# mravanelli/pytorch-kaldi

Hardware: AMD Instinct MI355X
Metric: train_frames_per_sec (higher is better)
Workload: dtype bf16

## Files before the change

### include/pk_amd.h

```cpp
#ifndef PK_AMD_H
#define PK_AMD_H

#include <stdint.h>

#ifdef __cplusplus
extern "C" {
#endif

#define PK_PREC_F32 0
#define PK_PREC_BF16 1

#define PK_ACT_LINEAR 0
#define PK_ACT_RELU 1
#define PK_ACT_TANH 2
#define PK_ACT_SIGMOID 3
#define PK_ACT_LEAKY_RELU 4
#define PK_ACT_ELU 5

#define PK_CELL_LIGRU 0
#define PK_CELL_RNN 1
#define PK_CELL_LSTM 2
#define PK_CELL_GRU 3
#define PK_CELL_MINGRU 4

#define PK_REC_STEPWISE 0
#define PK_REC_PERSISTENT 1

int pk_version(void);
const char* pk_last_error(void);
int pk_num_cu(void);

int pk_gemm(void* stream, int prec, int M, int N, int K, float alpha, const float* A, int64_t a_rs,
            int64_t a_cs, const float* B, int64_t b_rs, int64_t b_cs, float beta, float* C, int64_t ldc,
            const float* bias, int splitk, float* workspace);
void pk_gemm_f32_set_form(int form);

int pk_gemm_bf16_tile_m(int M);
int pk_gemm_bf16_auto_splitk(int M, int N, int K);
int pk_gemm_bf16_auto_splitk_cus(int M, int N, int K, int cus);
void pk_gemm_bf16_set_tile(int tile);
int pk_gemm_bf16(void* stream, int M, int N, int K, float alpha, const uint16_t* A, int64_t lda, int a_kc,
                 const uint16_t* B, int64_t ldb, int b_kc, float beta, float* C, int64_t ldc, const float* bias,
                 int splitk, float* workspace);
int64_t pk_gemm_bf16_stats_floats(int M, int N);
int pk_gemm_bf16_stats(void* stream, int M, int N, int K, float alpha, const uint16_t* A, int64_t lda, int a_kc,
                       const uint16_t* B, int64_t ldb, int b_kc, float* C, int64_t ldc, const float* bias, float* stats,
                       int* row_blocks);
int pk_cvt_bf16(void* stream, const float* src, int64_t ld_src, int64_t rows, int nseg, int seglen, int segpad,
                uint16_t* dst, int64_t ld_dst);

int64_t pk_bn_partial_floats(int64_t M, int64_t N);
int pk_bn_stats(void* stream, const float* x, int64_t ldx, int64_t M, int64_t N, float* partial, float* mean,
                float* var);
int pk_bn_stats_merge(void* stream, const float* partial, int rb, int64_t N, float* mean, float* var);
int pk_bn_finalize(void* stream, int64_t N, const float* mean, const float* var, const float* gamma,
                   const float* beta, float eps, float* scale, float* shift, float* running_mean,
                   float* running_var, float momentum, double count);
int pk_bn_finalize_gates(void* stream, int G, int H, const float* mean, const float* var, const float* gamma,
                         const float* beta, float eps, float* scale, float* shift, float* const* running_mean,
                         float* const* running_var, int64_t* const* num_batches, float momentum, double count);
int pk_bn_stats_merge_finalize_gates(void* stream, const float* partial, int rb, int G, int H, float* mean, float* var,
                                     const float* gamma, const float* beta, float eps, float* scale, float* shift,
                                     float* const* running_mean, float* const* running_var, int64_t* const* num_batches,
                                     float momentum, double count);
int pk_affine_act_fwd(void* stream, const float* x, int64_t ldx, int64_t M, int64_t N, const float* scale,
                      const float* shift, int act, const float* mask, float* y, int64_t ldy);
int pk_act_bwd(void* stream, const float* dy, const float* a, const float* mask, int act, int64_t n, float* g);
int pk_bn_bwd_reduce(void* stream, const float* g, const float* g2, int64_t ldg, const float* x, int64_t ldx,
                     int64_t M, int64_t N, const float* mean, const float* var, float eps, float* partial,
                     float* sum_g, float* sum_gx);
int pk_bn_bwd_apply(void* stream, const float* g, const float* g2, int64_t ldg, const float* x, int64_t ldx,
                    int64_t M, int64_t N, const float* mean, const float* var, float eps, const float* gamma,
                    const float* sum_g, const float* sum_gx, double count, float* dx, int64_t lddx);
int pk_bn_bwd_bf16(void* stream, const uint16_t* g0, const uint16_t* g1, int64_t g_pitch, int G, int H, const float* x,
                   int64_t ldx, int64_t M, const float* mean, const float* var, float eps, const float* gamma,
                   double count, float* partial, float* sum_g, float* sum_gx, uint16_t* out, int64_t out_pitch,
                   float* acc_beta, float* acc_gamma);
int pk_bn_act_bwd_small_covers(int64_t M, int64_t N);
int pk_bn_act_bwd_small(void* stream, const float* dy, const float* a, const float* mask, int act, const float* z,
                        const float* mean, const float* var, float eps, const float* gamma, int64_t M, int64_t N,
                        uint16_t* dzb, int64_t ldb, float* dz, float* sum_g, float* sum_gx, float* acc_beta,
                        float* acc_gamma, float* db, float* acc_bias);
int pk_colsum(void* stream, const float* g, const float* g2, int64_t ldg, int64_t M, int64_t N, float* partial,
              float* out);
int pk_add(void* stream, const float* a, const float* b, int64_t n, float* out);

int pk_mt19937_bernoulli(void* stream, uint32_t* state, int64_t n, float keep, float* out);

int pk_sinc_bank_fwd(void* stream, const float* low_hz, const float* band_hz, const float* n_, const float* window, int N, int K,
                     float sample_rate, float min_low, float min_band, float* filt, float* mx, int32_t* kstar);
int pk_sinc_bank_bwd(void* stream, const float* g, const float* low_hz, const float* band_hz, const float* n_, const float* window,
                     const float* mx, const int32_t* kstar, int N, int K, float sample_rate, float min_low, float min_band,
                     float* dlow, float* dband);

int pk_ln_last_act_drop_fwd(void* stream, const float* z, int64_t B, int C, int L, const float* gamma, const float* beta,
                            float eps, int act, const float* mask, float* a, float* y, float* mean, float* rinv);
int pk_ln_last_act_drop_bwd(void* stream, const float* dy, const float* z, const float* a, const float* mask, int64_t B, int C,
                            int L, const float* gamma, const float* mean, const float* rinv, float eps, int act, float* dz,
                            float* pg);

int pk_layernorm_fwd(void* stream, const float* x, int64_t rows, int64_t F, const float* gamma, const float* beta,
                     float eps, float* y, float* mean, float* rinv);
int pk_layernorm_bwd(void* stream, const float* dy, const float* x, int64_t rows, int64_t F, const float* gamma,
                     const float* mean, const float* rinv, float eps, float* dx, float* dgx);

int pk_logsoftmax_fwd(void* stream, const float* x, int64_t rows, int64_t N, float* y);
int pk_logsoftmax_bwd(void* stream, const float* dy, const float* y, int64_t rows, int64_t N, float* dx);
int pk_logsoftmax_bwd_ld(void* stream, const float* dy, const float* y, int64_t rows, int64_t N, float* dx, int64_t lddx);
int pk_logsoftmax_fwd_ld(void* stream, const float* x, int64_t ldx, int64_t rows, int64_t N, float* y);
int64_t pk_logsoftmax_bwd_bf16_partial_floats(int64_t rows, int64_t N);
int pk_logsoftmax_bwd_bf16(void* stream, const float* dy, const float* y, int64_t rows, int64_t N, uint16_t* dxb,
                           int64_t ldb, float* partial, float* colsum);
int64_t pk_nll_err_partial_floats(int64_t rows);
int pk_nll_err_fwd(void* stream, const float* y, const int64_t* lab, int64_t ignore_index, int64_t rows, int64_t N,
                   float* partial, float* out4, float* loss_out, float* bad_acc);
int pk_logsoftmax_fwd_ld_argmax(void* stream, const float* x, int64_t ldx, int64_t rows, int64_t N, float* y, int32_t* amax);
int pk_nll_err_fwd_argmax(void* stream, const float* y, const int64_t* lab, const int32_t* amax, int64_t ignore_index,
                          int64_t rows, int64_t N, float* partial, float* out4, float* loss_out, float* bad_acc);
int pk_nll_logsoftmax_bwd_bf16(void* stream, const float* y, const int64_t* lab, const float* dloss, const float* count,
                               int64_t ignore_index, int64_t rows, int64_t N, uint16_t* dxb, int64_t ldb, float* partial,
                               float* colsum);
int pk_logsoftmax_bwd_bf16_p(void* stream, const float* dy, const float* y, int64_t rows, int64_t N, uint16_t* dxb,
                             int64_t ldb, int64_t pitch, float* partial, float* colsum);
int pk_nll_logsoftmax_bwd_bf16_p(void* stream, const float* y, const int64_t* lab, const float* dloss, const float* count,
                                 int64_t ignore_index, int64_t rows, int64_t N, uint16_t* dxb, int64_t ldb, int64_t pitch,
                                 float* partial, float* colsum);

int pk_rec_num_saved(int cell);
int pk_rec_num_gates(int cell);
int64_t pk_rec_work_floats(int cell, int T, int B, int bidir, int H);
int64_t pk_rec_ln_saved_floats(int T, int B, int bidir, int H);
int64_t pk_rec_ln_work_floats(int T, int B, int bidir, int H);
int pk_rec_fwd(void* stream, int algo, int prec, int cell, int act, int T, int B, int bidir, int H,
               const float* P, const float* pscale, const float* pshift, const float* U, const float* mask,
               float mask_scalar, const float* ln_gamma, const float* ln_beta, float* Y, float* S, float* LNS,
               float* work);
int pk_rec_bwd(void* stream, int algo, int prec, int cell, int act, int T, int B, int bidir, int H,
               const float* U, const float* mask, float mask_scalar, const float* ln_gamma, const float* Y,
               const float* S, const float* LNS, const float* dY, float* dP2, float* dU, float* dln_gamma,
               float* dln_beta, float* work);

int pk_rec_plan_cus(int R, int H);
int pk_rec_self_fill(int cell);
int pk_rec_fwd_bf16(void* stream, int cell, int act, int T, int B, int bidir, int H, const float* P,
                    const float* pscale, const float* pshift, const float* U, const float* mask, float mask_scalar,
                    float* Y, float* S, uint16_t* Yb, int64_t y_pitch, int prefilled);
int pk_rec_bwd_bf16(void* stream, int cell, int act, int T, int B, int bidir, int H, const float* U, const float* mask,
                    float mask_scalar, const float* Y, const float* S, const float* dY, float* dP2, uint16_t* dGb,
                    int64_t g_pitch, int prefilled);
int pk_rec_fwd_bf16_ln(void* stream, int cell, int act, int T, int B, int bidir, int H, const float* P,
                       const float* pscale, const float* pshift, const float* U, const float* mask, float mask_scalar,
                       const float* ln_gamma, const float* ln_beta, float ln_eps, float* Y, float* S, float* LNS,
                       uint16_t* Yb, int64_t y_pitch, int prefilled, float* lnwork);
int pk_rec_bwd_bf16_ln(void* stream, int cell, int act, int T, int B, int bidir, int H, const float* U, const float* mask,
                       float mask_scalar, const float* ln_gamma, float ln_eps, const float* Y, const float* S,
                       const float* LNS, const float* dY, float* dP2, uint16_t* dGb, int64_t g_pitch, int prefilled,
                       float* lnwork, float* dln_gamma, float* dln_beta);
void pk_persist2_set_trace(void* dev_buf);
void pk_persist2_set_empty_step(int on);
void pk_persist2_set_mode(int force_safe);
void pk_persist2_set_poll_delay(int units);
void pk_persist2_set_lstm_waves(int waves);
int pk_persist2_get_lstm_waves(void);
void pk_rec_helper_set_mode(int mode);
int pk_rec_helper_get_mode(void);
int pk_rec2p_fwd_bf16(void* stream, int cell, int act, int T, int B, int bidir, int H, const float* P,
                      const float* pscale, const float* pshift, const float* U, const float* mask, float mask_scalar,
                      float* Y, float* S, uint16_t* Yb, uint16_t* Xb, int64_t y_pitch, int prefilled);
int pk_rec2p_bwd_bf16(void* stream, int cell, int act, int T, int B, int bidir, int H, const float* U, const float* mask,
                      float mask_scalar, const float* Y, const float* S, const float* dY, uint16_t* dGb, int64_t g_pitch,
                      int prefilled);
int pk_rec2p_fwd_bf16_ln(void* stream, int cell, int act, int T, int B, int bidir, int H, const float* P,
                         const float* pscale, const float* pshift, const float* U, const float* mask, float mask_scalar,
                         const float* ln_gamma, const float* ln_beta, float ln_eps, float* Y, float* S, float* LNS,
                         uint16_t* Yb, uint16_t* Xb, int64_t y_pitch, int prefilled, float* lnwork);
int pk_rec2p_bwd_bf16_ln(void* stream, int cell, int act, int T, int B, int bidir, int H, const float* U, const float* mask,
                         float mask_scalar, const float* ln_gamma, float ln_eps, const float* Y, const float* S,
                         const float* LNS, const float* dY, uint16_t* dGb, int64_t g_pitch, int prefilled, float* lnwork,
                         float* dln_gamma, float* dln_beta);
unsigned pk_persist2_error_count(void);
void pk_persist2_error_reset(void);

int pk_conv1d_pool_fwd(void* stream, const float* x, const float* w, const float* bias, int B, int Cin, int L,
                       int Cout, int K, int pool, float* y, int32_t* argmax, float* work);
int64_t pk_conv_fwd_work_floats(int Cin, int Cout, int K);
int64_t pk_conv_partial_floats(int B, int Cin, int L, int Cout, int K, int pool);
int pk_conv1d_pool_bwd(void* stream, const float* x, const float* w, const float* dy, const int32_t* argmax, int B,
                       int Cin, int L, int Cout, int K, int pool, float* dw, float* dbias, float* dx,
                       float* partial);

int pk_rmsprop_step(void* stream, float* p, const float* g, float* square_avg, int64_t n, float lr, float alpha,
                    float eps, float weight_decay);
int pk_sgd_step(void* stream, float* p, const float* g, float* momentum_buf, int64_t n, float lr, float momentum,
                float weight_decay, int first_step);
int pk_adam_step(void* stream, float* p, const float* g, float* exp_avg, float* exp_avg_sq, float* max_exp_avg_sq,
                 int64_t n, float lr, float beta1, float beta2, float eps, float weight_decay, int step);
int pk_fused_step(void* stream, int kind, float* p, float* g, float* s0, float* s1, float* s2, int64_t n, float lr, float h0,
                  float h1, float h2, float weight_decay, int step, int zero_grad, const int64_t* segs, int nseg,
                  uint16_t* shadow);
#define PK_OPT_CENTERED 1u
#define PK_OPT_NESTEROV 2u
int pk_fused_step_ex(void* stream, int kind, float* p, float* g, float* s0, float* s1, float* s2, int64_t n, float lr, float h0,
                     float h1, float h2, float weight_decay, unsigned flags, int step, int zero_grad, const int64_t* segs,
                     int nseg, uint16_t* shadow);

#define PK_QUAT_MAX_GATES 8
int pk_quat_assemble(void* stream, const float* const* comps, const float* base, int G, int I, int O, float* W);
int pk_quat_fold(void* stream, const float* dW, int G, int I, int O, float beta, float* const* dcomps, float* dbase);

#define PK_PACK_MAX_GATES 8
int pk_gates_pack(void* stream, const float* w_ih, const float* w_hh, const float* b_ih, const float* b_hh, int G, int H, int D,
                  const int* perm, float* Wcat, float* Ucat, float* bcat);
int pk_gates_unpack(void* stream, const float* dWcat, const float* dUcat, const float* dbcat, int G, int H, int D,
                    const int* perm, float* dw_ih, float* dw_hh, float* db_ih, float* db_hh);
int pk_seq_join_fwd(void* stream, const float* yf, const float* yb, const float* mask, float scale, int64_t T, int64_t B,
                    int64_t H, int ndir, float* y, float* y_rev);
int pk_seq_join_bwd(void* stream, const float* dy, const float* dy_rev, const float* mask, float scale, int64_t T, int64_t B,
                    int64_t H, int ndir, float* dyf, float* dyb);

int pk_seq_pack_len(void* stream, const float* x, const int32_t* lens, int64_t T, int64_t B, int64_t D, float* out_f,
                    float* out_r, int64_t ldo);
int pk_seq_join_len(void* stream, const float* hf, const float* hb, int64_t ldi, const int32_t* lens, int64_t T, int64_t B,
                    int64_t H, float* y_f, float* y_r, int64_t ldo);

int pk_post_normalize(void* stream, const float* x, const int64_t* rows, int64_t R, int64_t n, int64_t C,
                      const void* logprior, void* out, int f64);

unsigned pk_persist_error_count(void);
void pk_persist_error_reset(void);
// ... 41 lines not shown
```

### pytorch-kaldi_amd/_lib.py

```python
import ctypes
import os
import re
import threading

HERE = os.path.dirname(os.path.abspath(__file__))
LIB_PATH = os.path.join(HERE, "lib", "libpk_amd.so")
HEADER = os.path.join(HERE, "..", "include", "pk_amd.h")

_lock = threading.Lock()
_lib = None

c_void_p, c_int, c_float, c_double, c_int64 = ctypes.c_void_p, ctypes.c_int, ctypes.c_float, ctypes.c_double, ctypes.c_int64
P = c_void_p

SIGNATURES = {
    "pk_version": (c_int, []),
    "pk_last_error": (ctypes.c_char_p, []),
    "pk_num_cu": (c_int, []),
    "pk_gemm": (c_int, [P, c_int, c_int, c_int, c_int, c_float, P, c_int64, c_int64, P, c_int64, c_int64, c_float, P,
                        c_int64, P, c_int, P]),
    "pk_gemm_f32_set_form": (None, [c_int]),
    "pk_gemm_bf16_tile_m": (c_int, [c_int]),
    "pk_gemm_bf16_auto_splitk": (c_int, [c_int, c_int, c_int]),
    "pk_gemm_bf16_set_tile": (None, [c_int]),
    "pk_gemm_bf16": (c_int, [P, c_int, c_int, c_int, c_float, P, c_int64, c_int, P, c_int64, c_int, c_float, P, c_int64, P,
                             c_int, P]),
    "pk_gemm_bf16_stats_floats": (c_int64, [c_int, c_int]),
    "pk_gemm_bf16_stats": (c_int, [P, c_int, c_int, c_int, c_float, P, c_int64, c_int, P, c_int64, c_int, P, c_int64, P, P, P]),
    "pk_bn_stats_merge": (c_int, [P, P, c_int, c_int64, P, P]),
    "pk_cvt_bf16": (c_int, [P, P, c_int64, c_int64, c_int, c_int, c_int, P, c_int64]),
    "pk_bn_partial_floats": (c_int64, [c_int64, c_int64]),
    "pk_bn_stats": (c_int, [P, P, c_int64, c_int64, c_int64, P, P, P]),
    "pk_bn_finalize": (c_int, [P, c_int64, P, P, P, P, c_float, P, P, P, P, c_float, c_double]),
    "pk_bn_finalize_gates": (c_int, [P, c_int, c_int, P, P, P, P, c_float, P, P, P, P, P, c_float, c_double]),
    "pk_bn_stats_merge_finalize_gates": (c_int, [P, P, c_int, c_int, c_int, P, P, P, P, c_float, P, P, P, P, P, c_float,
                                                 c_double]),
    "pk_affine_act_fwd": (c_int, [P, P, c_int64, c_int64, c_int64, P, P, c_int, P, P, c_int64]),
    "pk_act_bwd": (c_int, [P, P, P, P, c_int, c_int64, P]),
    "pk_bn_bwd_reduce": (c_int, [P, P, P, c_int64, P, c_int64, c_int64, c_int64, P, P, c_float, P, P, P]),
    "pk_bn_bwd_apply": (c_int, [P, P, P, c_int64, P, c_int64, c_int64, c_int64, P, P, c_float, P, P, P, c_double, P,
                                c_int64]),
    "pk_bn_bwd_bf16": (c_int, [P, P, P, c_int64, c_int, c_int, P, c_int64, c_int64, P, P, c_float, P, c_double, P, P, P, P,
                               c_int64, P, P]),
    "pk_colsum": (c_int, [P, P, P, c_int64, c_int64, c_int64, P, P]),
    "pk_add": (c_int, [P, P, P, c_int64, P]),
    "pk_mt19937_bernoulli": (c_int, [P, P, c_int64, c_float, P]),
    "pk_sinc_bank_fwd": (c_int, [P, P, P, P, P, c_int, c_int, c_float, c_float, c_float, P, P, P]),
    "pk_sinc_bank_bwd": (c_int, [P, P, P, P, P, P, P, P, c_int, c_int, c_float, c_float, c_float, P, P]),
    "pk_ln_last_act_drop_fwd": (c_int, [P, P, c_int64, c_int, c_int, P, P, c_float, c_int, P, P, P, P, P]),
    "pk_ln_last_act_drop_bwd": (c_int, [P, P, P, P, P, c_int64, c_int, c_int, P, P, P, c_float, c_int, P, P]),
    "pk_layernorm_fwd": (c_int, [P, P, c_int64, c_int64, P, P, c_float, P, P, P]),
    "pk_layernorm_bwd": (c_int, [P, P, P, c_int64, c_int64, P, P, P, c_float, P, P]),
    "pk_logsoftmax_fwd": (c_int, [P, P, c_int64, c_int64, P]),
    "pk_logsoftmax_bwd": (c_int, [P, P, P, c_int64, c_int64, P]),
    "pk_logsoftmax_bwd_ld": (c_int, [P, P, P, c_int64, c_int64, P, c_int64]),
    "pk_logsoftmax_fwd_ld": (c_int, [P, P, c_int64, c_int64, c_int64, P]),
    "pk_logsoftmax_fwd_ld_argmax": (c_int, [P, P, c_int64, c_int64, c_int64, P, P]),
    "pk_logsoftmax_bwd_bf16_partial_floats": (c_int64, [c_int64, c_int64]),
    "pk_logsoftmax_bwd_bf16": (c_int, [P, P, P, c_int64, c_int64, P, c_int64, P, P]),
    "pk_nll_err_partial_floats": (c_int64, [c_int64]),
    "pk_nll_err_fwd": (c_int, [P, P, P, c_int64, c_int64, c_int64, P, P, P, P]),
    "pk_nll_err_fwd_argmax": (c_int, [P, P, P, P, c_int64, c_int64, c_int64, P, P, P, P]),
    "pk_nll_logsoftmax_bwd_bf16": (c_int, [P, P, P, P, P, c_int64, c_int64, c_int64, P, c_int64, P, P]),
    "pk_logsoftmax_bwd_bf16_p": (c_int, [P, P, P, c_int64, c_int64, P, c_int64, c_int64, P, P]),
    "pk_nll_logsoftmax_bwd_bf16_p": (c_int, [P, P, P, P, P, c_int64, c_int64, c_int64, P, c_int64, c_int64, P, P]),
    "pk_rec_num_saved": (c_int, [c_int]),
    "pk_rec_num_gates": (c_int, [c_int]),
    "pk_conv1d_pool_dgrad": (c_int, [P, P, P, P, c_int, c_int, c_int, c_int, c_int, c_int, P, P]),
    "pk_conv_bf16_covers": (c_int, [c_int, c_int, c_int, c_int]),
    "pk_conv_bf16_work_floats": (c_int64, [c_int, c_int, c_int, c_int, c_int, c_int, c_int]),
    "pk_conv1d_pool_fwd_bf16": (c_int, [P, P, P, P, c_int, c_int, c_int, c_int, c_int, c_int, P, P, P]),
    "pk_conv1d_pool_bwd_bf16": (c_int, [P, P, P, P, P, c_int, c_int, c_int, c_int, c_int, c_int, P, P, P]),
    "pk_bn_act_bwd_small_covers": (c_int, [c_int64, c_int64]),
    "pk_bn_act_bwd_small": (c_int, [P, P, P, P, c_int, P, P, P, c_float, P, c_int64, c_int64, P, c_int64, P, P, P, P, P, P, P]),
    "pk_rec_work_floats": (c_int64, [c_int, c_int, c_int, c_int, c_int]),
    "pk_rec_ln_saved_floats": (c_int64, [c_int, c_int, c_int, c_int]),
    "pk_rec_ln_work_floats": (c_int64, [c_int, c_int, c_int, c_int]),
    "pk_rec_fwd": (c_int, [P, c_int, c_int, c_int, c_int, c_int, c_int, c_int, c_int, P, P, P, P, P, c_float, P, P, P,
                           P, P, P]),
    "pk_rec_bwd": (c_int, [P, c_int, c_int, c_int, c_int, c_int, c_int, c_int, c_int, P, P, c_float, P, P, P, P, P, P,
                           P, P, P, P]),
    "pk_rec_self_fill": (c_int, [c_int]),
    "pk_rec_plan_cus": (c_int, [c_int, c_int]),
    "pk_gemm_bf16_auto_splitk_cus": (c_int, [c_int, c_int, c_int, c_int]),
    "pk_rec_fwd_bf16": (c_int, [P, c_int, c_int, c_int, c_int, c_int, c_int, P, P, P, P, P, c_float, P, P, P, c_int64, c_int]),
    "pk_rec_bwd_bf16": (c_int, [P, c_int, c_int, c_int, c_int, c_int, c_int, P, P, c_float, P, P, P, P, P, c_int64, c_int]),
    "pk_rec2p_fwd_bf16_ln": (c_int, [P, c_int, c_int, c_int, c_int, c_int, c_int, P, P, P, P, P, c_float, P, P, c_float, P, P, P,
                                     P, P, c_int64, c_int, P]),
    "pk_rec2p_bwd_bf16_ln": (c_int, [P, c_int, c_int, c_int, c_int, c_int, c_int, P, P, c_float, P, c_float, P, P, P, P, P,
                                     c_int64, c_int, P, P, P]),
    "pk_rec_fwd_bf16_ln": (c_int, [P, c_int, c_int, c_int, c_int, c_int, c_int, P, P, P, P, P, c_float, P, P, c_float, P, P, P,
                                   P, c_int64, c_int, P]),
    "pk_rec_bwd_bf16_ln": (c_int, [P, c_int, c_int, c_int, c_int, c_int, c_int, P, P, c_float, P, c_float, P, P, P, P, P, P,
                                   c_int64, c_int, P, P, P]),
    "pk_rec2p_fwd_bf16": (c_int, [P, c_int, c_int, c_int, c_int, c_int, c_int, P, P, P, P, P, c_float, P, P, P, P, c_int64, c_int]),
    "pk_rec2p_bwd_bf16": (c_int, [P, c_int, c_int, c_int, c_int, c_int, c_int, P, P, c_float, P, P, P, P, c_int64, c_int]),
    "pk_persist2_set_trace": (None, [P]),
    "pk_persist2_set_empty_step": (None, [c_int]),
    "pk_persist2_set_mode": (None, [c_int]),
    "pk_persist2_set_poll_delay": (None, [c_int]),
    "pk_persist2_set_lstm_waves": (None, [c_int]),
    "pk_rec_helper_set_mode": (None, [c_int]),
    "pk_rec_helper_get_mode": (c_int, []),
    "pk_persist2_get_lstm_waves": (c_int, []),
    "pk_persist2_error_count": (ctypes.c_uint, []),
    "pk_persist2_error_reset": (None, []),
    "pk_conv1d_pool_fwd": (c_int, [P, P, P, P, c_int, c_int, c_int, c_int, c_int, c_int, P, P, P]),
    "pk_conv_fwd_work_floats": (c_int64, [c_int, c_int, c_int]),
    "pk_conv_partial_floats": (c_int64, [c_int, c_int, c_int, c_int, c_int, c_int]),
    "pk_conv1d_pool_bwd": (c_int, [P, P, P, P, P, c_int, c_int, c_int, c_int, c_int, c_int, P, P, P, P]),
    "pk_ark_open": (P, [ctypes.c_char_p, c_int64]),
    "pk_ark_close": (None, [P]),
    "pk_ark_next": (c_int, [P, c_int, ctypes.c_char_p, c_int, ctypes.POINTER(c_int64), ctypes.POINTER(c_int64)]),
    "pk_ark_read": (c_int, [P, P]),
    "pk_ark_skip": (c_int, [P]),
    "pk_ivec_next": (c_int, [P, ctypes.c_char_p, c_int, ctypes.POINTER(c_int64)]),
    "pk_ivec_read": (c_int, [P, P]),
    "pk_context_window": (c_int, [P, c_int64, c_int64, c_int, c_int, P]),
    "pk_mean_var_norm": (c_int, [P, c_int64, c_int64]),
    "pk_rmsprop_step": (c_int, [P, P, P, P, c_int64, c_float, c_float, c_float, c_float]),
    "pk_sgd_step": (c_int, [P, P, P, P, c_int64, c_float, c_float, c_float, c_int]),
    "pk_adam_step": (c_int, [P, P, P, P, P, P, c_int64, c_float, c_float, c_float, c_float, c_float, c_int]),
    "pk_fused_step": (c_int, [P, c_int, P, P, P, P, P, c_int64, c_float, c_float, c_float, c_float, c_float, c_int, c_int, P, c_int, P]),
    "pk_fused_step_ex": (c_int, [P, c_int, P, P, P, P, P, c_int64, c_float, c_float, c_float, c_float, c_float, ctypes.c_uint, c_int,
                                 c_int, P, c_int, P]),
    "pk_quat_assemble": (c_int, [P, P, P, c_int, c_int, c_int, P]),
    "pk_quat_fold": (c_int, [P, P, c_int, c_int, c_int, c_float, P, P]),
    "pk_gates_pack": (c_int, [P, P, P, P, P, c_int, c_int, c_int, P, P, P, P]),
    "pk_gates_unpack": (c_int, [P, P, P, P, c_int, c_int, c_int, P, P, P, P, P]),
    "pk_seq_join_fwd": (c_int, [P, P, P, P, c_float, c_int64, c_int64, c_int64, c_int, P, P]),
    "pk_seq_join_bwd": (c_int, [P, P, P, P, c_float, c_int64, c_int64, c_int64, c_int, P, P]),
    "pk_seq_pack_len": (c_int, [P, P, P, c_int64, c_int64, c_int64, P, P, c_int64]),
    "pk_seq_join_len": (c_int, [P, P, P, c_int64, P, c_int64, c_int64, c_int64, P, P, c_int64]),
    "pk_post_normalize": (c_int, [P, P, P, c_int64, c_int64, c_int64, P, P, c_int]),
    "pk_persist_error_count": (ctypes.c_uint, []),
    "pk_persist_error_reset": (None, []),
    "pk_linear_bn_act_bf16_covers": (c_int, [c_int64, c_int64, c_int64]),
    "pk_linear_bn_act_bf16": (c_int, [P, c_int, c_int, c_int, P, c_int64, P, c_int64, P, P, P, c_float, c_float, P, P, c_int, P,
                                      P, P, P, P, c_int64, P, P]),
    "pk_gemm_bf16_small_splitk": (c_int, [c_int, c_int, c_int]),
    "pk_linear_bn_act_bf16_sk": (c_int, [P, c_int, c_int, c_int, P, c_int64, P, c_int64, P, P, P, c_float, c_float, P, P, c_int, P,
                                         P, P, P, P, c_int64, P, P, c_int, P]),
    "pk_selftest_mfma": (c_int, [P, ctypes.POINTER(c_int)]),
    "pk_selftest_permlane": (c_int, [P, ctypes.POINTER(c_int)]),
    "pk_selftest_dpp_row_sum": (c_int, [P, ctypes.POINTER(c_int)]),
    "pk_selftest_cu_hog": (c_int, [P, c_int, c_int, P]),
}


def declared_symbols():
    with open(HEADER) as f:
        text = re.sub(r"/\*.*?\*/", "", f.read(), flags=re.S)
    return sorted(set(re.findall(r"\b(pk_[a-z0-9_]+)\s*\(", text)))


class PkError(RuntimeError):
    pass


def _map_torch_hip_runtime():
    import torch

    hip = os.path.join(os.path.dirname(torch.__file__), "lib", "libamdhip64.so")
    if os.path.exists(hip):
        ctypes.CDLL(hip, mode=ctypes.RTLD_GLOBAL)
    return hip


# ... 188 lines not shown
```

### pytorch-kaldi_amd/csrc/pk_gemm_bf16.hip

```cpp
#include <stdlib.h>

#include "pk_common.h"

namespace {

constexpr int TM = 128, TN = 128, TK = 64;
typedef short s4v __attribute__((ext_vector_type(4)));

struct BArgs {
    int M, N, K;
    float alpha, beta;
    const unsigned short* A;
    long lda;
    const unsigned short* B;
    long ldb;
    float* C;
    long ldc;
    const float* bias;
    float* ws;
    int k_per_split;
    int tiles_m, tiles_n;
    int items, per_xcd;
    const unsigned short* zeros;
    float* stats;
};

__device__ unsigned short g_zero_page[64];

__device__ __forceinline__ int swz_kc(int row) { return (row >> 1) & 7; }
__device__ __forceinline__ int swz_km(int kr) { return 2 * ((kr & 3) | ((kr >> 1) & 4)); }

__device__ __forceinline__ void glds16(const void* gsrc, void* lds_wave_base) {
    __builtin_amdgcn_global_load_lds((const __attribute__((address_space(1))) void*)gsrc,
                                     (__attribute__((address_space(3))) void*)lds_wave_base, 16, 0, 0);
}

__device__ __forceinline__ unsigned long long sel_addr(bool ok, const void* a, const void* z) {
    const unsigned long long m = 0ull - (unsigned long long)ok;
    return ((unsigned long long)a & m) | ((unsigned long long)z & ~m);
}

template <bool KC, int NT = 256>
__device__ __forceinline__ void stage(const unsigned short* __restrict__ base, long ld, int r0, int rmax, int k0, int kmax,
                                      const unsigned short* zeros, unsigned char* buf, int tid, int wave) {
#pragma unroll
    for (int j = 0; j < 1024 / NT; ++j) {
        const int q = j * NT + tid;
        unsigned long long src;
        if (KC) {
            const int row = q >> 3, ps = q & 7;
            const int ks = ps ^ swz_kc(row);
            int gr = r0 + row;
            gr = gr < rmax ? gr : rmax - 1;
            const int gk = k0 + ks * 8;
            src = sel_addr(gk < kmax, base + (long)gr * ld + gk, zeros);
        } else {
            const int kr = q >> 4, ps = q & 15;
            const int cs = ps ^ swz_km(kr);
            int gc = r0 + cs * 8;
            if (gc >= rmax) gc = (rmax - 1) & ~7;
            const int gk = k0 + kr;
            src = sel_addr(gk < kmax, base + (long)gk * ld + gc, zeros);
        }
        glds16(reinterpret_cast<const void*>(src), buf + (j * NT + wave * 64) * 16);
    }
}

template <bool KC, int NT = 256>
struct TileSrc {
    unsigned long long a[1024 / NT];
    unsigned long long step;
    __device__ __forceinline__ void init(const unsigned short* __restrict__ base, long ld, int r0, int rmax, int k0, int tid) {
#pragma unroll
        for (int j = 0; j < 1024 / NT; ++j) {
            const int q = j * NT + tid;
            if (KC) {
                const int row = q >> 3, ps = q & 7;
                const int ks = ps ^ swz_kc(row);
                int gr = r0 + row;
                gr = gr < rmax ? gr : rmax - 1;
                a[j] = (unsigned long long)(base + (long)gr * ld + k0 + ks * 8);
            } else {
                const int kr = q >> 4, ps = q & 15;
                const int cs = ps ^ swz_km(kr);
                int gc = r0 + cs * 8;
                if (gc >= rmax) gc = (rmax - 1) & ~7;
                a[j] = (unsigned long long)(base + (long)(k0 + kr) * ld + gc);
            }
        }
        step = KC ? (unsigned long long)(TK * 2) : (unsigned long long)ld * (TK * 2);
    }
    __device__ __forceinline__ void issue(unsigned char* buf, int wave) {
#pragma unroll
        for (int j = 0; j < 1024 / NT; ++j) {
            glds16(reinterpret_cast<const void*>(a[j]), buf + (j * NT + wave * 64) * 16);
            a[j] += step;
        }
    }
};

template <bool KC>
__device__ __forceinline__ bf16x8 frag(const unsigned char* buf, int sub, int kk, int lane) {
    if (KC) {
        const int row = sub + (lane & 15);
        const int ks = kk * 4 + (lane >> 4);
        const int ps = ks ^ swz_kc(row);
        return *reinterpret_cast<const bf16x8*>(buf + row * 128 + ps * 16);
// ... 699 lines not shown
#pragma unroll
                for (int r = 0; r < 4; ++r) o[r] += p.beta * c[r];
            }
        }
        *reinterpret_cast<f32x4*>(dst) = o;
    } else {
#pragma unroll
        for (int r = 0; r < 4; ++r) {
            if (col + r >= p.N) continue;
            float o = v[r];
            if (p.ws == nullptr) {
                o = p.alpha * o + (p.bias ? p.bias[col + r] : 0.f);
                if (p.beta != 0.f) o += p.beta * dst[r];
            }
            dst[r] = o;
        }
    }
}

__device__ __forceinline__ void tile_colstats(const BArgs& p, const f32x4 (&acc)[2][2][4][2], int m0, int n0, int tm, int wm,
                                              int wn, int lane, float* sh) {
    const int nrows = (p.M - m0) < 256 ? (p.M - m0) : 256;
    __syncthreads();
    float part[2][2][4];
#pragma unroll
    for (int pass = 0; pass < 2; ++pass) {
        float mu[2][2][4];
        if (pass == 1) {
#pragma unroll
            for (int bh = 0; bh < 2; ++bh)
#pragma unroll
                for (int j = 0; j < 2; ++j)
#pragma unroll
                    for (int r = 0; r < 4; ++r) {
                        const int cl = bh * 128 + wn * 32 + j * 16 + (lane >> 4) * 4 + r;
                        mu[bh][j][r] = (sh[cl] + sh[256 + cl]) / (float)nrows;
                    }
        }
#pragma unroll
        for (int bh = 0; bh < 2; ++bh)
#pragma unroll
            for (int j = 0; j < 2; ++j)
#pragma unroll
                for (int r = 0; r < 4; ++r) {
                    float t = 0.f;
#pragma unroll
                    for (int ah = 0; ah < 2; ++ah)
#pragma unroll
                        for (int i = 0; i < 4; ++i) {
                            const bool in = ah * 128 + wm * 64 + i * 16 + (lane & 15) < nrows;
                            const float v = acc[ah][bh][i][j][r];
                            const float d = pass == 0 ? v : v - mu[bh][j][r];
                            t += in ? (pass == 0 ? d : d * d) : 0.f;
                        }
#pragma unroll
                    for (int off = 1; off < 16; off <<= 1) t += __shfl_xor(t, off);
                    part[bh][j][r] = t;
                }
        if ((lane & 15) == 0) {
#pragma unroll
            for (int bh = 0; bh < 2; ++bh)
#pragma unroll
                for (int j = 0; j < 2; ++j)
#pragma unroll
                    for (int r = 0; r < 4; ++r)
                        sh[pass * 512 + wm * 256 + bh * 128 + wn * 32 + j * 16 + (lane >> 4) * 4 + r] = part[bh][j][r];
        }
        __syncthreads();
    }
    const int c = threadIdx.x;
    if (c < 256 && n0 + c < p.N) {
        const float mean_v = (sh[c] + sh[256 + c]) / (float)nrows;
        const float m2_v = sh[512 + c] + sh[768 + c];
        float* o = p.stats + ((long)tm * p.N + n0 + c) * 3;
        o[0] = (float)nrows;
        o[1] = p.alpha * mean_v + (p.bias ? p.bias[n0 + c] : 0.f);
        o[2] = p.alpha * p.alpha * m2_v;
    }
}

#define PK_VMCNT(n) asm volatile("s_waitcnt vmcnt(" #n ")" ::: "memory")

template <bool A_KC, bool B_KC>
__global__ __launch_bounds__(512, 1) void gemm_bf16_256_kernel(BArgs p) {
    extern __shared__ __attribute__((aligned(1024))) unsigned char smem[];
    const int tid = threadIdx.x, lane = tid & 63, wave = tid >> 6;
    const int wm = wave >> 2, wn = wave & 3;
    const int item = (blockIdx.x & 7) * p.per_xcd + (blockIdx.x >> 3);
    if (item >= p.items) return;
    const int tn = item % p.tiles_n;
    const int tm = (item / p.tiles_n) % p.tiles_m;
    const int split = item / (p.tiles_n * p.tiles_m);
    const int m0 = tm * 256, n0 = tn * 256;
    const int kbeg = split * p.k_per_split;
    const int kend = min(p.K, kbeg + p.k_per_split);
    const int nk = (kend - kbeg + TK - 1) / TK;
    const bool a1_live = m0 + 128 < p.M, b1_live = n0 + 128 < p.N;

    f32x4 acc[2][2][4][2];
#pragma unroll
    for (int a = 0; a < 2; ++a)
#pragma unroll
        for (int b = 0; b < 2; ++b)
#pragma unroll
            for (int i = 0; i < 4; ++i)
#pragma unroll
                for (int j = 0; j < 2; ++j) acc[a][b][i][j] = f32x4{0.f, 0.f, 0.f, 0.f};

    PieceSrc<A_KC> sa0, sa1;
    PieceSrc<B_KC> sb0, sb1;
    sa0.init(p.A, p.lda, m0, p.M, kbeg, tid);
    sa1.init(p.A, p.lda, m0 + 128, p.M, kbeg, tid);
    sb0.init(p.B, p.ldb, n0, p.N, kbeg, tid);
    sb1.init(p.B, p.ldb, n0 + 128, p.N, kbeg, tid);
    auto slot = [&](int kt, int piece) { return smem + (((kt & 1) * 4 + piece) * PIECE); };
    auto issueA0 = [&](int kt, auto C) { sa0.template issue<decltype(C)::value != 0>(kbeg + kt * TK, kend, p.zeros, slot(kt, 0), tid, wave); };
    auto issueB0 = [&](int kt, auto C) { sb0.template issue<decltype(C)::value != 0>(kbeg + kt * TK, kend, p.zeros, slot(kt, 1), tid, wave); };
    auto issueB1 = [&](int kt, auto C) { sb1.template issue<decltype(C)::value != 0>(kbeg + kt * TK, kend, p.zeros, slot(kt, 2), tid, wave); };
    auto issueA1 = [&](int kt, auto C) { sa1.template issue<decltype(C)::value != 0>(kbeg + kt * TK, kend, p.zeros, slot(kt, 3), tid, wave); };

    issueA0(0, BoolK<1>()); issueB0(0, BoolK<1>()); issueB1(0, BoolK<1>()); issueA1(0, BoolK<1>());
    issueA0(1, BoolK<1>()); issueB0(1, BoolK<1>()); issueB1(1, BoolK<1>());
    PK_VMCNT(10);
    __builtin_amdgcn_s_barrier();
    if (wm == 1) __builtin_amdgcn_s_barrier();

    bf16x8 a[4][2], b[2][2][2];
#define PK_MFMA_BLOCK(AH, BH)                                                                                         \
    do {                                                                                                              \
        __builtin_amdgcn_s_setprio(1);                                                                                \
        _Pragma("unroll") for (int kk = 0; kk < 2; ++kk) _Pragma("unroll") for (int i = 0; i < 4; ++i)                   \
            _Pragma("unroll") for (int j = 0; j < 2; ++j)                                                              \
                acc[AH][BH][i][j] = __builtin_amdgcn_mfma_f32_16x16x32_bf16(b[BH][j][kk], a[i][kk], acc[AH][BH][i][j], 0, 0, 0); \
        __builtin_amdgcn_s_setprio(0);                                                                                \
    } while (0)
#define PK_END_L()                                         \
    do {                                                   \
        asm volatile("s_waitcnt lgkmcnt(0)" ::: "memory"); \
        __builtin_amdgcn_sched_barrier(0);                 \
        __builtin_amdgcn_s_barrier();                      \
    } while (0)
    auto ktile = [&](int kt, auto FQC, auto CKC) {
        constexpr bool FQ = decltype(FQC)::value != 0;
        issueA1(kt + 1, CKC);
#pragma unroll
        for (int kk = 0; kk < 2; ++kk) {
#pragma unroll
            for (int j = 0; j < 2; ++j) b[0][j][kk] = frag8<B_KC>(slot(kt, 1), wn * 32 + j * 16, kk, lane);
#pragma unroll
            for (int i = 0; i < 4; ++i) a[i][kk] = frag8<A_KC>(slot(kt, 0), wm * 64 + i * 16, kk, lane);
        }
        PK_VMCNT(10);
        PK_END_L();
        PK_MFMA_BLOCK(0, 0);
        __builtin_amdgcn_s_barrier();
        issueA0(kt + 2, CKC);
#pragma unroll
        for (int kk = 0; kk < 2; ++kk)
#pragma unroll
            for (int j = 0; j < 2; ++j) b[1][j][kk] = frag8<B_KC>(slot(kt, 2), wn * 32 + j * 16, kk, lane);
        PK_VMCNT(10);
        PK_END_L();
        if (FQ || b1_live) PK_MFMA_BLOCK(0, 1);
        __builtin_amdgcn_s_barrier();
        issueB0(kt + 2, CKC);
#pragma unroll
        for (int kk = 0; kk < 2; ++kk)
#pragma unroll
            for (int i = 0; i < 4; ++i) a[i][kk] = frag8<A_KC>(slot(kt, 3), wm * 64 + i * 16, kk, lane);
        PK_END_L();
        if (FQ || (a1_live && b1_live)) PK_MFMA_BLOCK(1, 1);
        __builtin_amdgcn_s_barrier();
        issueB1(kt + 2, CKC);
        PK_VMCNT(10);
        __builtin_amdgcn_s_barrier();
        if (FQ || a1_live) PK_MFMA_BLOCK(1, 0);
        __builtin_amdgcn_s_barrier();
    };
    const int nk_full = (kend - kbeg) / TK;
    auto run = [&](auto FQC) {
        int kt = 0;
        for (; kt + 2 < nk_full; ++kt) ktile(kt, FQC, BoolK<0>());
        for (; kt < nk; ++kt) ktile(kt, FQC, BoolK<1>());
    };
    if (a1_live && b1_live) run(BoolK<1>());
    else run(BoolK<0>());
#undef PK_MFMA_BLOCK
#undef PK_END_L
    if (wm == 0) __builtin_amdgcn_s_barrier();
    PK_VMCNT(0);
    if constexpr (A_KC && B_KC) {
        if (p.stats != nullptr) tile_colstats(p, acc, m0, n0, tm, wm, wn, lane, reinterpret_cast<float*>(smem));
    }
    const bool vec_ok = (((uintptr_t)(p.ws ? p.ws : p.C) & 15) == 0) && (((p.ws ? (long)p.N : p.ldc) & 3) == 0);
    const bool interior = m0 + 256 <= p.M && n0 + 256 <= p.N;
    if (vec_ok && interior && (p.ws != nullptr || p.beta == 0.f)) {
        const bool direct = p.ws == nullptr;
        float* base = direct ? p.C : p.ws + (long)split * p.M * p.N;
        const long ld = direct ? p.ldc : (long)p.N;
        const float alpha = direct ? p.alpha : 1.f;
#pragma unroll
        for (int bh = 0; bh < 2; ++bh)
#pragma unroll
            for (int j = 0; j < 2; ++j) {
                const int col = n0 + bh * 128 + wn * 32 + j * 16 + (lane >> 4) * 4;
                f32x4 bv = f32x4{0.f, 0.f, 0.f, 0.f};
                if (direct && p.bias != nullptr) {
#pragma unroll
                    for (int r = 0; r < 4; ++r) bv[r] = p.bias[col + r];
                }
#pragma unroll
                for (int ah = 0; ah < 2; ++ah)
#pragma unroll
                    for (int i = 0; i < 4; ++i) {
                        const int row = m0 + ah * 128 + wm * 64 + i * 16 + (lane & 15);
                        const f32x4 v = acc[ah][bh][i][j];
                        f32x4 o;
#pragma unroll
                        for (int r = 0; r < 4; ++r) o[r] = alpha * v[r] + bv[r];
                        *reinterpret_cast<f32x4*>(base + (long)row * ld + col) = o;
                    }
            }
        return;
    }
#pragma unroll
    for (int ah = 0; ah < 2; ++ah)
#pragma unroll
        for (int bh = 0; bh < 2; ++bh)
#pragma unroll
            for (int i = 0; i < 4; ++i)
#pragma unroll
                for (int j = 0; j < 2; ++j)
                    store_frag(p, acc[ah][bh][i][j], m0 + ah * 128 + wm * 64 + i * 16 + (lane & 15),
                               n0 + bh * 128 + wn * 32 + j * 16 + (lane >> 4) * 4, split, vec_ok);
}

__global__ void splitk_reduce_bf_kernel(const float* __restrict__ ws, int splitk, int M, int N, float alpha, float beta,
                                        const float* __restrict__ bias, float* __restrict__ C, long ldc) {
    const long total = (long)M * N;
    if ((N & 3) == 0 && (ldc & 3) == 0 && (((uintptr_t)C | (uintptr_t)ws) & 15) == 0) {
        const long quads = total >> 2;
        for (long qd = blockIdx.x * (long)blockDim.x + threadIdx.x; qd < quads; qd += (long)gridDim.x * blockDim.x) {
            const long i = qd << 2;
            const int row = (int)(i / N), col = (int)(i - (long)row * N);
            f32x4 s = f32x4{0.f, 0.f, 0.f, 0.f};
            for (int k0 = 0; k0 < splitk; k0 += 8) {
                f32x4 t[8];
#pragma unroll
                for (int j = 0; j < 8; ++j) t[j] = *reinterpret_cast<const f32x4*>(ws + (long)(k0 + j < splitk ? k0 + j : splitk - 1) * total + i);
#pragma unroll
                for (int j = 0; j < 8; ++j)
#pragma unroll
                    for (int e = 0; e < 4; ++e) s[e] += (k0 + j < splitk) ? t[j][e] : 0.f;
            }
            float* c = C + (long)row * ldc + col;
            f32x4 o;
#pragma unroll
            for (int e = 0; e < 4; ++e) o[e] = alpha * s[e] + (bias ? bias[col + e] : 0.f);
            if (beta != 0.f) {
                const f32x4 cv = *reinterpret_cast<const f32x4*>(c);
#pragma unroll
                for (int e = 0; e < 4; ++e) o[e] += beta * cv[e];
            }
            *reinterpret_cast<f32x4*>(c) = o;
        }
        return;
    }
    for (long i = blockIdx.x * (long)blockDim.x + threadIdx.x; i < total; i += (long)gridDim.x * blockDim.x) {
        const int row = (int)(i / N), col = (int)(i % N);
        float s = 0.f;
        for (int k = 0; k < splitk; ++k) s += ws[(long)k * total + i];
        float o = alpha * s + (bias ? bias[col] : 0.f);
        float* c = C + (long)row * ldc + col;
        if (beta != 0.f) o += beta * (*c);
        *c = o;
    }
}

__global__ void cvt_bf16_kernel(const float* __restrict__ src, long lds, long rows, int nseg, int seglen, int segpad,
                                unsigned short* __restrict__ dst, long ldd) {
    const long chunks_per_row = ldd >> 3;
    const long total = rows * chunks_per_row;
    for (long i = blockIdx.x * (long)blockDim.x + threadIdx.x; i < total; i += (long)gridDim.x * blockDim.x) {
        const long r = i / chunks_per_row;
        const int c0 = (int)(i - r * chunks_per_row) * 8;
        const float* s = src + r * lds;
        unsigned pk[4];
#pragma unroll
        for (int e = 0; e < 4; ++e) {
            float v[2];
#pragma unroll
            for (int h = 0; h < 2; ++h) {
                const int c = c0 + 2 * e + h;
                const int sg = c / segpad, off = c - sg * segpad;
                v[h] = (sg < nseg && off < seglen) ? s[sg * seglen + off] : 0.f;
            }
            pk[e] = pk_pack_bf2(v[0], v[1]);
        }
        *reinterpret_cast<uint4*>(dst + r * ldd + c0) = make_uint4(pk[0], pk[1], pk[2], pk[3]);
    }
}

}

extern "C" int pk_cvt_bf16(void* stream, const float* src, int64_t ld_src, int64_t rows, int nseg, int seglen, int segpad,
                           uint16_t* dst, int64_t ld_dst) {
    if (rows <= 0) return 0;
    PK_REQUIRE(nseg >= 1 && seglen >= 1 && segpad >= seglen, "pk_cvt_bf16: bad segments");
    PK_REQUIRE((ld_dst % 8) == 0 && ld_dst >= (int64_t)nseg * segpad - (segpad - seglen) && ((uintptr_t)dst & 15) == 0,
               "pk_cvt_bf16: destination pitch must be a multiple of 8 elements and hold every segment");
    const long total = rows * (ld_dst >> 3);
    long blocks = (total + 255) / 256;
    if (blocks > 8192) blocks = 8192;
    hipLaunchKernelGGL(cvt_bf16_kernel, dim3((unsigned)blocks), dim3(256), 0, pk_stream(stream), src, (long)ld_src,
                       (long)rows, nseg, seglen, segpad, (unsigned short*)dst, (long)ld_dst);
    PK_LAUNCH_CHECK();
    return 0;
}

static int g_gemm_tile_forced = -1;
extern "C" void pk_gemm_bf16_set_tile(int tile) { g_gemm_tile_forced = (tile == 128 || tile == 256) ? tile : 0; }
static int gemm_tile_for(int M, int N, int a_kc, int b_kc, int K = 1 << 30) {
    int& forced = g_gemm_tile_forced;
    if (forced < 0) {
        const char* e = pk_experiment("gemm_tile");
        forced = (e && atoi(e) == 128) ? 128 : (e && atoi(e) == 256) ? 256 : 0;
    }
    if (forced) return forced;
    static int rows256 = -1;
    if (rows256 < 0) {
        const char* e = pk_experiment("gemm_tile_rows");
        rows256 = (e && atoi(e) == 0) ? 0 : 1;
    }
    if (rows256 && a_kc && M >= 16384 && N >= 1024) return 256;
    if (!a_kc && !b_kc && M >= 1024 && N >= 1024) {
        const long tiles256 = (long)((M + 255) / 256) * ((N + 255) / 256);
        if (K < 2048 && tiles256 < 64) return 128;
        return 256;
    }
    return 128;
}

extern "C" int pk_gemm_bf16_tile_m(int M) {
    (void)M;
    return TM;
}

extern "C" int pk_gemm_bf16_auto_splitk_cus(int M, int N, int K, int cus) {
    if (K < 2048 || M <= 0 || N <= 0) return 1;
    const int t = gemm_tile_for(M, N, 0, 0);
    const long tiles = (long)((M + t - 1) / t) * ((N + t - 1) / t);
    long ncu = pk_num_cu();
    if (cus > 0 && cus < ncu) ncu = cus;
    long s = (t == 256 ? ncu : 2 * ncu) / (tiles > 0 ? tiles : 1);
    if (s < 1) s = 1;
    if (s > 32) s = 32;
    const long kmax = K / 512 > 0 ? K / 512 : 1;
    if (s > kmax) s = kmax;
    return (int)s;
}
extern "C" int pk_gemm_bf16_auto_splitk(int M, int N, int K) { return pk_gemm_bf16_auto_splitk_cus(M, N, K, 0); }

static int gemm_bf16_impl(void* stream, int M, int N, int K, float alpha, const uint16_t* A, int64_t lda, int a_kc,
                          const uint16_t* B, int64_t ldb, int b_kc, float beta, float* C, int64_t ldc, const float* bias,
                          int splitk, float* workspace, float* stats) {
    if (M <= 0 || N <= 0) return 0;
    PK_REQUIRE(K >= 0, "pk_gemm_bf16: negative K");
    PK_REQUIRE((lda % 8) == 0 && (ldb % 8) == 0 && ((uintptr_t)A & 15) == 0 && ((uintptr_t)B & 15) == 0,
               "pk_gemm_bf16: operands need 16-byte aligned bases and pitches that are multiples of 8 elements");
    PK_REQUIRE(!a_kc || (K % 8) == 0 || lda >= ((K + 7) & ~7), "pk_gemm_bf16: A pitch shorter than K rounded up to 8");
    PK_REQUIRE(!b_kc || (K % 8) == 0 || ldb >= ((K + 7) & ~7), "pk_gemm_bf16: B pitch shorter than K rounded up to 8");
    PK_REQUIRE(a_kc || lda >= ((M + 7) & ~7), "pk_gemm_bf16: k-major A needs a pitch of at least M rounded up to 8");
    PK_REQUIRE(b_kc || ldb >= ((N + 7) & ~7), "pk_gemm_bf16: k-major B needs a pitch of at least N rounded up to 8");
    hipStream_t st = pk_stream(stream);
    BArgs p;
    p.M = M; p.N = N; p.K = K;
    p.alpha = alpha; p.beta = beta;
    p.A = A; p.lda = lda; p.B = B; p.ldb = ldb;
    p.C = C; p.ldc = ldc; p.bias = bias;
    p.stats = stats;
    const int tile = gemm_tile_for(M, N, a_kc, b_kc, K);
    PK_REQUIRE(stats == nullptr || (tile == 256 && a_kc && b_kc && splitk <= 1 && beta == 0.f), "pk_gemm_bf16_stats: internal: shape not covered");
    p.tiles_m = (M + tile - 1) / tile;
    p.tiles_n = (N + tile - 1) / tile;
    static void* zp = nullptr;
    if (zp == nullptr) PK_CHECK_HIP(hipGetSymbolAddress(&zp, HIP_SYMBOL(g_zero_page)));
    p.zeros = (const unsigned short*)zp;
    if (splitk < 1) splitk = 1;
    if (splitk > 1) {
        PK_REQUIRE(workspace != nullptr, "pk_gemm_bf16: split-K needs a workspace");
        int kps = (K + splitk - 1) / splitk;
        kps = ((kps + TK - 1) / TK) * TK;
        splitk = kps > 0 ? (K + kps - 1) / kps : 1;
        p.k_per_split = kps;
    }
    if (splitk <= 1) {
        splitk = 1;
        p.k_per_split = ((K + TK - 1) / TK) * TK;
        if (p.k_per_split == 0) p.k_per_split = TK;
    }
    p.ws = splitk > 1 ? workspace : nullptr;
    p.items = splitk * p.tiles_m * p.tiles_n;
    p.per_xcd = (p.items + 7) / 8;
    {
        static int skinny_on = -1;
        if (skinny_on < 0) {
            const char* e = pk_experiment("gemm_skinny");
            skinny_on = (e && e[0] == '0') ? 0 : 1;
        }
        if (skinny_on && !g_gemm_tile_forced && a_kc && M <= TM && splitk > 1 && p.k_per_split <= SK_TILES * TK && stats == nullptr) {
            static bool attr_done = false;
            if (!attr_done) {
                PK_CHECK_HIP(hipFuncSetAttribute((const void*)gemm_bf16sk_kernel<true>, hipFuncAttributeMaxDynamicSharedMemorySize, SK_TILES * SSTAGE));
                PK_CHECK_HIP(hipFuncSetAttribute((const void*)gemm_bf16sk_kernel<false>, hipFuncAttributeMaxDynamicSharedMemorySize, SK_TILES * SSTAGE));
                attr_done = true;
            }
            const dim3 sgrid((unsigned)((N + SN - 1) / SN), (unsigned)splitk);
            if (b_kc) hipLaunchKernelGGL((gemm_bf16sk_kernel<true>), sgrid, dim3(256), SK_TILES * SSTAGE, st, p);
            else hipLaunchKernelGGL((gemm_bf16sk_kernel<false>), sgrid, dim3(256), SK_TILES * SSTAGE, st, p);
            PK_LAUNCH_CHECK();
            const long total = (long)M * N;
            int blocks = (int)((total + 255) / 256);
            if (blocks > 2048) blocks = 2048;
            hipLaunchKernelGGL(splitk_reduce_bf_kernel, dim3(blocks), dim3(256), 0, st, workspace, splitk, M, N, alpha, beta,
                               bias, C, (long)ldc);
            PK_LAUNCH_CHECK();
            return 0;
        }
        if (skinny_on && !g_gemm_tile_forced && !a_kc && !b_kc && splitk == 1 && K <= 512 && stats == nullptr &&
            (long)((M + TM - 1) / TM) * ((N + TN - 1) / TN) <= 192 && M >= 64 && N >= 64) {
            const dim3 tgrid((unsigned)((N + 63) / 64), (unsigned)((M + 63) / 64));
            hipLaunchKernelGGL(gemm_bf16_t64_kernel, tgrid, dim3(256), T64_TILES * T64_STAGE, st, p);
            PK_LAUNCH_CHECK();
            return 0;
        }
        if (skinny_on && !g_gemm_tile_forced && a_kc && M <= TM && N >= 4 * SN && splitk == 1 && stats == nullptr) {
            BnActArgs q = {};
            const dim3 sgrid((unsigned)((N + SN - 1) / SN));
            if (b_kc) hipLaunchKernelGGL((gemm_bf16s_kernel<false, true>), sgrid, dim3(256), 2 * SSTAGE, st, p, q);
            else hipLaunchKernelGGL((gemm_bf16s_kernel<false, false>), sgrid, dim3(256), 2 * SSTAGE, st, p, q);
            PK_LAUNCH_CHECK();
            return 0;
        }
    }
    if (tile == 256) {
        static bool attr_done = false;
        if (!attr_done) {
            PK_CHECK_HIP(hipFuncSetAttribute((const void*)gemm_bf16_256_kernel<true, true>, hipFuncAttributeMaxDynamicSharedMemorySize, 8 * PIECE));
            PK_CHECK_HIP(hipFuncSetAttribute((const void*)gemm_bf16_256_kernel<true, false>, hipFuncAttributeMaxDynamicSharedMemorySize, 8 * PIECE));
            PK_CHECK_HIP(hipFuncSetAttribute((const void*)gemm_bf16_256_kernel<false, true>, hipFuncAttributeMaxDynamicSharedMemorySize, 8 * PIECE));
            PK_CHECK_HIP(hipFuncSetAttribute((const void*)gemm_bf16_256_kernel<false, false>, hipFuncAttributeMaxDynamicSharedMemorySize, 8 * PIECE));
            attr_done = true;
        }
        dim3 grid256((unsigned)(p.per_xcd * 8)), block512(512);
        const size_t lds256 = 8 * PIECE;
        if (a_kc && b_kc) hipLaunchKernelGGL((gemm_bf16_256_kernel<true, true>), grid256, block512, lds256, st, p);
        else if (a_kc && !b_kc) hipLaunchKernelGGL((gemm_bf16_256_kernel<true, false>), grid256, block512, lds256, st, p);
        else if (!a_kc && b_kc) hipLaunchKernelGGL((gemm_bf16_256_kernel<false, true>), grid256, block512, lds256, st, p);
        else hipLaunchKernelGGL((gemm_bf16_256_kernel<false, false>), grid256, block512, lds256, st, p);
        PK_LAUNCH_CHECK();
        if (splitk > 1) {
            const long total = (long)M * N;
            int blocks = (int)((total + 255) / 256);
            if (blocks > 2048) blocks = 2048;
            hipLaunchKernelGGL(splitk_reduce_bf_kernel, dim3(blocks), dim3(256), 0, st, workspace, splitk, M, N, alpha, beta,
                               bias, C, (long)ldc);
            PK_LAUNCH_CHECK();
        }
        return 0;
    }
    dim3 grid((unsigned)(p.per_xcd * 8)), block(256);
    static int forced = -1;
    if (forced < 0) {
        const char* e = pk_experiment("gemm_stages");
        forced = (e && e[0] == '1') ? 1 : (e && e[0] == '2') ? 2 : 0;
        PK_CHECK_HIP(hipFuncSetAttribute((const void*)gemm_bf16x_kernel<true, true, 2>, hipFuncAttributeMaxDynamicSharedMemorySize, 65536));
        PK_CHECK_HIP(hipFuncSetAttribute((const void*)gemm_bf16x_kernel<true, false, 2>, hipFuncAttributeMaxDynamicSharedMemorySize, 65536));
        PK_CHECK_HIP(hipFuncSetAttribute((const void*)gemm_bf16x_kernel<false, true, 2>, hipFuncAttributeMaxDynamicSharedMemorySize, 65536));
        PK_CHECK_HIP(hipFuncSetAttribute((const void*)gemm_bf16x_kernel<false, false, 2>, hipFuncAttributeMaxDynamicSharedMemorySize, 65536));
    }
    const int stages = forced ? forced : (a_kc ? 1 : 2);
    const size_t lds = stages == 2 ? 65536 : 32768;
#define PK_LAUNCH_BF(ST)                                                                                     \
    do {                                                                                                     \
        if (a_kc && b_kc) hipLaunchKernelGGL((gemm_bf16x_kernel<true, true, ST>), grid, block, lds, st, p);    \
        else if (a_kc && !b_kc) hipLaunchKernelGGL((gemm_bf16x_kernel<true, false, ST>), grid, block, lds, st, p); \
        else if (!a_kc && b_kc) hipLaunchKernelGGL((gemm_bf16x_kernel<false, true, ST>), grid, block, lds, st, p); \
        else hipLaunchKernelGGL((gemm_bf16x_kernel<false, false, ST>), grid, block, lds, st, p);              \
    } while (0)
    if (stages == 2) PK_LAUNCH_BF(2);
    else PK_LAUNCH_BF(1);
#undef PK_LAUNCH_BF
    PK_LAUNCH_CHECK();
    if (splitk > 1) {
        const long total = (long)M * N;
        int blocks = (int)((total + 255) / 256);
        if (blocks > 2048) blocks = 2048;
        hipLaunchKernelGGL(splitk_reduce_bf_kernel, dim3(blocks), dim3(256), 0, st, workspace, splitk, M, N, alpha, beta,
                           bias, C, (long)ldc);
        PK_LAUNCH_CHECK();
    }
    return 0;
}

extern "C" int pk_gemm_bf16(void* stream, int M, int N, int K, float alpha, const uint16_t* A, int64_t lda, int a_kc,
                            const uint16_t* B, int64_t ldb, int b_kc, float beta, float* C, int64_t ldc,
                            const float* bias, int splitk, float* workspace) {
    return gemm_bf16_impl(stream, M, N, K, alpha, A, lda, a_kc, B, ldb, b_kc, beta, C, ldc, bias, splitk, workspace, nullptr);
}

extern "C" int64_t pk_gemm_bf16_stats_floats(int M, int N) { return (int64_t)((M + 255) / 256) * N * 3; }

extern "C" int pk_gemm_bf16_stats(void* stream, int M, int N, int K, float alpha, const uint16_t* A, int64_t lda, int a_kc,
                                  const uint16_t* B, int64_t ldb, int b_kc, float* C, int64_t ldc, const float* bias,
                                  float* stats, int* row_blocks) {
    PK_REQUIRE(row_blocks != nullptr, "pk_gemm_bf16_stats: null row_blocks");
    const bool fused = stats != nullptr && M > 0 && N > 0 && K > 0 && a_kc && b_kc && gemm_tile_for(M, N, a_kc, b_kc) == 256;
    *row_blocks = fused ? (M + 255) / 256 : 0;
    return gemm_bf16_impl(stream, M, N, K, alpha, A, lda, a_kc, B, ldb, b_kc, 0.f, C, ldc, bias, 1, nullptr,
                          fused ? stats : nullptr);
}

extern "C" int pk_gemm_bf16_small_splitk(int M, int N, int K) {
    if (M < 1 || M > TM || N < 1 || K < 2 * TK) return 1;
    const int col_tiles = (N + SN - 1) / SN;
    int s = 256 / col_tiles;
    const int need = (K + SK_TILES * TK - 1) / (SK_TILES * TK);
    if (s < need) s = need;
    if (s > 16) s = 16;
    const int tiles = (K + TK - 1) / TK;
    if (s > tiles) s = tiles;
    if (s < 2) return 1;
    int kps = ((K + s - 1) / s + TK - 1) / TK * TK;
    if (kps > SK_TILES * TK) return 1;
    return (K + kps - 1) / kps;
}

extern "C" int pk_linear_bn_act_bf16_sk(void* stream, int M, int N, int K, const uint16_t* xb, int64_t ldx, const uint16_t* wb,
                                        int64_t ldw, const float* bias, const float* gamma, const float* beta, float eps,
                                        float momentum, float* running_mean, float* running_var, int act, const float* mask,
                                        float* z, float* a, float* y, uint16_t* yb, int64_t ldyb, float* mean, float* var,
                                        int splitk, float* ws) {
    PK_REQUIRE(pk_linear_bn_act_bf16_covers(M, N, K), "pk_linear_bn_act_bf16_sk: needs 2 <= M <= 128 rows and N a multiple of 8 (got %d x %d)", M, N);
    PK_REQUIRE((ldx % 8) == 0 && (ldw % 8) == 0 && ((uintptr_t)xb & 15) == 0 && ((uintptr_t)wb & 15) == 0 && ldx >= ((K + 7) & ~7) &&
                   ldw >= ((K + 7) & ~7),
               "pk_linear_bn_act_bf16_sk: operands need 16-byte aligned bases and pitches that are multiples of 8 elements");
    PK_REQUIRE(z && a && yb && mean && var && (mask == nullptr || y != nullptr) && ldyb >= N && (ldyb % 4) == 0,
               "pk_linear_bn_act_bf16_sk: null output or bad pitch");
    PK_REQUIRE((((uintptr_t)z | (uintptr_t)a | (uintptr_t)y | (uintptr_t)mask | (uintptr_t)ws | (uintptr_t)bias) & 15) == 0 && ((uintptr_t)yb & 7) == 0,
               "pk_linear_bn_act_bf16_sk: fp32 matrices need 16-byte aligned bases");
    PK_REQUIRE(splitk >= 2 && ws != nullptr, "pk_linear_bn_act_bf16_sk: needs splitk >= 2 and a workspace of splitk x M x N floats");
    int kps = ((K + splitk - 1) / splitk + TK - 1) / TK * TK;
    PK_REQUIRE(kps <= SK_TILES * TK, "pk_linear_bn_act_bf16_sk: %d splits of K = %d exceed %d k-tiles per workgroup", splitk, K, SK_TILES);
    splitk = (K + kps - 1) / kps;
    hipStream_t st = pk_stream(stream);
    BArgs p;
    p.M = M; p.N = N; p.K = K;
    p.alpha = 1.f; p.beta = 0.f;
    p.A = xb; p.lda = ldx; p.B = wb; p.ldb = ldw;
    p.C = z; p.ldc = N; p.bias = nullptr;
    p.stats = nullptr; p.ws = ws;
    p.tiles_m = 1; p.tiles_n = (N + TN - 1) / TN;
    p.k_per_split = kps;
    p.items = p.tiles_n; p.per_xcd = (p.items + 7) / 8;
    static void* zp = nullptr;
    if (zp == nullptr) PK_CHECK_HIP(hipGetSymbolAddress(&zp, HIP_SYMBOL(g_zero_page)));
    p.zeros = (const unsigned short*)zp;
    static bool attr_done = false;
    if (!attr_done) {
        PK_CHECK_HIP(hipFuncSetAttribute((const void*)gemm_bf16sk_kernel<true>, hipFuncAttributeMaxDynamicSharedMemorySize, SK_TILES * SSTAGE));
        attr_done = true;
    }
    hipLaunchKernelGGL((gemm_bf16sk_kernel<true>), dim3((unsigned)((N + SN - 1) / SN), (unsigned)splitk), dim3(256), SK_TILES * SSTAGE, st, p);
    PK_LAUNCH_CHECK();
    BnActArgs q;
    q.gamma = gamma; q.beta = beta; q.mask = mask;
    q.eps = eps; q.momentum = momentum; q.unbias = M > 1 ? (float)M / (float)(M - 1) : 1.f;
    q.rmean = running_mean; q.rvar = running_var; q.mean = mean; q.var = var;
    q.zout = z; q.aout = a; q.yout = y; q.yb = (unsigned short*)yb; q.ldyb = ldyb; q.act = act;
    hipLaunchKernelGGL(linear_bn_act_epi_kernel, dim3((unsigned)((N + EP_COLS - 1) / EP_COLS)), dim3(256), 0, st, ws, splitk, M, N, bias, q);
    PK_LAUNCH_CHECK();
    return 0;
}

extern "C" int pk_linear_bn_act_bf16_covers(int64_t M, int64_t N, int64_t K) {
    return M >= 2 && M <= TM && N >= 8 && (N % 8) == 0 && K >= 1;
}
extern "C" int pk_linear_bn_act_bf16(void* stream, int M, int N, int K, const uint16_t* xb, int64_t ldx, const uint16_t* wb,
                                     int64_t ldw, const float* bias, const float* gamma, const float* beta, float eps,
                                     float momentum, float* running_mean, float* running_var, int act, const float* mask,
                                     float* z, float* a, float* y, uint16_t* yb, int64_t ldyb, float* mean, float* var) {
    PK_REQUIRE(pk_linear_bn_act_bf16_covers(M, N, K), "pk_linear_bn_act_bf16: needs 2 <= M <= 128 rows and N a multiple of 8 (got %d x %d)", M, N);
    PK_REQUIRE((ldx % 8) == 0 && (ldw % 8) == 0 && ((uintptr_t)xb & 15) == 0 && ((uintptr_t)wb & 15) == 0 && ldx >= ((K + 7) & ~7) &&
                   ldw >= ((K + 7) & ~7),
               "pk_linear_bn_act_bf16: operands need 16-byte aligned bases and pitches that are multiples of 8 elements");
    PK_REQUIRE(z && a && yb && mean && var && (mask == nullptr || y != nullptr) && ldyb >= N && (ldyb % 4) == 0,
               "pk_linear_bn_act_bf16: null output or bad pitch");
    PK_REQUIRE((((uintptr_t)z | (uintptr_t)a | (uintptr_t)y | (uintptr_t)mask) & 15) == 0 && ((uintptr_t)yb & 7) == 0,
               "pk_linear_bn_act_bf16: fp32 matrices need 16-byte aligned bases");
    hipStream_t st = pk_stream(stream);
    BArgs p;
    p.M = M; p.N = N; p.K = K;
    p.alpha = 1.f; p.beta = 0.f;
// ... 19 lines not shown
```

### pytorch-kaldi_amd/csrc/pk_rec2_common.h

```cpp
#pragma once
#ifndef PK_REC2_PRECISE
#define PK_CELL_FAST_MATH 1
#endif
#include "pk_cell.h"

#define PK_R2_FILL_AHEAD 4
struct R2Args {
    int T, B, R, H, Hp, YH, act;
    int C, Pn, rpc, row0;
    const float *P, *pscale, *pshift, *U, *mask;
    float mask_scalar;
    float* Y;
    float* S;
    unsigned short* Yb;
    unsigned short* Xb;
    int Ypitch;
    const float* dY;
    float* dP2;
    unsigned short* dGb;
    int Gpitch;
    float* Yx;
    float* dGx;
    float* Xx;
    unsigned* err;
    int spin_limit;
    float* trash;
    int poll_delay;
    int force_safe;
    unsigned* xcd_tab;
    unsigned hs_gen;
    unsigned long long* trace;
    int helper_delay;
    int self_fill;
    int flush_late;
    int empty_step;
    const float *ln_gamma, *ln_beta;
    float ln_eps;
    float* lnh;
    float* lnstat;
    float* lnx;
    float* lnpart;
    int ln_cg0;
    int ln_ncg;
};

struct Plan2 {
    int Pn, C, rpc, launches;
};

namespace {

typedef unsigned int u32x4 __attribute__((ext_vector_type(4)));

constexpr int KPAD = 576;
constexpr int KSTEPS = 18;
constexpr int RMAX = 16;

__host__ __device__ constexpr int pk_r2_lda_bf16(int k_elems) { return k_elems + 8 * ((((2 - k_elems / 8) % 16) + 16) % 16); }
__host__ __device__ constexpr int pk_r2_lda_f32(int k_elems) { return k_elems + 4 * ((((2 - k_elems / 4) % 16) + 16) % 16); }


#define PK_TRACE(slot)                                                                      \
    do {                                                                                    \
        if (TR && a.trace != nullptr && blockIdx.x == 0 && tid == 0) a.trace[(long)step_idx * 8 + (slot)] = __builtin_amdgcn_s_memtime(); \
    } while (0)

__device__ __forceinline__ bool has_sent16(const u32x4 v) {
    const unsigned m01 = v[0] > v[1] ? v[0] : v[1], m23 = v[2] > v[3] ? v[2] : v[3];
    return (m01 > m23 ? m01 : m23) == 0xFFFFFFFFu;
}
__device__ __forceinline__ unsigned short to_bf_pub(float f) {
    const unsigned short u = __builtin_bit_cast(unsigned short, (__bf16)f);
    return u == (unsigned short)0xFFFF ? (unsigned short)0x7FC0 : u;
}
__device__ __forceinline__ bool spin_check2(int& spins, int spin_limit, unsigned* err, int lane) {
    if (++spins > spin_limit) {
        if (lane == 0) atomicAdd_system(err, 1u);
        return true;
    }
    if ((spins & 63) == 0 && __hip_atomic_load(err, __ATOMIC_RELAXED, __HIP_MEMORY_SCOPE_SYSTEM) != 0u) return true;
    __builtin_amdgcn_s_sleep(1);
    return false;
}
__device__ __forceinline__ __amdgpu_buffer_rsrc_t make_rsrc(const void* p, unsigned bytes) {
    return __builtin_amdgcn_make_buffer_rsrc(const_cast<void*>(p), 0, (int)bytes, 0x00020000);
}

template <bool FAST>
__device__ __forceinline__ u32x4 poll_load(__amdgpu_buffer_rsrc_t rs, unsigned off) {
    return FAST ? __builtin_amdgcn_raw_buffer_load_b128(rs, off, 0, 2) : __builtin_amdgcn_raw_buffer_load_b128(rs, off, 0, 16);
}
template <bool FAST>
__device__ __forceinline__ void pub_store(__amdgpu_buffer_rsrc_t rs, unsigned off, u32x4 v) {
    if (FAST) __builtin_amdgcn_raw_buffer_store_b128(v, rs, off, 0, 0);
    else __builtin_amdgcn_raw_buffer_store_b128(v, rs, off, 0, 16);
}

template <int NCH, bool FAST>
__device__ __forceinline__ bool poll_to_lds(__amdgpu_buffer_rsrc_t rs, const unsigned (&goff)[NCH], const int (&loff)[NCH],
                                            unsigned char* tile, unsigned* err, int spin_limit, int lane, bool dead,
                                            int& retries) {
    u32x4 v[NCH];
#pragma unroll
    for (int i = 0; i < NCH; ++i) v[i] = poll_load<FAST>(rs, goff[i]);
    bool bad = false;
#pragma unroll
    for (int i = 0; i < NCH; ++i) bad = bad | has_sent16(v[i]);
    if (__any(bad) && !dead) {
        int spins = 0;
        while (true) {
#pragma unroll
            for (int i = 0; i < NCH; ++i)
                if (has_sent16(v[i])) v[i] = poll_load<FAST>(rs, goff[i]);
            bad = false;
#pragma unroll
            for (int i = 0; i < NCH; ++i) bad = bad | has_sent16(v[i]);
            ++retries;
            if (!__any(bad)) break;
            if (spin_check2(spins, spin_limit, err, lane)) {
                dead = true;
                break;
            }
        }
    }
#pragma unroll
    for (int i = 0; i < NCH; ++i) *reinterpret_cast<u32x4*>(tile + loff[i]) = v[i];
// ... 271 lines not shown
```

### pytorch-kaldi_amd/csrc/pk_rec_persist2.hip

```cpp
#include <atomic>
#include <stdlib.h>

#include "pk_rec2_common.h"

namespace {

template <int CELL, int ACT, bool TR, bool LN = false, bool NOSAVE = false>
__global__ __launch_bounds__(256, 1) void rec2_fwd_kernel(R2Args a) {
    const int act = ACT >= 0 ? ACT : a.act;
    constexpr int G = pk_cell_gates(CELL), NS = pk_cell_saved(CELL);
    constexpr int LDA = pk_r2_lda_bf16(KPAD);
    constexpr int ATILE = RMAX * LDA * 2;
    constexpr int NCH = (RMAX * (KPAD / 8) + 255) / 256;
    constexpr int NF = G + 1 + NS + (LN ? 1 : 0);
    constexpr int WAVE_LDS = NF * 1024 + 512;
    constexpr int LDS_TRASH = 2 * ATILE + 4 * WAVE_LDS;
    extern __shared__ __attribute__((aligned(16))) unsigned char smem[];

    const int tid = threadIdx.x, lane = tid & 63, wave = tid >> 6;
    const int c = blockIdx.x % a.C, p = blockIdx.x / a.C;
    const int H = a.H, Hp = a.Hp, B = a.B, T = a.T, GH = G * H;
    const int n_base = a.row0 + c * a.rpc;
    int nrows = a.R - n_base;
    nrows = nrows < a.rpc ? nrows : a.rpc;
    if (nrows <= 0) return;
    const int ubase = p * 64 + wave * 16;
    const int unit = ubase + (lane & 15);
    const bool unit_ok = unit < H;
    const int kq = lane >> 4;

    bf16x8 Bf[G][KSTEPS];
    {
        const unsigned szU = (unsigned)((size_t)G * H * H * 4);
        const __amdgpu_buffer_rsrc_t rsU = make_rsrc(a.U, szU);
#pragma unroll
        for (int g = 0; g < G; ++g) {
            u32x4 raw[KSTEPS][2];
#pragma unroll
            for (int kk = 0; kk < KSTEPS; ++kk) {
                const int k0 = kk * 32 + kq * 8;
                const unsigned off = (unsigned)(((g * H + unit) * H + k0) * 4);
                raw[kk][0] = __builtin_amdgcn_raw_buffer_load_b128(rsU, (unit_ok && k0 < H) ? off : szU, 0, 0);
                raw[kk][1] = __builtin_amdgcn_raw_buffer_load_b128(rsU, (unit_ok && k0 + 4 < H) ? off + 16 : szU, 0, 0);
            }
#pragma unroll
            for (int kk = 0; kk < KSTEPS; ++kk) {
                bf16x8 f;
#pragma unroll
                for (int e = 0; e < 8; ++e) {
                    const int k = kk * 32 + kq * 8 + e;
                    const float w = (k < H) ? __uint_as_float(raw[kk][e >> 2][e & 3]) : 0.f;
                    f[e] = (short)pk_f2bf(w);
                }
                Bf[g][kk] = f;
            }
        }
    }
    float psc[G], psh[G];
#pragma unroll
    for (int g = 0; g < G; ++g) {
        psc[g] = unit_ok ? a.pscale[g * H + unit] : 0.f;
        psh[g] = unit_ok ? a.pshift[g * H + unit] : 0.f;
    }
    for (int i = tid; i < (LDS_TRASH + 16) / 4; i += 256) reinterpret_cast<unsigned*>(smem)[i] = 0u;

    const int CPR = Hp >> 3;
    const unsigned TS = (unsigned)B * a.Ypitch * 2u;
    const unsigned szYb = (unsigned)T * TS;
    unsigned cbase[NCH], cstep[NCH];
    int clds[NCH];
#pragma unroll
    for (int i = 0; i < NCH; ++i) {
        const int ci = tid + 256 * i;
        const bool ok = ci < nrows * CPR;
        const int row = ok ? ci / CPR : 0, col = ok ? ci - row * CPR : 0;
        const int n = n_base + row;
        const int dir = n >= B ? 1 : 0, b = n - dir * B;
        cbase[i] = ok ? ((unsigned)b * a.Ypitch + dir * Hp + col * 8) * 2u + (unsigned)(dir ? (T - 1) : 0) * TS : szYb;
        cstep[i] = ok ? (dir ? 0u - TS : TS) : 0u;
        clds[i] = ok ? row * (LDA * 2) + col * 16 : LDS_TRASH;
    }
    float rvf[4], msk[4], hprev[4], cprev[4];
#pragma unroll
    for (int r = 0; r < 4; ++r) {
        const int row = kq * 4 + r, n = n_base + row;
        const bool ok = row < nrows && unit_ok;
        rvf[r] = ok ? 1.f : 0.f;
        msk[r] = (a.mask != nullptr && ok) ? a.mask[(long)n * H + unit] : a.mask_scalar;
        hprev[r] = 0.f;
        cprev[r] = 0.f;
    }
    const int vrow = lane >> 2, vu0 = ubase + (lane & 3) * 4;
    const int vn = n_base + (vrow < nrows ? vrow : 0);
    const int vdir = vn >= B ? 1 : 0, vb = vn - vdir * B;
    int vnv = H - vu0;
    vnv = vnv > 4 ? 4 : (vnv < 0 ? 0 : vnv);
    const int edge = __any(vnv > 0 && vnv < 4) != 0 ? ((H & 1) ? 2 : 1) : 0;
    vnv = vrow < nrows ? vnv : 0;
    const unsigned vP0 = ((unsigned)vb * GH + vu0), vPs = (unsigned)B * GH;
    const unsigned vY0 = ((unsigned)vb * a.YH + vdir * H + vu0), vYs = (unsigned)B * a.YH;
    const unsigned vS0 = (((unsigned)vdir * T * B + vb) * (NS * H) + vu0), vSs = (unsigned)B * NS * H;
    const int prow = lane >> 1, phalf = lane & 1;
    const int pu0 = ubase + phalf * 8;
    const bool pk_ok = lane < 32 && prow < nrows && pu0 < Hp;
    const int pn = n_base + (prow < nrows ? prow : 0);
    const int pdir = pn >= B ? 1 : 0, pb = pn - pdir * B;
    const unsigned pbase = pk_ok ? ((unsigned)pb * a.Ypitch + pdir * Hp + pu0) * 2u : szYb;

    unsigned char* wl = smem + 2 * ATILE + wave * WAVE_LDS;
    float* patchP = reinterpret_cast<float*>(wl);
    float* patchY = reinterpret_cast<float*>(wl + G * 1024);
    float* patchS = reinterpret_cast<float*>(wl + (G + 1) * 1024);
    float* patchL = reinterpret_cast<float*>(wl + (G + 1 + NS) * 1024);
    unsigned short* patchB = reinterpret_cast<unsigned short*>(wl + NF * 1024);
    const __amdgpu_buffer_rsrc_t rs = make_rsrc(a.Yb, szYb);
    float* trash = a.trash + (tid & 63) * 4;
    const LnSlots ls = LN ? ln_slots(a, c, p, wave, lane, T) : LnSlots();
    const __amdgpu_buffer_rsrc_t rsx = make_rsrc(LN ? (const void*)a.lnx : (const void*)a.Yb, LN ? ls.size : 0u);
    const float gam = (LN && unit_ok) ? a.ln_gamma[unit] : 0.f, bet = (LN && unit_ok) ? a.ln_beta[unit] : 0.f;
    const float invH = 1.0f / (float)H, inv_nm1 = 1.0f / (float)(H - 1);
    float piv[4] = {0.f, 0.f, 0.f, 0.f};
    pk_f32x2 st_val = {0.f, 0.f};
    const int st_row = kq * 4 + (lane & 3);
    const bool st_ok = LN && p == 0 && wave == 0 && (lane & 15) < 4 && st_row < nrows;
    float* const st_base = st_ok ? a.lnstat + (long)(n_base + st_row) * 2 : trash;
    const long st_step = st_ok ? (long)a.R * 2 : 0;

    f32x4 pv[G];
    auto load_proj = [&](int tt, auto E) {
        const unsigned ts = (unsigned)(vdir ? (T - 1 - tt) : tt);
#pragma unroll
        for (int g = 0; g < G; ++g) pv[g] = ld4<decltype(E)::value>(a.P, vP0 + ts * vPs + g * H, vnv);
    };
    const bool want_y = a.Y != nullptr;
    auto flush_outputs = [&](int tt, auto E) {
        constexpr int EE = decltype(E)::value;
        const unsigned ts = (unsigned)(vdir ? (T - 1 - tt) : tt);
        if (!NOSAVE || want_y) st4<EE>(a.Y, vY0 + ts * vYs, vnv, trash, patch_get_vec(patchY, lane));
        if constexpr (!NOSAVE) {
#pragma unroll
            for (int k = 0; k < NS; ++k) st4<EE>(a.S, vS0 + ts * vSs + k * H, vnv, trash, patch_get_vec(patchS + k * 256, lane));
        }
        if (LN) {
            st4<EE>(a.lnh, vY0 + ts * vYs, vnv, trash, patch_get_vec(patchL, lane));
            *reinterpret_cast<pk_f32x2*>(st_base + (long)tt * st_step) = st_val;
        }
    };
#define PK_LP0(E) load_proj(0, E)
    PK_EDGE_DISPATCH(PK_LP0);
    const u32x4 sentinel = u32x4{0xFFFFFFFFu, 0xFFFFFFFFu, 0xFFFFFFFFu, 0xFFFFFFFFu};
    if (a.self_fill) {
        for (int tt = 0; tt < PK_R2_FILL_AHEAD && tt < T; ++tt)
            pub_store<false>(rs, pbase + (pk_ok ? (unsigned)(pdir ? (T - 1 - tt) : tt) * TS : 0u), sentinel);
        asm volatile("s_waitcnt vmcnt(0)" ::: "memory");
    }
    __syncthreads();

    bool dead = false;
    const bool fast_rt = __builtin_amdgcn_readfirstlane((int)(cluster_on_one_xcd(a, c, p, tid, dead) && a.force_safe == 0)) != 0;
    auto run = [&](auto FASTC, auto SEC) {
    const bool fast = decltype(FASTC)::value < 0 ? fast_rt : decltype(FASTC)::value != 0;
    constexpr int SE = decltype(SEC)::value;
    for (int t = 0; t < T; ++t) {
        const int step_idx = t;
        PK_TRACE(0);
        f32x4 acc[G];
#pragma unroll
        for (int g = 0; g < G; ++g) acc[g] = f32x4{0.f, 0.f, 0.f, 0.f};
        unsigned char* At = smem + (t & 1) * ATILE;
        if (t > 0) {
            unsigned goff[NCH];
#pragma unroll
            for (int i = 0; i < NCH; ++i) goff[i] = cbase[i] + (unsigned)(t - 1) * cstep[i];
            for (int d = 0; d < a.poll_delay; ++d) __builtin_amdgcn_s_sleep(1);
            int retries = 0;
            dead = fast ? poll_to_lds<NCH, true>(rs, goff, clds, At, a.err, a.spin_limit, lane, dead, retries)
                        : poll_to_lds<NCH, false>(rs, goff, clds, At, a.err, a.spin_limit, lane, dead, retries);
            if (a.trace != nullptr && blockIdx.x == 0 && tid == 0) a.trace[(long)step_idx * 8 + 6] = (unsigned long long)retries;
        }
        PK_TRACE(1);
#pragma unroll
        for (int g = 0; g < G; ++g) patch_put_vec(patchP + g * 256, lane, pv[g]);
        if (t > 0) PK_BARRIER_LDS();
        else PK_LDS_ORDER();
        PK_TRACE(2);
        if (t > 0) {
#define PK_FO(E) flush_outputs(t - 1, E)
            PK_EDGE_DISPATCH_S(PK_FO);
        }
        if (t + 1 < T) {
#define PK_LP1(E) load_proj(t + 1, E)
            PK_EDGE_DISPATCH_S(PK_LP1);
        }
        if (a.self_fill && t + PK_R2_FILL_AHEAD < T) {
            const unsigned off = pbase + (pk_ok ? (unsigned)(pdir ? (T - 1 - (t + PK_R2_FILL_AHEAD)) : (t + PK_R2_FILL_AHEAD)) * TS : 0u);
            if (fast) pub_store<true>(rs, off, sentinel);
            else pub_store<false>(rs, off, sentinel);
        }
        const bool empty = TR && a.empty_step != 0;
        if (t > 0 && !empty) {
            const unsigned char* Ar = At + (lane & 15) * (LDA * 2) + kq * 16;
#pragma unroll
            for (int kk = 0; kk < KSTEPS; ++kk) {
                const bf16x8 af = *reinterpret_cast<const bf16x8*>(Ar + kk * 64);
#pragma unroll
                for (int g = 0; g < G; ++g) acc[g] = __builtin_amdgcn_mfma_f32_16x16x32_bf16(af, Bf[g][kk], acc[g], 0, 0, 0);
            }
        }
        PK_TRACE(3);
        float pre[G][4];
#pragma unroll
        for (int g = 0; g < G; ++g) patch_get_cd(patchP + g * 256, kq, lane, pre[g]);
        float hv[4], sv[NS][4];
#pragma unroll
        for (int r = 0; r < 4; ++r) {
            float pr[G];
#pragma unroll
            for (int g = 0; g < G; ++g) pr[g] = pre[g][r] * psc[g] + psh[g] + acc[g][r];
            float h, cc, s[NS];
            if (empty) {
                h = 0.25f;
                cc = 0.f;
#pragma unroll
                for (int k = 0; k < NS; ++k) s[k] = pr[0];
            } else {
                pk_cell_fwd<CELL>(act, pr, hprev[r], cprev[r], msk[r], h, cc, s);
            }
            h = rvf[r] != 0.f ? h : 0.f;
            cc = rvf[r] != 0.f ? cc : 0.f;
            hprev[r] = h;
            cprev[r] = cc;
            hv[r] = h;
#pragma unroll
            for (int k = 0; k < NS; ++k) sv[k][r] = s[k];
            if (!LN) patchB[(kq * 4 + r) * 16 + (lane & 15)] = to_bf_pub(h);
        }
        if (LN) {
            if (t == 0) {
                float ma[4], mb[4];
#pragma unroll
                for (int r = 0; r < 4; ++r) {
                    ma[r] = rvf[r] != 0.f ? hv[r] : 0.f;
                    mb[r] = 0.f;
                }
                unsigned po0[3];
                ls.poll_at(T, po0);
                dead = fast ? ln_row_allreduce<true>(rsx, ls.pub_at(T), po0, ma, mb, a.err, a.spin_limit, lane, dead)
                            : ln_row_allreduce<false>(rsx, ls.pub_at(T), po0, ma, mb, a.err, a.spin_limit, lane, dead);
#pragma unroll
                for (int r = 0; r < 4; ++r) piv[r] = ma[r] * invH;
            }
            float la[4], lb[4];
#pragma unroll
            for (int r = 0; r < 4; ++r) {
                const float d = hv[r] - piv[r];
                la[r] = rvf[r] != 0.f ? d : 0.f;
                lb[r] = rvf[r] != 0.f ? d * d : 0.f;
            }
            unsigned po[3];
            ls.poll_at(t, po);
            dead = fast ? ln_row_allreduce<true>(rsx, ls.pub_at(t), po, la, lb, a.err, a.spin_limit, lane, dead)
                        : ln_row_allreduce<false>(rsx, ls.pub_at(t), po, la, lb, a.err, a.spin_limit, lane, dead);
            patch_put_cd(patchL, kq, lane, hv);
            float mu4[4], ri4[4];
#pragma unroll
            for (int r = 0; r < 4; ++r) {
                const float md = la[r] * invH;
                const float mu = piv[r] + md;
                const float var = fmaxf((lb[r] - la[r] * md) * inv_nm1, 0.f);
                const float ri = 1.0f / (sqrtf(var) + a.ln_eps);
                const float hn = rvf[r] != 0.f ? gam * ((hv[r] - mu) * ri) + bet : 0.f;
                hv[r] = hn;
                hprev[r] = hn;
                piv[r] = mu;
                mu4[r] = mu;
                ri4[r] = ri;
                patchB[(kq * 4 + r) * 16 + (lane & 15)] = to_bf_pub(hn);
            }
            const int u3 = lane & 3;
            st_val[0] = u3 == 0 ? mu4[0] : u3 == 1 ? mu4[1] : u3 == 2 ? mu4[2] : mu4[3];
            st_val[1] = u3 == 0 ? ri4[0] : u3 == 1 ? ri4[1] : u3 == 2 ? ri4[2] : ri4[3];
        }
        PK_TRACE(4);
        PK_LDS_ORDER();
        {
            const u32x4 o = *reinterpret_cast<const u32x4*>(reinterpret_cast<const unsigned char*>(patchB) + (prow & 15) * 32 + phalf * 16);
            const unsigned off = pbase + (pk_ok ? (unsigned)(pdir ? (T - 1 - t) : t) * TS : 0u);
            if (fast) pub_store<true>(rs, off, o);
            else pub_store<false>(rs, off, o);
        }
        if (!NOSAVE || want_y) patch_put_cd(patchY, kq, lane, hv);
        if constexpr (!NOSAVE) {
#pragma unroll
            for (int k = 0; k < NS; ++k) patch_put_cd(patchS + k * 256, kq, lane, sv[k]);
        }
        PK_LDS_ORDER();
        PK_TRACE(5);
    }
    };
    if constexpr (LN) {
        run(BoolC<-1>(), BoolC<-1>());
    } else {
        PK_RUN_SPECIALISED(run, fast_rt);
    }
#define PK_FOL(E) flush_outputs(T - 1, E)
    PK_EDGE_DISPATCH(PK_FOL);
}

template <int CELL, int ACT, bool TR, bool LN = false>
__global__ __launch_bounds__(256, 1) void rec2_bwd_kernel(R2Args a) {
    const int act = ACT >= 0 ? ACT : a.act;
    constexpr int G = pk_cell_gates(CELL), NS = pk_cell_saved(CELL);
    constexpr bool LSTM = (CELL == PK_CELL_LSTM);
    constexpr int LDA = pk_r2_lda_bf16(G * KPAD);
    constexpr int ATILE = RMAX * LDA * 2;
    constexpr int NBUF = (2 * ATILE > 96 * 1024) ? 1 : 2;
    constexpr int NCH = (RMAX * G * (KPAD / 8) + 255) / 256;
    constexpr int NIN = NS + 2 + (LSTM ? 1 : 0) + (LN ? 1 : 0);
    constexpr int ILN = NS + 2 + (LSTM ? 1 : 0);
    constexpr int WAVE_LDS = (NIN + G) * 1024 + G * 512;
    constexpr int LDS_TRASH = NBUF * ATILE + 4 * WAVE_LDS;
    extern __shared__ __attribute__((aligned(16))) unsigned char smem[];

    const int tid = threadIdx.x, lane = tid & 63, wave = tid >> 6;
    const int c = blockIdx.x % a.C, p = blockIdx.x / a.C;
    const int H = a.H, Hp = a.Hp, B = a.B, T = a.T, GH = G * H;
    const unsigned TB = (unsigned)T * B;
    const int n_base = a.row0 + c * a.rpc;
    int nrows = a.R - n_base;
    nrows = nrows < a.rpc ? nrows : a.rpc;
    if (nrows <= 0) return;
    const int ubase = p * 64 + wave * 16;
    const int unit = ubase + (lane & 15);
    const bool unit_ok = unit < H;
    const int kq = lane >> 4;

    bf16x8 Bf[G][KSTEPS];
    {
        const unsigned szU = (unsigned)((size_t)G * H * H * 4);
        const __amdgpu_buffer_rsrc_t rsU = make_rsrc(a.U, szU);
#pragma unroll
        for (int g = 0; g < G; ++g)
#pragma unroll
            for (int kk = 0; kk < KSTEPS; ++kk) {
                unsigned raw[8];
#pragma unroll
                for (int e = 0; e < 8; ++e) {
                    const int j = kk * 32 + kq * 8 + e;
                    raw[e] = __builtin_amdgcn_raw_buffer_load_b32(rsU, (unit_ok && j < H) ? (unsigned)(((g * H + j) * H + unit) * 4) : szU, 0, 0);
                }
                bf16x8 f;
#pragma unroll
                for (int e = 0; e < 8; ++e) f[e] = (short)pk_f2bf(__uint_as_float(raw[e]));
                Bf[g][kk] = f;
            }
    }
    for (int i = tid; i < (LDS_TRASH + 16) / 4; i += 256) reinterpret_cast<unsigned*>(smem)[i] = 0u;

    const int CPR = Hp >> 3;
    const unsigned TS = (unsigned)B * a.Gpitch * 2u;
    const unsigned ndir = (unsigned)(a.R / B);
    const unsigned szGb = ndir * (unsigned)T * TS;
    unsigned cbase[NCH], cstep[NCH];
    int clds[NCH];
#pragma unroll
    for (int i = 0; i < NCH; ++i) {
        const int ci = tid + 256 * i;
        const bool ok = ci < nrows * G * CPR;
        const int row = ok ? ci / (G * CPR) : 0;
        const int rem = ok ? ci - row * (G * CPR) : 0;
        const int g = rem / CPR, col = rem - g * CPR;
        const int n = n_base + row;
        const int dir = n >= B ? 1 : 0, b = n - dir * B;
        cbase[i] = ok ? (unsigned)dir * (unsigned)T * TS + ((unsigned)b * a.Gpitch + g * Hp + col * 8) * 2u +
                            (unsigned)(dir ? 0 : (T - 1)) * TS
                      : szGb;
        cstep[i] = ok ? (dir ? TS : 0u - TS) : 0u;
        clds[i] = ok ? row * (LDA * 2) + (g * KPAD + col * 8) * 2 : LDS_TRASH;
    }
    float rvf[4], msk[4], dh_dir[4], dc_car[4];
#pragma unroll
    for (int r = 0; r < 4; ++r) {
        const int row = kq * 4 + r, n = n_base + row;
        const bool ok = row < nrows && unit_ok;
        rvf[r] = ok ? 1.f : 0.f;
        msk[r] = (a.mask != nullptr && ok) ? a.mask[(long)n * H + unit] : a.mask_scalar;
        dh_dir[r] = 0.f;
        dc_car[r] = 0.f;
// ... 417 lines not shown
    }
    if (cs != hipStreamCaptureStatusNone) PK_CHECK_HIP(hipMemsetAsync(g2_xcd_tab, 0xFF, XCD_TAB_BYTES, st));
    a.hs_gen = g;
    return 0;
}

int pk_rec2_run(hipStream_t st, R2Args& a, const Plan2& pl, int cell, bool backward, Rec2Kernel k, int threads, size_t lds,
                const char* who, const PkLnHost* ln, Rec2Help help_policy) {
    int rc = pk_rec2_ln_setup(st, a, pl, ln, backward);
    if (rc) return rc;
    rc = pk_grant_dynamic_lds((const void*)k, lds);
    if (rc) return rc;
    const bool proj = help_policy == REC2_HELP_PROJ;
    for (int l = 0; l < pl.launches; ++l) {
        a.row0 = l * pl.C * pl.rpc;
        a.ln_cg0 = l * pl.C;
        rc = pk_rec2_reset_handshake(st, a);
        if (rc) return rc;
        rc = pk_rec2_check_residency((const void*)k, threads, lds, pl.C * pl.Pn, who);
        if (rc) return rc;
        const int help = (ln || help_policy == REC2_HELP_NONE) ? 0 : pk_rec_helper_wanted(backward, pl.launches, cell) & (proj ? 1 : 7);
        if (help && (rc = pk_rec_helper_fork(st)) != 0) return rc;
        hipLaunchKernelGGL(k, dim3(pl.C * pl.Pn), dim3(threads), lds, st, a);
        PK_LAUNCH_CHECK();
        if (help && (rc = pk_rec_helper_launch(st, a, pl, pk_cell_gates(cell), proj ? 0 : pk_cell_saved(cell), backward, !proj, help)) != 0)
            return rc;
    }
    return backward ? pk_rec2_ln_finish(st, a, ln) : 0;
}

extern "C" int pk_rec_self_fill(int cell) {
    (void)cell;
    return 1;
}

extern "C" int pk_rec_plan_cus(int R, int H) {
    Plan2 pl;
    if (R <= 0 || H <= 0 || H > KPAD || pk_rec2_make_plan(R, H, pl) != 0) return 0;
    return pl.C * pl.Pn;
}

extern "C" void pk_persist2_set_mode(int force_safe) { g2_force_safe = force_safe ? 1 : 0; }
extern "C" void pk_persist2_set_poll_delay(int units) { g2_poll_delay = units; }
extern "C" void pk_persist2_set_trace(void* dev_buf) { g2_trace = (unsigned long long*)dev_buf; }
extern "C" void pk_persist2_set_empty_step(int on) { g2_empty_step = on; }
extern "C" unsigned pk_persist2_error_count(void) { return g2_err_host ? *g2_err_host : 0u; }
extern "C" void pk_persist2_error_reset(void) {
    if (g2_err_host) *g2_err_host = 0u;
}

template <int CELL>
Rec2Kernel pick_fwd(int act) {
    return pk_rec2_pick_act(act, rec2_fwd_kernel<CELL, PK_ACT_RELU, false>, rec2_fwd_kernel<CELL, PK_ACT_TANH, false>,
                            rec2_fwd_kernel<CELL, -1, false>);
}
template <int CELL>
Rec2Kernel pick_fwd_nosave(int act) {
    return pk_rec2_pick_act(act, rec2_fwd_kernel<CELL, PK_ACT_RELU, false, false, true>,
                            rec2_fwd_kernel<CELL, PK_ACT_TANH, false, false, true>, rec2_fwd_kernel<CELL, -1, false, false, true>);
}
template <int CELL>
Rec2Kernel pick_bwd(int act) {
    return pk_rec2_pick_act(act, rec2_bwd_kernel<CELL, PK_ACT_RELU, false>, rec2_bwd_kernel<CELL, PK_ACT_TANH, false>,
                            rec2_bwd_kernel<CELL, -1, false>);
}
inline bool traced(int cell, int act) { return g2_trace != nullptr && cell == PK_CELL_LIGRU && act == PK_ACT_RELU; }
inline Rec2Kernel pick_fwd_ln(int cell) {
    return cell == PK_CELL_LIGRU ? rec2_fwd_kernel<PK_CELL_LIGRU, -1, false, true>
         : cell == PK_CELL_RNN ? rec2_fwd_kernel<PK_CELL_RNN, -1, false, true> : rec2_fwd_kernel<PK_CELL_LSTM, -1, false, true>;
}
inline Rec2Kernel pick_bwd_ln(int cell) {
    return cell == PK_CELL_LIGRU ? rec2_bwd_kernel<PK_CELL_LIGRU, -1, false, true>
         : cell == PK_CELL_RNN ? rec2_bwd_kernel<PK_CELL_RNN, -1, false, true> : rec2_bwd_kernel<PK_CELL_LSTM, -1, false, true>;
}
inline Rec2Kernel pick_fwd(int cell, int act) {
    if (traced(cell, act)) return rec2_fwd_kernel<PK_CELL_LIGRU, PK_ACT_RELU, true>;
    return cell == PK_CELL_LIGRU ? pick_fwd<PK_CELL_LIGRU>(act) : cell == PK_CELL_RNN ? pick_fwd<PK_CELL_RNN>(act) : pick_fwd<PK_CELL_LSTM>(act);
}
inline Rec2Kernel pick_bwd(int cell, int act) {
    if (traced(cell, act)) return rec2_bwd_kernel<PK_CELL_LIGRU, PK_ACT_RELU, true>;
    return cell == PK_CELL_LIGRU ? pick_bwd<PK_CELL_LIGRU>(act) : cell == PK_CELL_RNN ? pick_bwd<PK_CELL_RNN>(act) : pick_bwd<PK_CELL_LSTM>(act);
}

static int rec_fwd_bf16_impl(void* stream, int cell, int act, int T, int B, int bidir, int H, const float* P,
                             const float* pscale, const float* pshift, const float* U, const float* mask,
                             float mask_scalar, float* Y, float* S, uint16_t* Yb, int64_t y_pitch, int prefilled,
                             const PkLnHost* ln) {
    const char* who = "pk_rec_fwd_bf16";
    int rc = pk_rec2_check(who, 1, cell, T, B, bidir, H);
    if (rc) return rc;
    PK_REQUIRE(S != nullptr || (ln == nullptr && !traced(cell, act)), "pk_rec_fwd_bf16: S may be null only without per-step LayerNorm");
    PK_REQUIRE(Y != nullptr || S == nullptr, "pk_rec_fwd_bf16: Y may be null only together with S");
    hipStream_t st = pk_stream(stream);
    const int ndir = 1 + bidir, Hp = (H + 7) & ~7;
    PK_REQUIRE(y_pitch >= (int64_t)ndir * Hp && (y_pitch % 8) == 0 && ((uintptr_t)Yb & 15) == 0,
               "pk_rec_fwd_bf16: Yb pitch must be a multiple of 8 and hold %d x %d elements", ndir, Hp);
    PK_REQUIRE((double)T * B * y_pitch * 2.0 < 4.0e9, "pk_rec_fwd_bf16: exchange buffer exceeds the 4 GB buffer-descriptor range");
    R2Args a{};
    Plan2 pl;
    rc = pk_rec2_prepare_fwd(a, pl, pk_rec2_make_plan, cell, act, T, B, bidir, H, y_pitch, P, pscale, pshift, U, mask, mask_scalar, Y, S);
    if (rc) return rc;
    a.Yb = (unsigned short*)Yb;
    a.self_fill = prefilled == 2 ? 1 : 0;
    if (prefilled != 1 && !a.self_fill) PK_CHECK_HIP(hipMemsetAsync(Yb, 0xFF, (size_t)T * B * y_pitch * 2, st));
    size_t lds;
    if (!ln && cell == PK_CELL_LSTM && pk_rec2l_enabled()) {
        const Rec2Kernel k8 = pk_rec2l_kernel(a, act, false, &lds);
        return pk_rec2_run(st, a, pl, cell, false, k8, 512, lds, "pk_rec_*_bf16 (LSTM, eight waves)", ln, REC2_HELP_FULL);
    }
    if (!ln && pk_rec3_covers(cell, 0)) {
        const Rec2Kernel k3 = pk_rec3_kernel(cell, act, false, traced(cell, act), &lds);
        return pk_rec2_run(st, a, pl, cell, false, k3, 256, lds, who, ln, REC2_HELP_FULL);
    }
    lds = 2 * (size_t)RMAX * pk_r2_lda_bf16(KPAD) * 2 + 4 * ((size_t)(pk_cell_gates(cell) + 1 + pk_cell_saved(cell) + (ln ? 1 : 0)) * 1024 + 512) + 16;
    const bool nosave = S == nullptr;
    const Rec2Kernel k = ln ? pick_fwd_ln(cell)
                       : nosave ? (cell == PK_CELL_LIGRU ? pick_fwd_nosave<PK_CELL_LIGRU>(act) : cell == PK_CELL_RNN ? pick_fwd_nosave<PK_CELL_RNN>(act)
                                                                                                                      : pick_fwd_nosave<PK_CELL_LSTM>(act))
                                : pick_fwd(cell, act);
    return pk_rec2_run(st, a, pl, cell, false, k, 256, lds, who, ln, REC2_HELP_FULL);
}
extern "C" int pk_rec_fwd_bf16(void* stream, int cell, int act, int T, int B, int bidir, int H, const float* P,
                               const float* pscale, const float* pshift, const float* U, const float* mask,
                               float mask_scalar, float* Y, float* S, uint16_t* Yb, int64_t y_pitch, int prefilled) {
    return rec_fwd_bf16_impl(stream, cell, act, T, B, bidir, H, P, pscale, pshift, U, mask, mask_scalar, Y, S, Yb, y_pitch,
                             prefilled, nullptr);
}
extern "C" int pk_rec_fwd_bf16_ln(void* stream, int cell, int act, int T, int B, int bidir, int H, const float* P,
                                  const float* pscale, const float* pshift, const float* U, const float* mask,
                                  float mask_scalar, const float* ln_gamma, const float* ln_beta, float ln_eps, float* Y,
                                  float* S, float* LNS, uint16_t* Yb, int64_t y_pitch, int prefilled, float* lnwork) {
    PK_REQUIRE(ln_gamma && ln_beta && LNS && lnwork, "pk_rec_fwd_bf16_ln: null LayerNorm argument");
    const PkLnHost ln = {ln_gamma, ln_beta, ln_eps, LNS, lnwork, nullptr, nullptr};
    return rec_fwd_bf16_impl(stream, cell, act, T, B, bidir, H, P, pscale, pshift, U, mask, mask_scalar, Y, S, Yb, y_pitch,
                             prefilled, &ln);
}

static int rec_bwd_bf16_impl(void* stream, int cell, int act, int T, int B, int bidir, int H, const float* U,
                             const float* mask, float mask_scalar, const float* Y, const float* S, const float* dY,
                             float* dP2, uint16_t* dGb, int64_t g_pitch, int prefilled, const PkLnHost* ln) {
    const char* who = "pk_rec_bwd_bf16";
    int rc = pk_rec2_check(who, 1, cell, T, B, bidir, H);
    if (rc) return rc;
    hipStream_t st = pk_stream(stream);
    const int ndir = 1 + bidir, Hp = (H + 7) & ~7, G = pk_cell_gates(cell);
    PK_REQUIRE(g_pitch >= (int64_t)G * Hp && (g_pitch % 8) == 0 && ((uintptr_t)dGb & 15) == 0,
               "pk_rec_bwd_bf16: dGb pitch must be a multiple of 8 and hold %d x %d elements", G, Hp);
    PK_REQUIRE((double)ndir * T * B * g_pitch * 2.0 < 4.0e9, "pk_rec_bwd_bf16: exchange buffer exceeds the 4 GB buffer-descriptor range");
    R2Args a{};
    Plan2 pl;
    rc = pk_rec2_prepare_bwd(a, pl, pk_rec2_make_plan, cell, act, T, B, bidir, H, g_pitch, U, mask, mask_scalar, Y, S, dY, dP2);
    if (rc) return rc;
    a.dGb = (unsigned short*)dGb;
    a.self_fill = prefilled == 2 ? 1 : 0;
    if (prefilled != 1 && !a.self_fill) PK_CHECK_HIP(hipMemsetAsync(dGb, 0xFF, (size_t)ndir * T * B * g_pitch * 2, st));
    size_t lds;
    if (!ln && cell == PK_CELL_LSTM && pk_rec2l_enabled()) {
        const Rec2Kernel k8 = pk_rec2l_kernel(a, act, true, &lds);
        return pk_rec2_run(st, a, pl, cell, true, k8, 512, lds, "pk_rec_*_bf16 (LSTM, eight waves)", ln, REC2_HELP_FULL);
    }
    if (!ln && pk_rec3_covers(cell, 1)) {
        const Rec2Kernel k3 = pk_rec3_kernel(cell, act, true, traced(cell, act), &lds);
        return pk_rec2_run(st, a, pl, cell, true, k3, 256, lds, who, ln, REC2_HELP_FULL);
    }
    const size_t atile = (size_t)RMAX * pk_r2_lda_bf16(G * KPAD) * 2;
    const int nin = pk_cell_saved(cell) + 2 + (cell == PK_CELL_LSTM ? 1 : 0) + (ln ? 1 : 0);
    lds = (2 * atile > 96 * 1024 ? 1 : 2) * atile + 4 * ((size_t)(nin + G) * 1024 + (size_t)G * 512) + 16;
    return pk_rec2_run(st, a, pl, cell, true, ln ? pick_bwd_ln(cell) : pick_bwd(cell, act), 256, lds, who, ln, REC2_HELP_FULL);
}
extern "C" int pk_rec_bwd_bf16(void* stream, int cell, int act, int T, int B, int bidir, int H, const float* U,
                               const float* mask, float mask_scalar, const float* Y, const float* S, const float* dY,
                               float* dP2, uint16_t* dGb, int64_t g_pitch, int prefilled) {
    return rec_bwd_bf16_impl(stream, cell, act, T, B, bidir, H, U, mask, mask_scalar, Y, S, dY, dP2, dGb, g_pitch, prefilled,
                             nullptr);
}
extern "C" int pk_rec_bwd_bf16_ln(void* stream, int cell, int act, int T, int B, int bidir, int H, const float* U,
                                  const float* mask, float mask_scalar, const float* ln_gamma, float ln_eps, const float* Y,
                                  const float* S, const float* LNS, const float* dY, float* dP2, uint16_t* dGb,
                                  int64_t g_pitch, int prefilled, float* lnwork, float* dln_gamma, float* dln_beta) {
    PK_REQUIRE(ln_gamma && LNS && lnwork && dln_gamma && dln_beta, "pk_rec_bwd_bf16_ln: null LayerNorm argument");
    const PkLnHost ln = {ln_gamma, nullptr, ln_eps, const_cast<float*>(LNS), lnwork, dln_gamma, dln_beta};
    return rec_bwd_bf16_impl(stream, cell, act, T, B, bidir, H, U, mask, mask_scalar, Y, S, dY, dP2, dGb, g_pitch, prefilled,
                             &ln);
}
```

### pytorch-kaldi_amd/functional.py

```python
import ctypes
import os
import weakref
from typing import NamedTuple

import torch

from . import _lib

PREC = {"fp32": 0, "bf16": 1}
ACT = {"linear": 0, "relu": 1, "tanh": 2, "sigmoid": 3, "leaky_relu": 4, "elu": 5}
CELL = {"liGRU": 0, "RNN": 1, "LSTM": 2, "GRU": 3, "minimalGRU": 4}
REC_STEPWISE, REC_PERSISTENT = 0, 1


class _Settings:

    def __init__(self):
        self.precision = os.environ.get("PK_PRECISION", "fp32")
        self.rec_algo = os.environ.get("PK_REC_ALGO", "auto")
        self.mask_rng = os.environ.get("PK_MASK_RNG", "device")
        assert self.mask_rng in ("reference", "reference_host", "device"), self.mask_rng
        self.wgrad_side = _lib.experiment("wgrad_side", "1") != "0"
        self.self_fill = _lib.experiment("rec_self_fill", "1") != "0"
        self.side_late = _lib.experiment("side_late", "1") != "0"
        self.side_cus = _lib.experiment("side_cus", "0") != "0"
        self.fused_cost = _lib.experiment("fused_cost", "1") != "0"
        assert self.precision in PREC, self.precision
        assert self.rec_algo in ("auto", "stepwise", "persistent"), self.rec_algo


settings = _Settings()


def set_precision(p):
    assert p in PREC, p
    settings.precision = p


def set_mask_rng(m):
    assert m in ("reference", "reference_host", "device"), m
    settings.mask_rng = m


def set_rec_algo(a):
    assert a in ("auto", "stepwise", "persistent"), a
    settings.rec_algo = a


class _Kinks:
    queue = None
    report = None


def set_forced_kinks(patterns):
    _Kinks.queue = None if patterns is None else list(patterns)
    _Kinks.report = []
    return _Kinks.report


_KINK_SLOT = {"liGRU": 1, "RNN": 0, "GRU": 2, "minimalGRU": 1}


def _force_kinks(S, cell, T, B, ndir, H):
    if _Kinks.queue is None:
        return
    if cell not in _KINK_SLOT:
        raise _lib.PkError("kink-forced mode covers the cells whose candidate goes through act(a): %s" % cell)
    k = _Kinks.queue.pop(0).to(S.device)
    NS = S.shape[2] // H
    flipped, worst = 0, 0.0
    for d in range(ndir):
        a = S[d].view(T, B, NS, H)[:, :, _KINK_SLOT[cell], :]
        kd = k[:, d * B:(d + 1) * B]
        if d == 1:
            kd = torch.flip(kd, [0])
        diff = (a > 0) != kd
        n = int(diff.sum())
        if n:
            flipped += n
            worst = max(worst, float(a[diff].abs().max()))
        mag = a.abs().clamp_min(1e-30)
        a.copy_(torch.where(kd, mag, -mag))
    _Kinks.report.append((flipped, ndir * T * B * H, worst))


class _Drops:
    queue = None


def set_forced_dropout(masks):
    _Drops.queue = None if masks is None else list(masks)


class _Decisions:
    relu = None
    pool = None
    report = None


def set_forced_decisions(relu=None, pool=None):
    _Decisions.relu = None if relu is None else list(relu)
    _Decisions.pool = None if pool is None else list(pool)
    _Decisions.report = []
    return _Decisions.report


class _RefRng:
    dev = None
    base = None
# ... 178 lines not shown
    lib = _lib.load()
    ws = None
    if splitk == 1 and a_cs == 1 and (prec or settings.precision) == "fp32":
        splitk = _small_m_splitk(M, N, K)
    if splitk > 1:
        ws = torch.empty(splitk * M * N, device=C.device, dtype=torch.float32)
    rc = lib.pk_gemm(_stream(), PREC[prec or settings.precision], M, N, K, alpha, _p(A), a_rs, a_cs, _p(B), b_rs, b_cs,
                     beta, _p(C), ldc, _p(bias), splitk, _p(ws))
    _lib.check(rc, "pk_gemm")
    return C


def _tiles(M, N):
    return ((M + 127) // 128) * ((N + 127) // 128)


def _tiles_bf(M, N):
    return (M, N)


def _up(n, m):
    return (n + m - 1) // m * m


def weight_bf16(w):
    sh = getattr(w, "_pk_shadow", None)
    if sh is not None:
        view, version, alive, flat_version = sh
        if alive() is not None:
            owner = getattr(w, "_pk_owner", None)
            owner = owner() if owner is not None else None
            fv = owner.flat._version if owner is not None else flat_version
            if w._version == version and fv == flat_version:
                return view
            cvt_bf16(w.detach(), out=view)
            w._pk_shadow = (view, w._version, alive, fv)
            return view
    owner = getattr(w, "_pk_owner", None)
    owner = owner() if owner is not None else None
    if owner is not None and w.is_contiguous():
        owner.want_shadow(w)
    return cvt_bf16(w.contiguous())


def cvt_bf16(x2, nseg=1, seglen=None, segpad=None, out=None):
    lib = _lib.load()
    rows, cols = x2.shape
    if seglen is None:
        nseg, seglen = 1, cols
    if segpad is None:
        segpad = _up(seglen, 8)
    assert nseg * seglen == cols and x2.stride(1) == 1
    pitch = _up(nseg * segpad, 64)
    if out is None:
        out = torch.empty(rows, pitch, device=x2.device, dtype=torch.bfloat16)
    assert tuple(out.shape) == (rows, pitch) and out.dtype == torch.bfloat16 and out.is_contiguous()
    _lib.check(lib.pk_cvt_bf16(_stream(), _p(x2), x2.stride(0), rows, nseg, seglen, segpad, _p(out), pitch),
               "pk_cvt_bf16")
    return out


_SMALL_SPLITK = _lib.experiment("small_splitk", "1") != "0"


def gemm_bf16(M, N, K, A, lda, a_kc, B, ldb, b_kc, C, ldc, alpha=1.0, beta=0.0, bias=None, splitk=1):
    lib = _lib.load()
    ws = None
    if splitk == 1 and a_kc and M <= 128 and _SMALL_SPLITK:
        splitk = int(lib.pk_gemm_bf16_small_splitk(M, N, K))
    if splitk > 1:
        ws = torch.empty(splitk * M * N, device=C.device, dtype=torch.float32)

    def ptr(t):
        if isinstance(t, tuple):
            return ctypes.c_void_p(t[0].data_ptr() + 2 * t[1])
        return ctypes.c_void_p(t.data_ptr())

    rc = lib.pk_gemm_bf16(_stream(), M, N, K, alpha, ptr(A), lda, int(a_kc), ptr(B), ldb, int(b_kc), beta, _p(C), ldc,
                          _p(bias), splitk, _p(ws))
    _lib.check(rc, "pk_gemm_bf16")
    return C


def gemm_bf16_bn_stats(M, N, K, A, lda, a_kc, B, ldb, b_kc, C, ldc, bias=None, gates=None):
    lib = _lib.load()

    def done(mean, var):
        return (mean, var) if gates is None else (mean, var) + tuple(bn_finalize_gates(mean, var, *gates))

    if _lib.experiment("gemm_stats", "1") == "0":
        gemm_bf16(M, N, K, A, lda, a_kc, B, ldb, b_kc, C, ldc, bias=bias)
        return done(*bn_stats(C if ldc == N else C.as_strided((M, N), (ldc, 1))))
    stats = torch.empty(int(lib.pk_gemm_bf16_stats_floats(M, N)), device=C.device, dtype=torch.float32)
    rb = ctypes.c_int(0)
    rc = lib.pk_gemm_bf16_stats(_stream(), M, N, K, 1.0, _p(A), lda, int(a_kc), _p(B), ldb, int(b_kc), _p(C), ldc, _p(bias),
                                _p(stats), ctypes.byref(rb))
    _lib.check(rc, "pk_gemm_bf16_stats")
    if rb.value == 0:
        return done(*bn_stats(C if ldc == N else C.as_strided((M, N), (ldc, 1))))
    mean, var = torch.empty(N, device=C.device), torch.empty(N, device=C.device)
    if gates is not None:
        gamma, beta, eps, H, rms, rvs, nbs, momentum, count = gates
        G = len(rms)
        scale, shift = torch.empty_like(mean), torch.empty_like(mean)
        arr = lambda ts: (ctypes.c_void_p * G)(*[t.data_ptr() for t in ts])
        _lib.check(lib.pk_bn_stats_merge_finalize_gates(_stream(), _p(stats), rb.value, G, H, _p(mean), _p(var), _p(gamma),
                                                        _p(beta), eps, _p(scale), _p(shift), arr(rms), arr(rvs), arr(nbs),
                                                        momentum, float(count)), "pk_bn_stats_merge_finalize_gates")
        return mean, var, scale, shift
    _lib.check(lib.pk_bn_stats_merge(_stream(), _p(stats), rb.value, N, _p(mean), _p(var)), "pk_bn_stats_merge")
    return mean, var


def _splitk_bf(out_tiles, K):
    M, N = out_tiles
    return int(_lib.load().pk_gemm_bf16_auto_splitk_cus(int(M), int(N), int(K), int(_SideCus.cus)))


class _SideCus:
    cus = 0


def _sized_for(cus, fn):
    def run():
        old, _SideCus.cus = _SideCus.cus, cus
        try:
            fn()
        finally:
            _SideCus.cus = old
    return run


def bf16_mode():
    return settings.precision == "bf16"



class _Side:
    stream = None
    pending = False
    listener = None
    deferred = []


def set_side_listener(fn):
    _Side.listener = fn


def side_targets_ok(params):
    return bf16_mode() and side_targets_any_ok(params)


def side_targets_any_ok(params):
    if not bf16_mode() and _lib.experiment("f32_wgrad_side", "1") == "0":
        return False
    return (settings.wgrad_side and params is not None and len(params) > 0
            and all(getattr(q, "_pk_flat", False) and q.grad is not None and q.requires_grad for q in params))


class accumulating_backward:
    depth = 0

    def __enter__(self):
        accumulating_backward.depth += 1
        return self

    def __exit__(self, *exc):
        accumulating_backward.depth -= 1
        return False


def direct_grads_ok(params):
    return (accumulating_backward.depth > 0 and _Side.listener is None and _lib.experiment("direct_grads", "1") != "0"
            and torch.is_grad_enabled() is False and side_targets_ok(params))


def direct_affine_ok(params):
    return (accumulating_backward.depth > 0 and _Side.listener is None and _lib.experiment("direct_grads", "1") != "0"
            and torch.is_grad_enabled() and side_targets_ok(params))


_DEBUG_SKIP_SIDE = _lib.experiment("debug_skip_side", "0") == "1"


def _make_side_stream():
    return torch.cuda.Stream()


def side_launch(fn, keep, params=None, defer=False):
    if defer and settings.side_late and _lib.experiment("side_defer_heads", "1") != "0":
        _Side.deferred.append((fn, keep, params))
        _Side.pending = True
        return
    flush_deferred_side()
    main = torch.cuda.current_stream()
    if _Side.stream is None:
        _Side.stream = _make_side_stream()
    side = _Side.stream
    side.wait_stream(main)
    with torch.cuda.stream(side):
        if not _DEBUG_SKIP_SIDE:
            fn()
    for t in keep:
        if t is not None:
            t.record_stream(side)
    _Side.pending = True
    if _Side.listener is not None and params:
        _Side.listener(params)


def flush_deferred_side():
    if _Side.deferred:
        items, _Side.deferred = _Side.deferred, []
        for fn, keep, params in items:
            side_launch(fn, keep, params)


def join_side():
    flush_deferred_side()
    if _Side.pending:
        if _Side.stream is not None:
            torch.cuda.current_stream().wait_stream(_Side.stream)
        _Side.pending = False


def adjacent_view(ts):
    if not ts:
        return None
    base = ts[0]
    if len(ts) == 1:
        return base.detach() if base.is_contiguous() else None
    ptr, rows = base.data_ptr(), 0
    for t in ts:
        if (not t.is_contiguous() or t.dtype != base.dtype or t.shape[1:] != base.shape[1:] or t.data_ptr() != ptr
                or t.untyped_storage().data_ptr() != base.untyped_storage().data_ptr()):
            return None
        ptr += t.numel() * t.element_size()
        rows += t.shape[0]
    if base.data_ptr() % 16 != 0:
        return None
    return base.detach().as_strided((rows,) + tuple(base.shape[1:]), base.stride())


def _accumulate_rows(params, rows):
    with torch.no_grad():
        gview = adjacent_view([q.grad for q in params])
        whole = adjacent_view(list(rows)) if gview is not None else None
        if whole is not None and whole.shape == gview.shape:
            gview.add_(whole)
            return
        for q, r in zip(params, rows):
            q.grad.add_(r)

_XB_LAST = None


def _cvt_bf16_shared(x2):
    global _XB_LAST
    key = (x2.data_ptr(), tuple(x2.shape), tuple(x2.stride()), x2._version)
    if _XB_LAST is not None and _XB_LAST[1] == key and x2.numel() >= (1 << 20):
        return _XB_LAST[2]
    xb = cvt_bf16(x2)
    _XB_LAST = (x2, key, xb) if x2.numel() >= (1 << 20) else None
    return xb


class LinearFn(torch.autograd.Function):
    @staticmethod
    def forward(ctx, x, weight, bias):
        _need_gpu(x, weight, bias)
        x2 = _rows2d(x)
        weight = weight.contiguous()
        M, K = x2.shape
        N = weight.shape[0]
        y = _new(M, N, like=x2)
        ctx.bf = bf16_mode()
        if ctx.bf:
            xb, wb = _cvt_bf16_shared(x2), cvt_bf16(weight)
            gemm_bf16(M, N, K, xb, xb.shape[1], 1, wb, wb.shape[1], 1, y, N, bias=bias)
            ctx.save_for_backward(xb, wb)
        else:
            gemm(M, N, K, x2, x2.stride(0), 1, weight, 1, K, y, N, bias=bias)
            ctx.save_for_backward(x2, weight)
        ctx.dims = (M, N, K)
        ctx.has_bias = bias is not None
        ctx.in_shape = x.shape
        ctx.wparam = weight if isinstance(weight, torch.nn.Parameter) else None
        return y.view(*x.shape[:-1], N)

    @staticmethod
    def backward(ctx, dy):
        x2, weight = ctx.saved_tensors
        M, N, K = ctx.dims
        if (not ctx.bf and dy.dim() == 2 and dy.stride(1) == 1 and dy.stride(0) % 4 == 0 and dy.stride(0) >= N
                and dy.data_ptr() % 16 == 0):
            dy2 = dy
        else:
            dy2 = _rows2d(dy.contiguous())
        ldy = dy2.stride(0)
        dx = dw = db = None
        if ctx.bf:
            dx, dw = _linear_bwd_bf16(ctx, cvt_bf16(dy2), x2, weight, dy2)
            if ctx.has_bias and ctx.needs_input_grad[2]:
                db = colsum(dy2)
            return dx, dw, db
        if ctx.needs_input_grad[0]:
            dx = _new(M, K, like=dy2)
            gemm(M, K, N, dy2, ldy, 1, weight, K, 1, dx, K)
            dx = dx.view(ctx.in_shape)
        if ctx.needs_input_grad[1]:
            wp = ctx.wparam
            sk = _splitk(_tiles(N, K), M)
            if M >= 4096 and wp is not None and wp.is_contiguous() and side_targets_any_ok([wp]):
                side_launch(lambda: gemm(N, K, M, dy2, 1, ldy, x2, x2.stride(0), 1, wp.grad, K, beta=1.0, splitk=sk), (dy2, x2), [wp],
                            defer=True)
            else:
                dw = _new(N, K, like=dy2)
                gemm(N, K, M, dy2, 1, ldy, x2, x2.stride(0), 1, dw, K, splitk=sk)
        if ctx.has_bias and ctx.needs_input_grad[2]:
            db = colsum(dy2)
        return dx, dw, db


class _DxShare:
    on = _lib.experiment("head_dx_share", "1") != "0"
    epoch = 0
    epoch_fwd = 0
    table = {}
    alias = None
    cat = {}
    wcat = {}


def _cat_register(key, ctx_id, N, wb, M):
    if not (_DxShare.on and _lib.experiment("head_dx_cat", "1") != "0" and M >= 4096):
# ... 73 lines not shown


def _dx_share_key(x):
    return (x.data_ptr(), x._version, tuple(x.shape), tuple(x.stride()))


def _linear_bwd_bf16(ctx, dyb, xb, wb, like, cat=None):
    M, N, K = ctx.dims
    xseg = getattr(ctx, "xseg", None)
    Kx = K if xseg is None else xseg[0] * xseg[2]
    dx = dw = None
    ldy = dyb.stride(0)
    if ctx.needs_input_grad[0] and cat is not None:
        c = cat[0]
        c["done"].add(id(ctx))
        c["dims"], c["in_shape"] = (M, K), ctx.in_shape
    elif ctx.needs_input_grad[0]:
        key = getattr(ctx, "dx_share", None)
        shared = _DxShare.table.get(key) if key is not None else None
        if shared is not None and shared[0] == _DxShare.epoch and id(ctx) not in shared[2]:
            gemm_bf16(M, K, N, dyb, ldy, 1, wb, wb.shape[1], 0, shared[1], K, beta=1.0)
            shared[2].add(id(ctx))
            dx = None
        else:
            dx = _new(M, K, like=like)
            gemm_bf16(M, K, N, dyb, ldy, 1, wb, wb.shape[1], 0, dx, K)
            if key is not None:
                _DxShare.table[key] = (_DxShare.epoch, dx, {id(ctx)})
            dx = dx.view(ctx.in_shape)
    if ctx.needs_input_grad[1]:
        wp = ctx.wparam
        side = M >= 4096 and wp is not None and wp.is_contiguous() and side_targets_ok([wp])
        sk = _splitk_bf(_tiles_bf(N, Kx), M)
        if xseg is None:
            if side:
                side_launch(lambda: gemm_bf16(N, K, M, dyb, ldy, 0, xb, xb.shape[1], 0, wp.grad, K, beta=1.0,
                                              splitk=sk), (dyb, xb), [wp])
            elif M <= 512 and wp is not None and wp.is_contiguous() and direct_grads_ok([wp]):
                gemm_bf16(N, K, M, dyb, ldy, 0, xb, xb.shape[1], 0, wp.grad, K, beta=1.0, splitk=sk)
            else:
                dw = _new(N, K, like=like)
                gemm_bf16(N, K, M, dyb, ldy, 0, xb, xb.shape[1], 0, dw, K, splitk=sk)
        else:
            nseg, seglen, segpad = xseg
            dwp = _new(N, Kx, like=like)

            def run():
                gemm_bf16(N, Kx, M, dyb, ldy, 0, xb, xb.shape[1], 0, dwp, Kx, splitk=sk)
                if side:
                    with torch.no_grad():
                        for s_ in range(nseg):
                            wp.grad[:, s_ * seglen:(s_ + 1) * seglen].add_(dwp[:, s_ * segpad:s_ * segpad + seglen])

            if side:
                side_launch(run, (dyb, xb, dwp), [wp], defer=True)
            else:
                run()
                dw = torch.cat([dwp[:, s_ * segpad:s_ * segpad + seglen] for s_ in range(nseg)], 1)
    return dx, dw


def input_twin(x2):
    tw = getattr(x2, "_pk_twin", None)
    if tw is None:
        return None
    xb, xseg, version = tw
    if x2._version != version or x2.dim() != 2 or xb.shape[0] != x2.shape[0] or xseg[0] * xseg[1] != x2.shape[1]:
        return None
    return xb, xseg


class LinearLogSoftmaxFn(torch.autograd.Function):

    @staticmethod
    def forward(ctx, x, weight, bias, xb, wb, wb_plain, xseg):
        _need_gpu(x, weight, bias)
        lib = _lib.load()
        x2 = _rows2d(x)
        M, K = x2.shape
        N = weight.shape[0]
        ldz = _up(N, 32)
        z = torch.empty(M, ldz, device=x2.device, dtype=torch.float32)
        Kx = K if xseg is None else xseg[0] * xseg[2]
        gemm_bf16(M, N, Kx, xb, xb.shape[1], 1, wb, wb.shape[1], 1, z, ldz, bias=bias)
        y = _new(M, N, like=x2)
        amax = torch.empty(M, device=x2.device, dtype=torch.int32)
        _lib.check(lib.pk_logsoftmax_fwd_ld_argmax(_stream(), _p(z), ldz, M, N, _p(y), _p(amax)), "pk_logsoftmax_fwd_ld_argmax")
        ctx.save_for_backward(xb, wb_plain, y)
        ctx.xseg = xseg
        ctx.dims = (M, N, K)
        ctx.has_bias = bias is not None
        ctx.in_shape = x.shape
        ctx.wparam = weight if isinstance(weight, torch.nn.Parameter) else None
        ctx.mark_non_differentiable(amax)
        return y, amax

    @staticmethod
    def backward(ctx, dy, _damax=None):
        lib = _lib.load()
        xb, wb, y = ctx.saved_tensors
        M, N, K = ctx.dims
        dy2 = dy.contiguous()
        ldb = _up(N, 64)
        dzb = torch.empty(M, ldb, device=y.device, dtype=torch.bfloat16)
        part = _new(int(lib.pk_logsoftmax_bwd_bf16_partial_floats(M, N)), like=y)
        db = _new(N, like=y)
        _lib.check(lib.pk_logsoftmax_bwd_bf16(_stream(), _p(dy2), _p(y), M, N, _p(dzb), ldb, _p(part), _p(db)),
                   "pk_logsoftmax_bwd_bf16")
        dx, dw = _linear_bwd_bf16(ctx, dzb, xb, wb, y)
        return dx, dw, (db if ctx.has_bias and ctx.needs_input_grad[2] else None), None, None, None, None


def linear_log_softmax_ok(x, weight):
    return bf16_mode() and x.dim() == 2 and weight.shape[0] <= 8192


def linear_log_softmax(x, weight, bias=None):
    with torch.no_grad():
        w = weight.contiguous()
        x2 = _rows2d(x)
        tw = input_twin(x2)
        wb_plain = weight_bf16(weight)
        if tw is None:
            xb, xseg, wb = _cvt_bf16_shared(x2), None, wb_plain
        elif tw[1][0] == 1 and tw[0].shape[1] == wb_plain.shape[1]:
            xb, xseg, wb = tw[0], None, wb_plain
        else:
            xb, xseg = tw
            wb = cvt_bf16(w, *xseg)
            assert wb.shape[1] == xb.shape[1]
    _DxShare.epoch += 1
    _DxShare.table.clear()
    _DxShare.epoch_fwd = _DxShare.epoch
    xs = _head_input(x)
    y, amax = LinearLogSoftmaxFn.apply(xs, weight if weight.is_contiguous() else w, bias, xb, wb, wb_plain, xseg)
    y._pk_head = (xs, weight, bias, xb, wb_plain, xseg, y._version, amax)
    return y


class HeadNllFn(torch.autograd.Function):

    @staticmethod
    def forward(ctx, x, weight, bias, y, lab, xb, wb, xseg, ignore_index, amax=None):
        lib = _lib.load()
        ctx.set_materialize_grads(False)
        ctx.xseg = xseg
        M, N = y.shape
        lab = lab.contiguous()
        out4 = _new(4, like=y)
        loss = torch.empty((), device=y.device, dtype=torch.float32)
        part = _new(int(lib.pk_nll_err_partial_floats(M)), like=y)
        if amax is not None and _lib.experiment("head_argmax", "1") != "0":
            _lib.check(lib.pk_nll_err_fwd_argmax(_stream(), _p(y), _p(lab), _p(amax), int(ignore_index), M, N, _p(part), _p(out4),
                                                 _p(loss), _p(label_check_counter(y.device))), "pk_nll_err_fwd_argmax")
        else:
            _lib.check(lib.pk_nll_err_fwd(_stream(), _p(y), _p(lab), int(ignore_index), M, N, _p(part), _p(out4), _p(loss),
                                          _p(label_check_counter(y.device))), "pk_nll_err_fwd")
        ctx.save_for_backward(xb, wb, y, lab, out4)
        ctx.dx_share = _dx_share_key(x) if (_DxShare.on and x.is_contiguous()) else None
        if ctx.dx_share is not None and x.requires_grad:
            _cat_register(ctx.dx_share, id(ctx), N, wb, M)
        ctx.dims = (M, N, x.shape[-1])
        ctx.has_bias = bias is not None
        ctx.in_shape = x.shape
        ctx.wparam = weight if isinstance(weight, torch.nn.Parameter) else None
        ctx.ignore_index = int(ignore_index)
        ctx.mark_non_differentiable(out4)
        return loss, out4

    @staticmethod
    def backward(ctx, dloss, _d4):
        lib = _lib.load()
        if dloss is None:
            return (None,) * 10
        xb, wb, y, lab, out4 = ctx.saved_tensors
        M, N, K = ctx.dims
        dl = dloss.contiguous().float()
        ldb = _up(N, 64)
        part = _new(int(lib.pk_logsoftmax_bwd_bf16_partial_floats(M, N)), like=y)
        db = _new(N, like=y)
        cnt = ctypes.c_void_p(out4.data_ptr() + 8)
        cat = _cat_slot(ctx, M) if ctx.needs_input_grad[0] else None
        if cat is not None:
            dz, off = cat[0]["dz"], cat[1]["off"]
            dzb = dz[:, off:off + ldb]
            _lib.check(lib.pk_nll_logsoftmax_bwd_bf16_p(_stream(), _p(y), _p(lab), _p(dl), cnt, ctx.ignore_index, M, N,
                                                        ctypes.c_void_p(dzb.data_ptr()), ldb, dz.shape[1], _p(part), _p(db)),
                       "pk_nll_logsoftmax_bwd_bf16_p")
        else:
            dzb = torch.empty(M, ldb, device=y.device, dtype=torch.bfloat16)
            _lib.check(lib.pk_nll_logsoftmax_bwd_bf16(_stream(), _p(y), _p(lab), _p(dl), cnt, ctx.ignore_index, M, N, _p(dzb),
                                                      ldb, _p(part), _p(db)), "pk_nll_logsoftmax_bwd_bf16")
        dx, dw = _linear_bwd_bf16(ctx, dzb, xb, wb, y, cat)
        return dx, dw, (db if ctx.has_bias and ctx.needs_input_grad[2] else None), None, None, None, None, None, None, None


def linear(x, weight, bias=None):
    return LinearFn.apply(x, weight, bias)


def colsum(g, g2=None):
    lib = _lib.load()
    M, N = g.shape
    out = _new(N, like=g)
    part = _new(int(lib.pk_bn_partial_floats(M, N)), like=g)
    _lib.check(lib.pk_colsum(_stream(), _p(g), _p(g2), g.stride(0), M, N, _p(part), _p(out)), "pk_colsum")
    return out


class _LabelCheck:
    bad = {}


# ... 700 lines not shown
    if want == "stepwise":
        return REC_STEPWISE
    return REC_PERSISTENT if ok else REC_STEPWISE


def perf_path_ok(cell, H, use_ln, use_bn, training):
    if not bf16_mode() or settings.rec_algo == "stepwise":
        return False
    if cell not in ("liGRU", "RNN", "LSTM", "GRU", "minimalGRU") or H > 576 or use_ln:
        return False
    return training or not use_bn or not torch.is_grad_enabled()


class RecRoute(NamedTuple):
    perf: bool
    algo: int
    family: str


_REC_BF16 = {"bf16": "pk_rec_%s_bf16", "bf16_ln": "pk_rec_%s_bf16_ln", "2p_bf16": "pk_rec2p_%s_bf16", "2p_bf16_ln": "pk_rec2p_%s_bf16_ln"}


def rec_route(cell, H, use_ln, use_bn, training):
    two_phase = cell in ("GRU", "minimalGRU")
    if perf_path_ok(cell, H, use_ln, use_bn, training):
        return RecRoute(True, REC_PERSISTENT, "2p_bf16" if two_phase else "bf16")
    algo = choose_rec_algo(cell, H, use_ln)
    if not bf16_mode() or algo != REC_PERSISTENT:
        return RecRoute(False, algo, "generic")
    if use_ln:
        return RecRoute(False, algo, "2p_bf16_ln" if two_phase else "bf16_ln")
    return RecRoute(False, algo, "2p_bf16" if two_phase else "bf16")


def rec_keep_y(routes, i, grad_enabled):
    return bool(grad_enabled or i == len(routes) - 1 or not routes[i].perf or not routes[i + 1].perf)


class RecCfg(NamedTuple):
    cell: str
    act: str
    H: int
    bidir: bool
    use_bn: bool
    training: bool
    eps: float
    momentum: float
    mask_scalar: float
    xseg: tuple = None
    wparams: list = None
    uparams: list = None
    side_w: bool = False
    side_u: bool = False
    bn_bufs: tuple = None
    affine: tuple = None
    keep_y: bool = True
    route: RecRoute = None


_RecGeom = NamedTuple("_RecGeom", [(n, int) for n in "T B D G NS ndir TB GH Hp y_pitch g_pitch".split()])


def _rec_geom(lib, cfg, shape):
    T, B, D = shape
    G, NS = lib.pk_rec_num_gates(CELL[cfg.cell]), lib.pk_rec_num_saved(CELL[cfg.cell])
    ndir, Hp = 2 if cfg.bidir else 1, _up(cfg.H, 8)
    return _RecGeom(T, B, D, G, NS, ndir, T * B, G * cfg.H, Hp, _up(ndir * Hp, 64), _up(G * Hp, 64))


def _proj_scale_shift(cfg, P, mean, var, gamma, beta, running_mean, running_var, bcat):
    if not cfg.use_bn:
        pscale = torch.ones(P.shape[1], device=P.device)
        return None, None, pscale, bcat.contiguous() if bcat is not None else torch.zeros(P.shape[1], device=P.device)
    if cfg.training:
        return (mean, var) + bn_finalize(mean, var, gamma, beta, cfg.eps, running_mean, running_var, cfg.momentum,
                                         (2 if cfg.bidir else 1) * P.shape[0])
    return (running_mean, running_var) + bn_finalize(running_mean, running_var, gamma, beta, cfg.eps)


def _accumulate_gate_rows(params, d, G, H):
    _accumulate_rows(params, [d[g * H:(g + 1) * H] for g in range(G)])


def _rec_bf16_fwd(lib, cfg, geom, P, pscale, pshift, Ucat, mask, Y, S, Yb, prefilled, Xb=None, ln=None):
    name = _REC_BF16[cfg.route.family] % "fwd"
    a = [_stream(), CELL[cfg.cell], ACT[cfg.act], geom.T, geom.B, int(cfg.bidir), cfg.H, _p(P), _p(pscale), _p(pshift),
         _p(Ucat), _p(mask), float(cfg.mask_scalar)]
    if ln is not None:
        a += [_p(ln[0]), _p(ln[1]), LN_EPS]
    a += [_p(Y), _p(S)] + ([_p(ln[2])] if ln is not None else []) + [_p(Yb)]
    if cfg.route.family.startswith("2p"):
        a.append(_p(Xb))
    a += [geom.y_pitch, prefilled] + ([_p(ln[3])] if ln is not None else [])
    _lib.check(getattr(lib, name)(*a), name)


def _rec_bf16_bwd(lib, cfg, geom, Ucat, mask, Y, S, dY, dP2, dGb, prefilled, ln=None):
    name = _REC_BF16[cfg.route.family] % "bwd"
    a = [_stream(), CELL[cfg.cell], ACT[cfg.act], geom.T, geom.B, int(cfg.bidir), cfg.H, _p(Ucat), _p(mask),
         float(cfg.mask_scalar)]
    if ln is not None:
        a += [_p(ln[0]), LN_EPS]
    a += [_p(Y), _p(S)] + ([_p(ln[1])] if ln is not None else []) + [_p(dY)]
    if not cfg.route.family.startswith("2p"):
        a.append(_p(dP2))
    a += [_p(dGb), geom.g_pitch, prefilled] + ([_p(x) for x in ln[2:]] if ln is not None else [])
    _lib.check(getattr(lib, name)(*a), name)


_DU_SPLITK = 16


def _gemm_km_f32(M, N, K, A, a_ld, bflat, b_off, b_ld, oflat, overwrite, realign=True):
    Bm = bflat[b_off:]
    shift = (Bm.data_ptr() % 16) // 4
    if not realign or shift == 0 or b_ld % 4 != 0 or a_ld % 4 != 0 or b_off < shift or _lib.experiment("f32_du_shift", "1") == "0":
        gemm(M, N, K, A, 1, a_ld, Bm, b_ld, 1, oflat, N, beta=0.0 if overwrite else 1.0, splitk=_DU_SPLITK, prec="fp32")
        return
    Nw = N + shift
    tmp = torch.empty(M, Nw, device=oflat.device, dtype=torch.float32)
    gemm(M, Nw, K, A, 1, a_ld, bflat[b_off - shift:], b_ld, 1, tmp, Nw, beta=0.0, splitk=_DU_SPLITK, prec="fp32")
    o2 = oflat[:M * N].view(M, N)
    with torch.no_grad():
        if overwrite:
            o2.copy_(tmp[:, shift:])
        else:
            o2.add_(tmp[:, shift:])


def _deferred_dU_f32(cell, T, B, ndir, H, G, NS, Y, S, dP2, out, accumulate):
    TB, GH, YH = T * B, G * H, ndir * H
    two_phase = cell in ("GRU", "minimalGRU")
    Gh = G - 1 if two_phase else G
    Kh = (T - 1) * B
    dflat, yflat, sflat, oflat = dP2.reshape(-1), Y.reshape(-1), S.reshape(-1), out.reshape(-1)
    first = not accumulate
    realign = cell in ("liGRU", "RNN") or _lib.experiment("f32_du_shift", "") == "all"
    if Kh == 0 and not accumulate:
        out[:Gh * H].zero_()
    for d in range(ndir if Kh > 0 else 0):
        A = dflat[(d * TB + (0 if d else B)) * GH:]
        _gemm_km_f32(Gh * H, H, Kh, A, GH, yflat, (B if d else 0) * YH + d * H, YH, oflat, first, realign)
        first = False
    if two_phase:
        slot = 3 if cell == "GRU" else 2
        for d in range(ndir):
            A = dflat[d * TB * GH + Gh * H:]
            _gemm_km_f32(H, H, TB, A, GH, sflat, d * TB * NS * H + slot * H, NS * H, oflat[Gh * H * H:], not (accumulate or d),
                         realign)


def _deferred_dU_bf16(lib, cell, T, B, ndir, H, G, Y, S, dP2, dU, Yb=None, dGb=None, Xb=None):
    TB, GH = T * B, G * H
    two_phase = cell in ("GRU", "minimalGRU")
    Gh = G - 1 if two_phase else G
    Kh = (T - 1) * B
    Hp = _up(H, 8)
    if Yb is None:
        Yb = cvt_bf16(Y.view(TB, ndir * H), ndir, H, Hp)
    Yp = Yb.shape[1]
    if dGb is None:
        dGb = cvt_bf16(dP2.view(ndir * TB, GH), G, H, Hp)
    Gp = dGb.shape[1]
    Mp = Gh * H if Hp == H else Gh * Hp
    out = dU[:Gh * H] if Hp == H else _new(Mp, H, like=dU)
    if Kh == 0:
        dU[:Gh * H].zero_()
    else:
        for d in range(ndir):
            a_off = (d * TB + (0 if d else B)) * Gp
            b_off = (B if d else 0) * Yp + d * Hp
            gemm_bf16(Mp, H, Kh, (dGb, a_off), Gp, 0, (Yb, b_off), Yp, 0, out, H, beta=0.0 if d == 0 else 1.0,
                      splitk=_splitk_bf(_tiles_bf(Mp, H), Kh))
        if Hp != H:
            for g in range(Gh):
                dU[g * H:(g + 1) * H].copy_(out[g * Hp:g * Hp + H])
    if two_phase:
# ... 145 lines not shown
                                                 _p(dPraw), ldp), "pk_affine_act_fwd")
        else:
            if g2 is not None:
                _lib.check(lib.pk_add(_stream(), _p(g1), _p(g2), TB * GH, _p(dPraw)), "pk_add")
            else:
                dPraw = g1
            if ctx.has_bias:
                dbias = colsum(dPraw)
        dx = dW = None
        dW = _new(GH, D, like=dY)
        if bf:
            xb, Wb = x2, Wcat
            dPb = cvt_bf16(dPraw)
            if ctx.needs_input_grad[0]:
                dx = _new(TB, D, like=dY)
                gemm_bf16(TB, D, GH, dPb, dPb.shape[1], 1, Wb, Wb.shape[1], 0, dx, D)
                dx = dx.view(T, B, D)
            gemm_bf16(GH, D, TB, dPb, dPb.shape[1], 0, xb, xb.shape[1], 0, dW, D, splitk=_splitk_bf(_tiles_bf(GH, D), TB))
            return dx, dW, dbias, dU, dgamma, dbeta, None, None, None, dlg, dlb, None
        if ctx.needs_input_grad[0]:
            dx = _new(TB, D, like=dY)
            gemm(TB, D, GH, dPraw, ldp, 1, Wcat, D, 1, dx, D)
            dx = dx.view(T, B, D)
        side_w = cfg.side_w and side_targets_any_ok(cfg.wparams)
        if cfg.side_w and not side_w:
            raise _lib.PkError("recurrent layer: the flat gradient buffer of the input weights is gone between forward and backward")
        if cfg.side_u:
            side_launch(do_dU_f32, (Y, S, dP2, dU), cfg.uparams)

        def do_dW_f32():
            gview = adjacent_view([q.grad for q in cfg.wparams])
            sk = _splitk(_tiles(GH, D), TB)
            if gview is not None:
                gemm(GH, D, TB, dPraw, 1, ldp, x2, x2.stride(0), 1, gview, D, beta=1.0, splitk=sk)
            else:
                gemm(GH, D, TB, dPraw, 1, ldp, x2, x2.stride(0), 1, dW, D, splitk=sk)
                _accumulate_gate_rows(cfg.wparams, dW, G, H)

        if side_w:
            side_launch(do_dW_f32, (dPraw, x2, dW), cfg.wparams)
        else:
            gemm(GH, D, TB, dPraw, 1, ldp, x2, x2.stride(0), 1, dW, D, splitk=_splitk(_tiles(GH, D), TB))
        return (dx, None if side_w else dW, dbias, None if cfg.side_u else dU, dgamma, dbeta, None, None, None, dlg, dlb, None)


class _Prefill:
    stream = None

    def __init__(self):
        self.done = 0

    def start(self, *bufs):
        if not settings.wgrad_side:
            return
        main = torch.cuda.current_stream()
        if _Prefill.stream is None:
            _Prefill.stream = torch.cuda.Stream()
        st = _Prefill.stream
        st.wait_stream(main)
        with torch.cuda.stream(st):
            for b in bufs:
                if b is not None:
                    b.view(torch.int16).fill_(-1)
        for b in bufs:
            if b is not None:
                b.record_stream(st)
        self.done = 1

    def wait(self):
        if self.done:
            torch.cuda.current_stream().wait_stream(_Prefill.stream)


class RecLayerPerfFn(torch.autograd.Function):

    @staticmethod
    def forward(ctx, x, xb_in, Wcat, bcat, Ucat, gamma, beta, running_mean, running_var, mask, cfg, edge=None):
        ctx.set_materialize_grads(False)
        _need_gpu(x, Wcat, bcat, Ucat, gamma, beta, mask)
        lib = _lib.load()
        geom = _rec_geom(lib, cfg, x.shape)
        H, bn_train = cfg.H, cfg.use_bn and cfg.training
        T, B, D, ndir, TB, GH = geom.T, geom.B, geom.D, geom.ndir, geom.TB, geom.GH
        Wcat, Ucat = Wcat.contiguous(), Ucat.contiguous()
        if xb_in is None:
            xseg = None
            xb, Wb, K = cvt_bf16(_rows2d(x)), cvt_bf16(Wcat), D
        else:
            xseg = cfg.xseg
            nseg, seglen, segpad = xseg
            assert nseg * seglen == D and xb_in.shape[0] == TB
            xb, Wb, K = xb_in, cvt_bf16(Wcat, nseg, seglen, segpad), nseg * segpad
            assert Wb.shape[1] == xb.shape[1]
        Yb = torch.empty(TB, geom.y_pitch, device=x.device, dtype=torch.bfloat16)
        self_fill = settings.self_fill and lib.pk_rec_self_fill(CELL[cfg.cell]) == 1
        dGb = None
        if any(ctx.needs_input_grad) and not self_fill:
            dGb = torch.empty(ndir * TB, geom.g_pitch, device=x.device, dtype=torch.bfloat16)
        Xb = torch.empty_like(Yb) if cfg.route.family.startswith("2p") else None
        fill = _Prefill()
        if not self_fill:
            fill.start(Yb, Xb, dGb)
        P = _new(TB, GH, like=Wcat)
        mean = var = pscale = pshift = None
        if bn_train and cfg.bn_bufs is not None:
            mean, var, pscale, pshift = gemm_bf16_bn_stats(TB, GH, K, xb, xb.shape[1], 1, Wb, Wb.shape[1], 1, P, GH, gates=(
                gamma, beta, cfg.eps, H, cfg.bn_bufs[0], cfg.bn_bufs[1], cfg.bn_bufs[2], cfg.momentum, ndir * TB))
        elif bn_train:
            mean, var = gemm_bf16_bn_stats(TB, GH, K, xb, xb.shape[1], 1, Wb, Wb.shape[1], 1, P, GH)
        else:
            gemm_bf16(TB, GH, K, xb, xb.shape[1], 1, Wb, Wb.shape[1], 1, P, GH)
        if pscale is None:
            mean, var, pscale, pshift = _proj_scale_shift(cfg, P, mean, var, gamma, beta, running_mean, running_var, bcat)
        infer = not any(ctx.needs_input_grad) and _Kinks.queue is None and _lib.experiment("fwd_nosave", "1") != "0"
        Y = _new(T, B, ndir * H, like=Wcat)
        S = None if infer else _new(ndir, TB, geom.NS * H, like=Wcat)
        Yarg = Y if (cfg.keep_y or not infer) else None
        _lib.raise_if_persist_failed()
        fill.wait()
        _rec_bf16_fwd(lib, cfg, geom, P, pscale, pshift, Ucat, mask, Yarg, S, Yb, 2 if self_fill else fill.done, Xb)
        if S is not None:
            _force_kinks(S, cfg.cell, T, B, ndir, H)
        ctx.self_fill = self_fill
        ctx.dGb = dGb if fill.done else None
        ctx.Xb = Xb
        ctx.save_for_backward(xb, Wb, Wcat, Ucat, P, mean, var, gamma, mask, Y, S, Yb)
        ctx.cfg, ctx.geom, ctx.xseg = cfg, geom, xseg
        ctx.has_bias = bcat is not None
        if bn_train:
            ctx.mark_non_differentiable(mean, var, Yb)
            return Y, mean, var, Yb
        ctx.mark_non_differentiable(Yb)
        return Y, None, None, Yb

    @staticmethod
    def backward(ctx, dY, _dm, _dv, _dyb):
        if dY is None:
            return (None,) * 12
        lib = _lib.load()
        xb, Wb, Wcat, Ucat, P, mean, var, gamma, mask, Y, S, Yb = ctx.saved_tensors
        cfg, geom, xseg = ctx.cfg, ctx.geom, ctx.xseg
        cell, H, use_bn = cfg.cell, cfg.H, cfg.use_bn
        if use_bn and not cfg.training:
            raise _lib.PkError("perf-mode recurrent layer: backward through frozen BatchNorm statistics is not covered")
        T, B, D, G, ndir, TB, GH, Gp = geom.T, geom.B, geom.D, geom.G, geom.ndir, geom.TB, geom.GH, geom.g_pitch
        dY = dY.contiguous()
        dGb, prefilled = ctx.dGb, 1
        ctx.dGb = None
        if dGb is None:
            dGb = torch.empty(ndir * TB, Gp, device=dY.device, dtype=torch.bfloat16)
            prefilled = 2 if ctx.self_fill else 0
        flush_deferred_side()
        _rec_bf16_bwd(lib, cfg, geom, Ucat, mask, Y, S, dY, None, dGb, prefilled)
        side_u, side_w = cfg.side_u, cfg.side_w
        Xb = ctx.Xb
        ctx.Xb = None
        dU = _new(GH, H, like=dY)

        def do_dU():
            _deferred_dU_bf16(lib, cell, T, B, ndir, H, G, Y, S, None, dU, Yb, dGb, Xb)
            if side_u:
                _accumulate_gate_rows(cfg.uparams, dU, G, H)

        late = settings.side_late and bool(ctx.needs_input_grad[0])
        if side_u and not late:
            side_launch(do_dU, (Y, S, Yb, dGb, Xb, dU), cfg.uparams)
        elif not side_u:
            do_dU()
        dPb = torch.empty(TB, _up(GH, 64), device=dY.device, dtype=torch.bfloat16)
        part = _new(int(lib.pk_bn_partial_floats(TB, GH)), like=dY)
        sum_g = _new(GH, like=dY)
        sum_gx = _new(GH, like=dY) if use_bn else None
        g1 = ctypes.c_void_p(dGb.data_ptr() + 2 * TB * Gp) if cfg.bidir else None
        acc_g = acc_b = None
        if use_bn and cfg.affine is not None:
            acc_g = adjacent_view([q.grad for q in cfg.affine[0]])
            acc_b = adjacent_view([q.grad for q in cfg.affine[1]])
            if acc_g is None or acc_b is None:
                raise _lib.PkError("perf-mode recurrent layer: the BatchNorm gradients left the flat buffer between forward "
                                   "and backward (optim.FlatParams.zero_grad() re-aliases them)")
        rc = lib.pk_bn_bwd_bf16(_stream(), _p(dGb), g1, Gp, G, H, _p(P), GH, TB, _p(mean) if use_bn else None,
                                _p(var) if use_bn else None, cfg.eps, _p(gamma) if use_bn else None, float(TB), _p(part),
                                _p(sum_g), _p(sum_gx), _p(dPb), dPb.shape[1], _p(acc_b), _p(acc_g))
        _lib.check(rc, "pk_bn_bwd_bf16")
        dgamma = dbeta = dbias = None
        if use_bn and acc_g is None:
            dgamma, dbeta = sum_gx, sum_g
        elif not use_bn and ctx.has_bias:
            dbias = sum_g
        Kx = D if xseg is None else xseg[0] * xseg[2]
        dWp = _new(GH, Kx, like=dY)
        dW = None

        def do_dW():
            nonlocal dW
            gview = adjacent_view([q.grad for q in cfg.wparams]) if side_w else None
            sk = _splitk_bf(_tiles_bf(GH, Kx), TB)
            if gview is not None and xseg is None:
                gemm_bf16(GH, Kx, TB, dPb, dPb.shape[1], 0, xb, xb.shape[1], 0, gview, Kx, beta=1.0, splitk=sk)
                return
            gemm_bf16(GH, Kx, TB, dPb, dPb.shape[1], 0, xb, xb.shape[1], 0, dWp, Kx, splitk=sk)
            if gview is not None:
                nseg, seglen, segpad = xseg
# ... 108 lines not shown
```

Measured before the change: 3.870 million.

## Overlap next layer's projection GEMM with recurrent forward via time-windowed slices

Splits the persistent recurrent forward kernel into time windows and records an event after each one. The next layer's input-projection GEMM (with fused BN stats or logsoftmax) then runs on a side stream over the row tiles already finished, capped to the CUs the recurrence leaves free. A walking GEMM kernel and row-window entry points are added to support this. The aim is to hide the serial recurrence tail behind projection work, at the cost of extra launches, cross-stream synchronisation and restarting the recurrence at each window boundary.

After: 3.818 million. -1.3%, worse.

```diff
diff --git a/include/pk_amd.h b/include/pk_amd.h
--- a/include/pk_amd.h
+++ b/include/pk_amd.h
@@ -46,6 +46,12 @@
 int pk_gemm_bf16_stats(void* stream, int M, int N, int K, float alpha, const uint16_t* A, int64_t lda, int a_kc,
                        const uint16_t* B, int64_t ldb, int b_kc, float* C, int64_t ldc, const float* bias, float* stats,
                        int* row_blocks);
+int pk_gemm_bf16_rows_ok(int M, int N);
+int pk_gemm_bf16_rows(void* stream, int M, int N, int K, float alpha, const uint16_t* A, int64_t lda, const uint16_t* B,
+                      int64_t ldb, float* C, int64_t ldc, const float* bias, int row0, int rows, int max_workgroups);
+int pk_gemm_bf16_stats_rows(void* stream, int M, int N, int K, float alpha, const uint16_t* A, int64_t lda,
+                            const uint16_t* B, int64_t ldb, float* C, int64_t ldc, const float* bias, float* stats, int row0,
+                            int rows, int max_workgroups);
 int pk_cvt_bf16(void* stream, const float* src, int64_t ld_src, int64_t rows, int nseg, int seglen, int segpad,
                 uint16_t* dst, int64_t ld_dst);
 
@@ -145,6 +151,10 @@
 int pk_rec_fwd_bf16(void* stream, int cell, int act, int T, int B, int bidir, int H, const float* P,
                     const float* pscale, const float* pshift, const float* U, const float* mask, float mask_scalar,
                     float* Y, float* S, uint16_t* Yb, int64_t y_pitch, int prefilled);
+int pk_rec_fwd_bf16_window_ok(int cell);
+int pk_rec_fwd_bf16_window(void* stream, int cell, int act, int T, int B, int bidir, int H, const float* P,
+                           const float* pscale, const float* pshift, const float* U, const float* mask, float mask_scalar,
+                           float* Y, float* S, uint16_t* Yb, int64_t y_pitch, int prefilled, int t_begin, int t_end);
 int pk_rec_bwd_bf16(void* stream, int cell, int act, int T, int B, int bidir, int H, const float* U, const float* mask,
                     float mask_scalar, const float* Y, const float* S, const float* dY, float* dP2, uint16_t* dGb,
                     int64_t g_pitch, int prefilled);
diff --git a/pytorch-kaldi_amd/_lib.py b/pytorch-kaldi_amd/_lib.py
--- a/pytorch-kaldi_amd/_lib.py
+++ b/pytorch-kaldi_amd/_lib.py
@@ -27,6 +27,10 @@
                              c_int, P]),
     "pk_gemm_bf16_stats_floats": (c_int64, [c_int, c_int]),
     "pk_gemm_bf16_stats": (c_int, [P, c_int, c_int, c_int, c_float, P, c_int64, c_int, P, c_int64, c_int, P, c_int64, P, P, P]),
+    "pk_gemm_bf16_rows_ok": (c_int, [c_int, c_int]),
+    "pk_gemm_bf16_rows": (c_int, [P, c_int, c_int, c_int, c_float, P, c_int64, P, c_int64, P, c_int64, P, c_int, c_int, c_int]),
+    "pk_gemm_bf16_stats_rows": (c_int, [P, c_int, c_int, c_int, c_float, P, c_int64, P, c_int64, P, c_int64, P, P, c_int, c_int,
+                                        c_int]),
     "pk_bn_stats_merge": (c_int, [P, P, c_int, c_int64, P, P]),
     "pk_cvt_bf16": (c_int, [P, P, c_int64, c_int64, c_int, c_int, c_int, P, c_int64]),
     "pk_bn_partial_floats": (c_int64, [c_int64, c_int64]),
@@ -84,6 +88,9 @@
     "pk_rec_plan_cus": (c_int, [c_int, c_int]),
     "pk_gemm_bf16_auto_splitk_cus": (c_int, [c_int, c_int, c_int, c_int]),
     "pk_rec_fwd_bf16": (c_int, [P, c_int, c_int, c_int, c_int, c_int, c_int, P, P, P, P, P, c_float, P, P, P, c_int64, c_int]),
+    "pk_rec_fwd_bf16_window_ok": (c_int, [c_int]),
+    "pk_rec_fwd_bf16_window": (c_int, [P, c_int, c_int, c_int, c_int, c_int, c_int, P, P, P, P, P, c_float, P, P, P, c_int64, c_int,
+                                       c_int, c_int]),
     "pk_rec_bwd_bf16": (c_int, [P, c_int, c_int, c_int, c_int, c_int, c_int, P, P, c_float, P, P, P, P, P, c_int64, c_int]),
     "pk_rec2p_fwd_bf16_ln": (c_int, [P, c_int, c_int, c_int, c_int, c_int, c_int, P, P, P, P, P, c_float, P, P, c_float, P, P, P,
                                      P, P, c_int64, c_int, P]),
diff --git a/pytorch-kaldi_amd/csrc/pk_gemm_bf16.hip b/pytorch-kaldi_amd/csrc/pk_gemm_bf16.hip
--- a/pytorch-kaldi_amd/csrc/pk_gemm_bf16.hip
+++ b/pytorch-kaldi_amd/csrc/pk_gemm_bf16.hip
@@ -23,6 +23,7 @@
     int items, per_xcd;
     const unsigned short* zeros;
     float* stats;
+    int tm0;
 };
 
 __device__ unsigned short g_zero_page[64];
@@ -888,14 +889,11 @@
 #define PK_VMCNT(n) asm volatile("s_waitcnt vmcnt(" #n ")" ::: "memory")
 
 template <bool A_KC, bool B_KC>
-__global__ __launch_bounds__(512, 1) void gemm_bf16_256_kernel(BArgs p) {
-    extern __shared__ __attribute__((aligned(1024))) unsigned char smem[];
+__device__ __forceinline__ void gemm_bf16_256_item(const BArgs& p, const int item, unsigned char* const smem) {
     const int tid = threadIdx.x, lane = tid & 63, wave = tid >> 6;
     const int wm = wave >> 2, wn = wave & 3;
-    const int item = (blockIdx.x & 7) * p.per_xcd + (blockIdx.x >> 3);
-    if (item >= p.items) return;
     const int tn = item % p.tiles_n;
-    const int tm = (item / p.tiles_n) % p.tiles_m;
+    const int tm = p.tm0 + (item / p.tiles_n) % p.tiles_m;
     const int split = item / (p.tiles_n * p.tiles_m);
     const int m0 = tm * 256, n0 = tn * 256;
     const int kbeg = split * p.k_per_split;
@@ -1041,6 +1039,23 @@
                                n0 + bh * 128 + wn * 32 + j * 16 + (lane >> 4) * 4, split, vec_ok);
 }
 
+template <bool A_KC, bool B_KC>
+__global__ __launch_bounds__(512, 1) void gemm_bf16_256_kernel(BArgs p) {
+    extern __shared__ __attribute__((aligned(1024))) unsigned char smem[];
+    const int item = (blockIdx.x & 7) * p.per_xcd + (blockIdx.x >> 3);
+    if (item >= p.items) return;
+    gemm_bf16_256_item<A_KC, B_KC>(p, item, smem);
+}
+template <bool A_KC, bool B_KC>
+__global__ __launch_bounds__(512, 1) void gemm_bf16_256_walk_kernel(BArgs p) {
+    extern __shared__ __attribute__((aligned(1024))) unsigned char smem[];
+    for (int bx = blockIdx.x; bx < p.per_xcd * 8; bx += gridDim.x) {
+        const int item = (bx & 7) * p.per_xcd + (bx >> 3);
+        if (item < p.items) gemm_bf16_256_item<A_KC, B_KC>(p, item, smem);
+        __syncthreads();
+    }
+}
+
 __global__ void splitk_reduce_bf_kernel(const float* __restrict__ ws, int splitk, int M, int N, float alpha, float beta,
                                         const float* __restrict__ bias, float* __restrict__ C, long ldc) {
     const long total = (long)M * N;
@@ -1169,8 +1184,10 @@
 
 static int gemm_bf16_impl(void* stream, int M, int N, int K, float alpha, const uint16_t* A, int64_t lda, int a_kc,
                           const uint16_t* B, int64_t ldb, int b_kc, float beta, float* C, int64_t ldc, const float* bias,
-                          int splitk, float* workspace, float* stats) {
+                          int splitk, float* workspace, float* stats, int row0 = 0, int rows = -1, int max_workgroups = 0) {
     if (M <= 0 || N <= 0) return 0;
+    const bool win = rows >= 0;
+    if (win && rows == 0) return 0;
     PK_REQUIRE(K >= 0, "pk_gemm_bf16: negative K");
     PK_REQUIRE((lda % 8) == 0 && (ldb % 8) == 0 && ((uintptr_t)A & 15) == 0 && ((uintptr_t)B & 15) == 0,
                "pk_gemm_bf16: operands need 16-byte aligned bases and pitches that are multiples of 8 elements");
@@ -1189,6 +1206,14 @@
     PK_REQUIRE(stats == nullptr || (tile == 256 && a_kc && b_kc && splitk <= 1 && beta == 0.f), "pk_gemm_bf16_stats: internal: shape not covered");
     p.tiles_m = (M + tile - 1) / tile;
     p.tiles_n = (N + tile - 1) / tile;
+    p.tm0 = 0;
+    if (win) {
+        PK_REQUIRE(tile == 256 && a_kc && b_kc && splitk <= 1 && beta == 0.f, "pk_gemm_bf16_rows: shape not on the 256-tile");
+        PK_REQUIRE(row0 >= 0 && (row0 % 256) == 0 && (long)row0 + rows <= M && ((row0 + rows) % 256 == 0 || row0 + rows == M),
+                   "pk_gemm_bf16_rows: window [%d, %d) of %d rows is not a set of whole 256-row tiles", row0, row0 + rows, M);
+        p.tm0 = row0 / 256;
+        p.tiles_m = (row0 + rows + 255) / 256 - p.tm0;
+    }
     static void* zp = nullptr;
     if (zp == nullptr) PK_CHECK_HIP(hipGetSymbolAddress(&zp, HIP_SYMBOL(g_zero_page)));
     p.zeros = (const unsigned short*)zp;
@@ -1214,7 +1239,7 @@
             const char* e = pk_experiment("gemm_skinny");
             skinny_on = (e && e[0] == '0') ? 0 : 1;
         }
-        if (skinny_on && !g_gemm_tile_forced && a_kc && M <= TM && splitk > 1 && p.k_per_split <= SK_TILES * TK && stats == nullptr) {
+        if (!win && skinny_on && !g_gemm_tile_forced && a_kc && M <= TM && splitk > 1 && p.k_per_split <= SK_TILES * TK && stats == nullptr) {
             static bool attr_done = false;
             if (!attr_done) {
                 PK_CHECK_HIP(hipFuncSetAttribute((const void*)gemm_bf16sk_kernel<true>, hipFuncAttributeMaxDynamicSharedMemorySize, SK_TILES * SSTAGE));
@@ -1233,14 +1258,14 @@
             PK_LAUNCH_CHECK();
             return 0;
         }
-        if (skinny_on && !g_gemm_tile_forced && !a_kc && !b_kc && splitk == 1 && K <= 512 && stats == nullptr &&
+        if (!win && skinny_on && !g_gemm_tile_forced && !a_kc && !b_kc && splitk == 1 && K <= 512 && stats == nullptr &&
             (long)((M + TM - 1) / TM) * ((N + TN - 1) / TN) <= 192 && M >= 64 && N >= 64) {
             const dim3 tgrid((unsigned)((N + 63) / 64), (unsigned)((M + 63) / 64));
             hipLaunchKernelGGL(gemm_bf16_t64_kernel, tgrid, dim3(256), T64_TILES * T64_STAGE, st, p);
             PK_LAUNCH_CHECK();
             return 0;
         }
-        if (skinny_on && !g_gemm_tile_forced && a_kc && M <= TM && N >= 4 * SN && splitk == 1 && stats == nullptr) {
+        if (!win && skinny_on && !g_gemm_tile_forced && a_kc && M <= TM && N >= 4 * SN && splitk == 1 && stats == nullptr) {
             BnActArgs q = {};
             const dim3 sgrid((unsigned)((N + SN - 1) / SN));
             if (b_kc) hipLaunchKernelGGL((gemm_bf16s_kernel<false, true>), sgrid, dim3(256), 2 * SSTAGE, st, p, q);
@@ -1256,11 +1281,15 @@
             PK_CHECK_HIP(hipFuncSetAttribute((const void*)gemm_bf16_256_kernel<true, false>, hipFuncAttributeMaxDynamicSharedMemorySize, 8 * PIECE));
             PK_CHECK_HIP(hipFuncSetAttribute((const void*)gemm_bf16_256_kernel<false, true>, hipFuncAttributeMaxDynamicSharedMemorySize, 8 * PIECE));
             PK_CHECK_HIP(hipFuncSetAttribute((const void*)gemm_bf16_256_kernel<false, false>, hipFuncAttributeMaxDynamicSharedMemorySize, 8 * PIECE));
+            PK_CHECK_HIP(hipFuncSetAttribute((const void*)gemm_bf16_256_walk_kernel<true, true>, hipFuncAttributeMaxDynamicSharedMemorySize, 8 * PIECE));
             attr_done = true;
         }
         dim3 grid256((unsigned)(p.per_xcd * 8)), block512(512);
         const size_t lds256 = 8 * PIECE;
-        if (a_kc && b_kc) hipLaunchKernelGGL((gemm_bf16_256_kernel<true, true>), grid256, block512, lds256, st, p);
+        int cap = win ? max_workgroups : 0;
+        if (cap >= 8) cap &= ~7;
+        if (cap > 0 && cap < p.per_xcd * 8) hipLaunchKernelGGL((gemm_bf16_256_walk_kernel<true, true>), dim3((unsigned)cap), block512, lds256, st, p);
+        else if (a_kc && b_kc) hipLaunchKernelGGL((gemm_bf16_256_kernel<true, true>), grid256, block512, lds256, st, p);
         else if (a_kc && !b_kc) hipLaunchKernelGGL((gemm_bf16_256_kernel<true, false>), grid256, block512, lds256, st, p);
         else if (!a_kc && b_kc) hipLaunchKernelGGL((gemm_bf16_256_kernel<false, true>), grid256, block512, lds256, st, p);
         else hipLaunchKernelGGL((gemm_bf16_256_kernel<false, false>), grid256, block512, lds256, st, p);
@@ -1325,6 +1354,22 @@
     *row_blocks = fused ? (M + 255) / 256 : 0;
     return gemm_bf16_impl(stream, M, N, K, alpha, A, lda, a_kc, B, ldb, b_kc, 0.f, C, ldc, bias, 1, nullptr,
                           fused ? stats : nullptr);
+}
+
+extern "C" int pk_gemm_bf16_rows_ok(int M, int N) { return M > 0 && N > 0 && gemm_tile_for(M, N, 1, 1) == 256; }
+extern "C" int pk_gemm_bf16_rows(void* stream, int M, int N, int K, float alpha, const uint16_t* A, int64_t lda,
+                                 const uint16_t* B, int64_t ldb, float* C, int64_t ldc, const float* bias, int row0, int rows,
+                                 int max_workgroups) {
+    PK_REQUIRE(rows >= 0, "pk_gemm_bf16_rows: negative row count");
+    return gemm_bf16_impl(stream, M, N, K, alpha, A, lda, 1, B, ldb, 1, 0.f, C, ldc, bias, 1, nullptr, nullptr, row0, rows,
+                          max_workgroups);
+}
+extern "C" int pk_gemm_bf16_stats_rows(void* stream, int M, int N, int K, float alpha, const uint16_t* A, int64_t lda,
+                                       const uint16_t* B, int64_t ldb, float* C, int64_t ldc, const float* bias, float* stats,
+                                       int row0, int rows, int max_workgroups) {
+    PK_REQUIRE(rows >= 0 && stats != nullptr, "pk_gemm_bf16_stats_rows: negative row count or null statistics buffer");
+    return gemm_bf16_impl(stream, M, N, K, alpha, A, lda, 1, B, ldb, 1, 0.f, C, ldc, bias, 1, nullptr, stats, row0, rows,
+                          max_workgroups);
 }
 
 extern "C" int pk_gemm_bf16_small_splitk(int M, int N, int K) {
diff --git a/pytorch-kaldi_amd/csrc/pk_rec2_common.h b/pytorch-kaldi_amd/csrc/pk_rec2_common.h
--- a/pytorch-kaldi_amd/csrc/pk_rec2_common.h
+++ b/pytorch-kaldi_amd/csrc/pk_rec2_common.h
@@ -42,6 +42,7 @@
     float* lnpart;
     int ln_cg0;
     int ln_ncg;
+    int t0, t1;
 };
 
 struct Plan2 {
diff --git a/pytorch-kaldi_amd/csrc/pk_rec_persist2.hip b/pytorch-kaldi_amd/csrc/pk_rec_persist2.hip
--- a/pytorch-kaldi_amd/csrc/pk_rec_persist2.hip
+++ b/pytorch-kaldi_amd/csrc/pk_rec_persist2.hip
@@ -20,6 +20,7 @@
     const int tid = threadIdx.x, lane = tid & 63, wave = tid >> 6;
     const int c = blockIdx.x % a.C, p = blockIdx.x / a.C;
     const int H = a.H, Hp = a.Hp, B = a.B, T = a.T, GH = G * H;
+    const int t0 = a.t0, t1 = a.t1;
     const int n_base = a.row0 + c * a.rpc;
     int nrows = a.R - n_base;
     nrows = nrows < a.rpc ? nrows : a.rpc;
@@ -89,6 +90,11 @@
         msk[r] = (a.mask != nullptr && ok) ? a.mask[(long)n * H + unit] : a.mask_scalar;
         hprev[r] = 0.f;
         cprev[r] = 0.f;
+        if (t0 > 0 && ok) {
+            const int dir = n >= B ? 1 : 0, b = n - dir * B;
+            const long ts = dir ? (T - t0) : (t0 - 1);
+            hprev[r] = a.Y[(ts * B + b) * a.YH + dir * H + unit];
+        }
     }
     const int vrow = lane >> 2, vu0 = ubase + (lane & 3) * 4;
     const int vn = n_base + (vrow < nrows ? vrow : 0);
@@ -146,11 +152,11 @@
             *reinterpret_cast<pk_f32x2*>(st_base + (long)tt * st_step) = st_val;
         }
     };
-#define PK_LP0(E) load_proj(0, E)
+#define PK_LP0(E) load_proj(t0, E)
     PK_EDGE_DISPATCH(PK_LP0);
     const u32x4 sentinel = u32x4{0xFFFFFFFFu, 0xFFFFFFFFu, 0xFFFFFFFFu, 0xFFFFFFFFu};
     if (a.self_fill) {
-        for (int tt = 0; tt < PK_R2_FILL_AHEAD && tt < T; ++tt)
+        for (int tt = t0; tt < t0 + PK_R2_FILL_AHEAD && tt < T; ++tt)
             pub_store<false>(rs, pbase + (pk_ok ? (unsigned)(pdir ? (T - 1 - tt) : tt) * TS : 0u), sentinel);
         asm volatile("s_waitcnt vmcnt(0)" ::: "memory");
     }
@@ -161,7 +167,7 @@
     auto run = [&](auto FASTC, auto SEC) {
     const bool fast = decltype(FASTC)::value < 0 ? fast_rt : decltype(FASTC)::value != 0;
     constexpr int SE = decltype(SEC)::value;
-    for (int t = 0; t < T; ++t) {
+    for (int t = t0; t < t1; ++t) {
         const int step_idx = t;
         PK_TRACE(0);
         f32x4 acc[G];
@@ -184,11 +190,11 @@
         if (t > 0) PK_BARRIER_LDS();
         else PK_LDS_ORDER();
         PK_TRACE(2);
-        if (t > 0) {
+        if (t > t0) {
 #define PK_FO(E) flush_outputs(t - 1, E)
             PK_EDGE_DISPATCH_S(PK_FO);
         }
-        if (t + 1 < T) {
+        if (t + 1 < t1) {
 #define PK_LP1(E) load_proj(t + 1, E)
             PK_EDGE_DISPATCH_S(PK_LP1);
         }
@@ -303,7 +309,7 @@
     } else {
         PK_RUN_SPECIALISED(run, fast_rt);
     }
-#define PK_FOL(E) flush_outputs(T - 1, E)
+#define PK_FOL(E) flush_outputs(t1 - 1, E)
     PK_EDGE_DISPATCH(PK_FOL);
 }
 
@@ -887,13 +893,27 @@
     return cell == PK_CELL_LIGRU ? pick_bwd<PK_CELL_LIGRU>(act) : cell == PK_CELL_RNN ? pick_bwd<PK_CELL_RNN>(act) : pick_bwd<PK_CELL_LSTM>(act);
 }
 
+extern "C" int pk_rec_fwd_bf16_window_ok(int cell) {
+    return (cell == PK_CELL_LIGRU || cell == PK_CELL_RNN) && !pk_rec3_covers(cell, 0);
+}
+
 static int rec_fwd_bf16_impl(void* stream, int cell, int act, int T, int B, int bidir, int H, const float* P,
                              const float* pscale, const float* pshift, const float* U, const float* mask,
                              float mask_scalar, float* Y, float* S, uint16_t* Yb, int64_t y_pitch, int prefilled,
-                             const PkLnHost* ln) {
+                             const PkLnHost* ln, int t_begin = 0, int t_end = -1) {
     const char* who = "pk_rec_fwd_bf16";
     int rc = pk_rec2_check(who, 1, cell, T, B, bidir, H);
     if (rc) return rc;
+    if (t_end < 0) t_end = T;
+    const bool window = t_begin != 0 || t_end != T;
+    if (window) {
+        PK_REQUIRE(t_begin >= 0 && t_begin < t_end && t_end <= T, "pk_rec_fwd_bf16_window: bad window [%d, %d) of %d steps",
+                   t_begin, t_end, T);
+        PK_REQUIRE(pk_rec_fwd_bf16_window_ok(cell) && ln == nullptr && !traced(cell, act),
+                   "pk_rec_fwd_bf16_window: cell %d does not run on the kernel that takes a time window", cell);
+        PK_REQUIRE(Y != nullptr && S != nullptr && prefilled != 0,
+                   "pk_rec_fwd_bf16_window: training form only (Y and S written), exchange buffer self-filled or filled by the caller");
+    }
     PK_REQUIRE(S != nullptr || (ln == nullptr && !traced(cell, act)), "pk_rec_fwd_bf16: S may be null only without per-step LayerNorm");
     PK_REQUIRE(Y != nullptr || S == nullptr, "pk_rec_fwd_bf16: Y may be null only together with S");
     hipStream_t st = pk_stream(stream);
@@ -906,6 +926,8 @@
     rc = pk_rec2_prepare_fwd(a, pl, pk_rec2_make_plan, cell, act, T, B, bidir, H, y_pitch, P, pscale, pshift, U, mask, mask_scalar, Y, S);
     if (rc) return rc;
     a.Yb = (unsigned short*)Yb;
+    a.t0 = t_begin;
+    a.t1 = t_end;
     a.self_fill = prefilled == 2 ? 1 : 0;
     if (prefilled != 1 && !a.self_fill) PK_CHECK_HIP(hipMemsetAsync(Yb, 0xFF, (size_t)T * B * y_pitch * 2, st));
     size_t lds;
@@ -923,13 +945,20 @@
                        : nosave ? (cell == PK_CELL_LIGRU ? pick_fwd_nosave<PK_CELL_LIGRU>(act) : cell == PK_CELL_RNN ? pick_fwd_nosave<PK_CELL_RNN>(act)
                                                                                                                       : pick_fwd_nosave<PK_CELL_LSTM>(act))
                                 : pick_fwd(cell, act);
-    return pk_rec2_run(st, a, pl, cell, false, k, 256, lds, who, ln, REC2_HELP_FULL);
+    return pk_rec2_run(st, a, pl, cell, false, k, 256, lds, who, ln, window ? REC2_HELP_NONE : REC2_HELP_FULL);
 }
 extern "C" int pk_rec_fwd_bf16(void* stream, int cell, int act, int T, int B, int bidir, int H, const float* P,
                                const float* pscale, const float* pshift, const float* U, const float* mask,
                                float mask_scalar, float* Y, float* S, uint16_t* Yb, int64_t y_pitch, int prefilled) {
     return rec_fwd_bf16_impl(stream, cell, act, T, B, bidir, H, P, pscale, pshift, U, mask, mask_scalar, Y, S, Yb, y_pitch,
                              prefilled, nullptr);
+}
+extern "C" int pk_rec_fwd_bf16_window(void* stream, int cell, int act, int T, int B, int bidir, int H, const float* P,
+                                      const float* pscale, const float* pshift, const float* U, const float* mask,
+                                      float mask_scalar, float* Y, float* S, uint16_t* Yb, int64_t y_pitch, int prefilled,
+                                      int t_begin, int t_end) {
+    return rec_fwd_bf16_impl(stream, cell, act, T, B, bidir, H, P, pscale, pshift, U, mask, mask_scalar, Y, S, Yb, y_pitch,
+                             prefilled, nullptr, t_begin, t_end);
 }
 extern "C" int pk_rec_fwd_bf16_ln(void* stream, int cell, int act, int T, int B, int bidir, int H, const float* P,
                                   const float* pscale, const float* pshift, const float* U, const float* mask,
diff --git a/pytorch-kaldi_amd/functional.py b/pytorch-kaldi_amd/functional.py
--- a/pytorch-kaldi_amd/functional.py
+++ b/pytorch-kaldi_amd/functional.py
@@ -25,6 +25,7 @@
         self.side_late = _lib.experiment("side_late", "1") != "0"
         self.side_cus = _lib.experiment("side_cus", "0") != "0"
         self.fused_cost = _lib.experiment("fused_cost", "1") != "0"
+        self.fwd_slices = int(_lib.experiment("fwd_slices", "0"))
         assert self.precision in PREC, self.precision
         assert self.rec_algo in ("auto", "stepwise", "persistent"), self.rec_algo
 
@@ -369,20 +370,37 @@
     return C
 
 
-def gemm_bf16_bn_stats(M, N, K, A, lda, a_kc, B, ldb, b_kc, C, ldc, bias=None, gates=None):
+def gemm_bf16_bn_stats(M, N, K, A, lda, a_kc, B, ldb, b_kc, C, ldc, bias=None, gates=None, sliced=None):
     lib = _lib.load()
 
     def done(mean, var):
         return (mean, var) if gates is None else (mean, var) + tuple(bn_finalize_gates(mean, var, *gates))
 
     if _lib.experiment("gemm_stats", "1") == "0":
+        assert sliced is None
         gemm_bf16(M, N, K, A, lda, a_kc, B, ldb, b_kc, C, ldc, bias=bias)
         return done(*bn_stats(C if ldc == N else C.as_strided((M, N), (ldc, 1))))
-    stats = torch.empty(int(lib.pk_gemm_bf16_stats_floats(M, N)), device=C.device, dtype=torch.float32)
-    rb = ctypes.c_int(0)
-    rc = lib.pk_gemm_bf16_stats(_stream(), M, N, K, 1.0, _p(A), lda, int(a_kc), _p(B), ldb, int(b_kc), _p(C), ldc, _p(bias),
-                                _p(stats), ctypes.byref(rb))
-    _lib.check(rc, "pk_gemm_bf16_stats")
+    if sliced is not None:
+        assert a_kc and b_kc
+        chunks, free_cus, make_B = sliced
+        stats = _side_empty(int(lib.pk_gemm_bf16_stats_floats(M, N)), C.device, torch.float32)
+        Bt = [B]
+
+        def prep():
+            Bt[0] = make_B()
+
+        def launch(row0, rows, cap):
+            _lib.check(lib.pk_gemm_bf16_stats_rows(_stream(), M, N, K, 1.0, _p(A), lda, _p(Bt[0]), ldb, _p(C), ldc, _p(bias),
+                                                   _p(stats), row0, rows, cap), "pk_gemm_bf16_stats_rows")
+
+        _gemm_rows_sliced(chunks, free_cus, launch, lambda: [A, C, stats, bias, Bt[0]], prep if make_B is not None else None)
+        rb = ctypes.c_int((M + 255) // 256)
+    else:
+        stats = torch.empty(int(lib.pk_gemm_bf16_stats_floats(M, N)), device=C.device, dtype=torch.float32)
+        rb = ctypes.c_int(0)
+        rc = lib.pk_gemm_bf16_stats(_stream(), M, N, K, 1.0, _p(A), lda, int(a_kc), _p(B), ldb, int(b_kc), _p(C), ldc,
+                                    _p(bias), _p(stats), ctypes.byref(rb))
+        _lib.check(rc, "pk_gemm_bf16_stats")
     if rb.value == 0:
         return done(*bn_stats(C if ldc == N else C.as_strided((M, N), (ldc, 1))))
     mean, var = torch.empty(N, device=C.device), torch.empty(N, device=C.device)
@@ -538,6 +556,75 @@
             return
         for q, r in zip(params, rows):
             q.grad.add_(r)
+
+def fwd_slice_plan(T, B, bidir, k, tile_rows=256):
+    if k < 1 or not bidir or T < 2 or B < 1:
+        return None
+    g = 1
+    while (B * g) % tile_rows:
+        g += 1
+    if T % g:
+        return None
+    s0 = ((T + 1) // 2 + g - 1) // g * g
+    if s0 >= T:
+        return None
+    cuts = sorted({s0 + (T - s0) * j // k // g * g for j in range(k)} | {T})
+    plan, prev = [], 0
+    for s in cuts:
+        lo, hi = T - s, T - prev
+        if prev == 0:
+            ranges = [(B * lo, B * (s - lo))] if s > lo else []
+        else:
+            ranges = [(B * lo, B * (hi - lo)), (B * prev, B * (s - prev))]
+            if hi == prev:
+                ranges = [(B * lo, B * (s - lo))]
+        plan.append((prev, s, [r for r in ranges if r[1] > 0]))
+        prev = s
+    return plan
+
+
+class _FwdSlices:
+    handover = None
+
+
+def _fwd_slices_take(h, xb, M, N):
+    if h is None or h[0] != xb.data_ptr() or h[1] != M or xb.shape[0] != M:
+        return None
+    if not _lib.load().pk_gemm_bf16_rows_ok(M, N):
+        return None
+    return h[2], h[3]
+
+
+def _side_empty(*shape_device_dtype):
+    *shape, device, dtype = shape_device_dtype
+    if _Side.stream is None:
+        _Side.stream = _make_side_stream()
+    with torch.cuda.stream(_Side.stream):
+        return torch.empty(*shape, device=device, dtype=dtype)
+
+
+def _gemm_rows_sliced(chunks, free_cus, launch, side_tensors, prepare=None):
+    main = torch.cuda.current_stream()
+    if _Side.stream is None:
+        _Side.stream = _make_side_stream()
+    side = _Side.stream
+    if len(chunks) == 1 and prepare is not None:
+        prepare()
+    with torch.cuda.stream(side):
+        for i, (ranges, ev) in enumerate(chunks[:-1]):
+            side.wait_event(ev)
+            if i == 0 and prepare is not None:
+                prepare()
+            for row0, rows in ranges:
+                launch(row0, rows, free_cus)
+    for t in side_tensors():
+        if t is not None:
+            t.record_stream(side)
+            t.record_stream(main)
+    main.wait_stream(side)
+    for row0, rows in chunks[-1][0]:
+        launch(row0, rows, 0)
+
 
 _XB_LAST = None
 
@@ -777,7 +864,21 @@
         ldz = _up(N, 32)
         z = torch.empty(M, ldz, device=x2.device, dtype=torch.float32)
         Kx = K if xseg is None else xseg[0] * xseg[2]
-        gemm_bf16(M, N, Kx, xb, xb.shape[1], 1, wb, wb.shape[1], 1, z, ldz, bias=bias)
+        if callable(wb):
+            chunks, free_cus, make_wb = wb()
+            z = _side_empty(M, ldz, x2.device, torch.float32)
+            wbt = [None]
+
+            def prep():
+                wbt[0] = make_wb()
+
+            def launch(row0, rows, cap):
+                _lib.check(lib.pk_gemm_bf16_rows(_stream(), M, N, Kx, 1.0, _p(xb), xb.shape[1], _p(wbt[0]), wbt[0].shape[1], _p(z),
+                                                 ldz, _p(bias), row0, rows, cap), "pk_gemm_bf16_rows")
+
+            _gemm_rows_sliced(chunks, free_cus, launch, lambda: [xb, z, bias, wbt[0]], prep)
+        else:
+            gemm_bf16(M, N, Kx, xb, xb.shape[1], 1, wb, wb.shape[1], 1, z, ldz, bias=bias)
         y = _new(M, N, like=x2)
         amax = torch.empty(M, device=x2.device, dtype=torch.int32)
         _lib.check(lib.pk_logsoftmax_fwd_ld_argmax(_stream(), _p(z), ldz, M, N, _p(y), _p(amax)), "pk_logsoftmax_fwd_ld_argmax")
@@ -822,8 +923,17 @@
             xb, xseg, wb = tw[0], None, wb_plain
         else:
             xb, xseg = tw
-            wb = cvt_bf16(w, *xseg)
-            assert wb.shape[1] == xb.shape[1]
+            sliced = None
+            if weight.is_contiguous() and weight.is_leaf and (bias is None or bias.is_leaf):
+                sliced = _fwd_slices_take(_FwdSlices.handover, xb, x2.shape[0], weight.shape[0])
+                if sliced is not None:
+                    _FwdSlices.handover = None
+            if sliced is None:
+                wb = cvt_bf16(w, *xseg)
+                assert wb.shape[1] == xb.shape[1]
+            else:
+                wside = _side_empty(w.shape[0], xb.shape[1], w.device, torch.bfloat16)
+                wb = lambda: sliced + ((lambda: cvt_bf16(w, *xseg, out=wside)),)
     _DxShare.epoch += 1
     _DxShare.table.clear()
     _DxShare.epoch_fwd = _DxShare.epoch
@@ -1690,8 +1800,11 @@
     _accumulate_rows(params, [d[g * H:(g + 1) * H] for g in range(G)])
 
 
-def _rec_bf16_fwd(lib, cfg, geom, P, pscale, pshift, Ucat, mask, Y, S, Yb, prefilled, Xb=None, ln=None):
+def _rec_bf16_fwd(lib, cfg, geom, P, pscale, pshift, Ucat, mask, Y, S, Yb, prefilled, Xb=None, ln=None, window=None):
     name = _REC_BF16[cfg.route.family] % "fwd"
+    if window is not None:
+        assert cfg.route.family == "bf16" and ln is None
+        name += "_window"
     a = [_stream(), CELL[cfg.cell], ACT[cfg.act], geom.T, geom.B, int(cfg.bidir), cfg.H, _p(P), _p(pscale), _p(pshift),
          _p(Ucat), _p(mask), float(cfg.mask_scalar)]
     if ln is not None:
@@ -1700,7 +1813,18 @@
     if cfg.route.family.startswith("2p"):
         a.append(_p(Xb))
     a += [geom.y_pitch, prefilled] + ([_p(ln[3])] if ln is not None else [])
+    if window is not None:
+        a += [int(window[0]), int(window[1])]
     _lib.check(getattr(lib, name)(*a), name)
+
+
+def _fwd_slices_wanted(lib, cfg, geom, Y, S, prefilled):
+    k = settings.fwd_slices
+    if (k < 1 or not settings.wgrad_side or Y is None or S is None or not prefilled or cfg.route.family != "bf16"
+            or _Kinks.queue is not None or current_lengths() is not None or torch.cuda.is_current_stream_capturing()
+            or not lib.pk_rec_fwd_bf16_window_ok(CELL[cfg.cell])):
+        return None
+    return fwd_slice_plan(geom.T, geom.B, cfg.bidir, k)
 
 
 def _rec_bf16_bwd(lib, cfg, geom, Ucat, mask, Y, S, dY, dP2, dGb, prefilled, ln=None):
@@ -2012,7 +2136,13 @@
         geom = _rec_geom(lib, cfg, x.shape)
         H, bn_train = cfg.H, cfg.use_bn and cfg.training
         T, B, D, ndir, TB, GH = geom.T, geom.B, geom.D, geom.ndir, geom.TB, geom.GH
+        sliced, handover, _FwdSlices.handover = None, _FwdSlices.handover, None
+        if (handover is not None and xb_in is not None and bn_train and Wcat.is_contiguous() and cfg.wparams
+                and Wcat.untyped_storage().data_ptr() == cfg.wparams[0].untyped_storage().data_ptr()
+                and _lib.experiment("gemm_stats", "1") != "0"):
+            sliced = _fwd_slices_take(handover, xb_in, TB, GH)
         Wcat, Ucat = Wcat.contiguous(), Ucat.contiguous()
+        make_Wb = None
         if xb_in is None:
             xseg = None
             xb, Wb, K = cvt_bf16(_rows2d(x)), cvt_bf16(Wcat), D
@@ -2020,7 +2150,12 @@
             xseg = cfg.xseg
             nseg, seglen, segpad = xseg
             assert nseg * seglen == D and xb_in.shape[0] == TB
-            xb, Wb, K = xb_in, cvt_bf16(Wcat, nseg, seglen, segpad), nseg * segpad
+            xb, K = xb_in, nseg * segpad
+            if sliced is None:
+                Wb = cvt_bf16(Wcat, nseg, seglen, segpad)
+            else:
+                Wb = _side_empty(Wcat.shape[0], _up(K, 64), Wcat.device, torch.bfloat16)
+                make_Wb = lambda: cvt_bf16(Wcat, nseg, seglen, segpad, out=Wb)
             assert Wb.shape[1] == xb.shape[1]
         Yb = torch.empty(TB, geom.y_pitch, device=x.device, dtype=torch.bfloat16)
         self_fill = settings.self_fill and lib.pk_rec_self_fill(CELL[cfg.cell]) == 1
@@ -2031,13 +2166,14 @@
         fill = _Prefill()
         if not self_fill:
             fill.start(Yb, Xb, dGb)
-        P = _new(TB, GH, like=Wcat)
+        P = _new(TB, GH, like=Wcat) if sliced is None else _side_empty(TB, GH, Wcat.device, Wcat.dtype)
         mean = var = pscale = pshift = None
+        sl = None if sliced is None else sliced + (make_Wb,)
         if bn_train and cfg.bn_bufs is not None:
             mean, var, pscale, pshift = gemm_bf16_bn_stats(TB, GH, K, xb, xb.shape[1], 1, Wb, Wb.shape[1], 1, P, GH, gates=(
-                gamma, beta, cfg.eps, H, cfg.bn_bufs[0], cfg.bn_bufs[1], cfg.bn_bufs[2], cfg.momentum, ndir * TB))
+                gamma, beta, cfg.eps, H, cfg.bn_bufs[0], cfg.bn_bufs[1], cfg.bn_bufs[2], cfg.momentum, ndir * TB), sliced=sl)
         elif bn_train:
-            mean, var = gemm_bf16_bn_stats(TB, GH, K, xb, xb.shape[1], 1, Wb, Wb.shape[1], 1, P, GH)
+            mean, var = gemm_bf16_bn_stats(TB, GH, K, xb, xb.shape[1], 1, Wb, Wb.shape[1], 1, P, GH, sliced=sl)
         else:
             gemm_bf16(TB, GH, K, xb, xb.shape[1], 1, Wb, Wb.shape[1], 1, P, GH)
         if pscale is None:
@@ -2048,7 +2184,20 @@
         Yarg = Y if (cfg.keep_y or not infer) else None
         _lib.raise_if_persist_failed()
         fill.wait()
-        _rec_bf16_fwd(lib, cfg, geom, P, pscale, pshift, Ucat, mask, Yarg, S, Yb, 2 if self_fill else fill.done, Xb)
+        prefilled = 2 if self_fill else fill.done
+        plan = _fwd_slices_wanted(lib, cfg, geom, Yarg, S, prefilled)
+        if plan is None:
+            _rec_bf16_fwd(lib, cfg, geom, P, pscale, pshift, Ucat, mask, Yarg, S, Yb, prefilled, Xb)
+        else:
+            chunks = []
+            for t0, t1, ranges in plan:
+                _rec_bf16_fwd(lib, cfg, geom, P, pscale, pshift, Ucat, mask, Yarg, S, Yb, prefilled, Xb, window=(t0, t1))
+                if ranges:
+                    ev = torch.cuda.Event()
+                    ev.record()
+                    chunks.append((ranges, ev))
+            free_cus = max(int(lib.pk_num_cu()) - int(lib.pk_rec_plan_cus(ndir * B, H)), 8)
+            _FwdSlices.handover = (Yb.data_ptr(), TB, chunks, free_cus)
         if S is not None:
             _force_kinks(S, cfg.cell, T, B, ndir, H)
         ctx.self_fill = self_fill
```
